# fanzhongyi/diffusion

Measured on AMD Instinct MI355X. Metric: U-Net training images/sec @256 (SD-2-base U-Net, precomputed latents 4x32x32), higher is better.
Workload: dtype bf16; 1 GPU; SD-2-base U-Net train step, latents 4x32x32, text 77x1024, batch 256/GPU (global 256), microbatch 256, AdamW, dp1; global_batch=256, microbatch=256, parallelism=dp1, params=865910724

## Files before the change

diffusion_amd/_lib.py:

```python
from __future__ import annotations

import ctypes as C
import os

_HERE = os.path.dirname(os.path.abspath(__file__))
LIB_PATH = os.path.join(_HERE, os.environ.get('DA_LIB_ALT') or 'libdiffusion_amd.so')

_vp, _l, _i, _f, _fp, _ll = C.c_void_p, C.c_long, C.c_int, C.c_float, C.c_void_p, C.c_void_p



class DaWgradItem(C.Structure):
    _fields_ = [('dY', C.c_void_p), ('lddy', C.c_long), ('X', C.c_void_p), ('ldx', C.c_long), ('dW', C.c_void_p),
                ('dbias', C.c_void_p), ('N', C.c_int), ('Cin', C.c_int)]


SIGNATURES = {
    'da_gemm_nt': [_vp, _l, _vp, _vp, _l, _fp, _vp, _l, _vp, _l, _i, _i, _i, _i, _i, _i, _i, _i, _i, _i, _i, _f, _fp, _l,
                   _vp],
    'da_set_option': [C.c_char_p, _i],
    'da_gemm_nt_variant_for': [_i, _i, _i, _i, _l],
    'da_gemm_nt_geglu': [_vp, _l, _vp, _vp, _l, _vp, _l, _fp, _i, _i, _i, _vp],
    'da_gemm_nt_geglu_bwd': [_vp, _l, _vp, _vp, _l, _vp, _l, _i, _i, _i, _vp],
    'da_gemm_tn_wgrad': [_vp, _l, _vp, _l, _fp, _fp, _fp, _i, _i, _i, _i, _i, _i, _i, _i, _i, _fp, _l, _vp],
    'da_gemm_tn_variant_for': [_i, _i, _i, _i, _i, _i, _i, _i, _i],
    'da_gemm_tn_wgrad_group': [C.POINTER(DaWgradItem), _i, _i, _fp, _l, _vp],
    'da_gemm_tn_group_plan': [C.POINTER(DaWgradItem), _i, _i, _l, C.POINTER(_i), _i, C.POINTER(_i)],
    'da_attn_fwd': [_vp, _l, _vp, _l, _vp, _l, _vp, _l, _fp, _i, _i, _i, _i, _f, _vp],
    'da_attn_fwd_causal': [_vp, _l, _vp, _l, _vp, _l, _vp, _l, _fp, _i, _i, _i, _f, _vp],
    'da_attn_fwd_wide': [_vp, _l, _vp, _l, _vp, _l, _vp, _l, _fp, _i, _i, _i, _i, _i, _f, _vp],
    'da_attn_bwd': [_vp, _l, _vp, _l, _vp, _l, _vp, _l, _vp, _l, _fp, _fp, _vp, _l, _vp, _l, _vp, _l, _i, _i, _i, _i,
                    _f, _vp],
    'da_norm_scratch_floats': [_i, _i, _i],
    'da_groupnorm_fwd': [_vp, _l, _vp, _l, _fp, _fp, _fp, _fp, _fp, _i, _i, _i, _i, _f, _i, _vp],
    'da_groupnorm_bwd': [_vp, _l, _vp, _l, _vp, _l, _vp, _l, _fp, _fp, _fp, _fp, _fp, _fp, _fp, _i, _i, _i, _i, _i,
                         _vp],
    'da_groupnorm_plan_for': [_i, _i, _i, _i, _l, _l, _i, C.POINTER(_i)],
    'da_layernorm_fwd': [_vp, _l, _vp, _l, _fp, _fp, _fp, _i, _i, _f, _vp],
    'da_layernorm_bwd': [_vp, _l, _vp, _l, _vp, _l, _vp, _l, _fp, _fp, _fp, _fp, _fp, _i, _i, _vp],
    'da_colsum_accum': [_vp, _l, _fp, _fp, _i, _i, _vp],
    'da_image_colsum': [_vp, _l, _vp, _l, _fp, _fp, _i, _i, _i, _vp],
    'da_geglu_fwd': [_vp, _l, _vp, _l, _i, _i, _vp],
    'da_geglu_bwd': [_vp, _l, _vp, _l, _vp, _l, _i, _i, _vp],
    'da_silu_fwd': [_vp, _l, _vp, _l, _i, _i, _vp],
    'da_gelu_fwd': [_vp, _l, _vp, _l, _i, _i, _vp],
    'da_silu_bwd': [_vp, _l, _vp, _l, _vp, _l, _i, _i, _vp],
    'da_quick_gelu_fwd': [_vp, _l, _vp, _l, _i, _i, _vp],
    'da_add': [_vp, _l, _vp, _l, _vp, _l, _i, _i, _vp],
    'da_copy2d': [_vp, _l, _vp, _l, _i, _i, _vp],
    'da_upsample2x_fwd': [_vp, _vp, _i, _i, _i, _i, _vp],
    'da_upsample2x_bwd': [_vp, _vp, _i, _i, _i, _i, _vp],
    'da_timestep_embed': [_ll, _vp, _i, _i, _vp],
    'da_timestep_embed_f32': [_fp, _vp, _i, _i, _vp],
    'da_add_noise': [_fp, _fp, _ll, _fp, _fp, _vp, _fp, _i, _i, _i, _vp],
    'da_add_noise_ex': [_fp, _fp, _vp, _i, _fp, _fp, _vp, _fp, _i, _i, _i, _i, _vp],
    'da_image_ingest': [_vp, _vp, _vp, _i, _i, _vp, _i, _vp],
    'da_image_ingest_rect': [_vp, _vp, _vp, _i, _i, _i, _vp, _i, _vp],
    'da_image_resize': [_vp, _vp, _vp, _i, _i, _i, _vp, _i, _i, _i, _i, _vp],
    'da_clip_preprocess': [_vp, _i, _i, _i, _i, _i, _vp, _i, _vp, _i, _fp, _fp, _vp, _i, _vp],
    'da_clip_score': [_fp, _l, _fp, _l, _i, _i, _fp, _fp, _vp],
    'da_sampler_step': [_fp, _fp, _fp, _fp, _fp, _vp, _l, _i, _i, _i, _i, _vp],
    'da_sampler_step_ms': [_fp, _fp, _fp, _fp, _fp, _vp, _l, _i, _i, _i, _i, _vp],
    'da_sampler_step_blend': [_fp, _fp, _fp, _fp, _fp, _fp, _fp, _fp, _vp, _l, _i, _i, _i, _i, _vp],
    'da_sampler_step_ms_blend': [_fp, _fp, _fp, _fp, _fp, _fp, _fp, _fp, _vp, _l, _i, _i, _i, _i, _vp],
    'da_sampler_init': [_fp, _fp, _fp, _fp, _fp, _fp, _fp, _fp, _vp, _i, _i, _i, _i, _i, _i, _vp],
    'da_guidance_rescale': [_fp, _fp, _i, _f, _fp, _l, _i, _i, _vp],
    'da_sampler_step_rs': [_fp, _fp, _fp, _fp, _fp, _fp, _vp, _l, _i, _i, _i, _i, _vp],
    'da_sampler_step_ms_rs': [_fp, _fp, _fp, _fp, _fp, _fp, _vp, _l, _i, _i, _i, _i, _vp],
    'da_sampler_step_blend_rs': [_fp, _fp, _fp, _fp, _fp, _fp, _fp, _fp, _fp, _vp, _l, _i, _i, _i, _i, _vp],
    'da_sampler_step_ms_blend_rs': [_fp, _fp, _fp, _fp, _fp, _fp, _fp, _fp, _fp, _vp, _l, _i, _i, _i, _i, _vp],
    'da_mse_loss_w': [_fp, _fp, _vp, _fp, _fp, _l, _i, _i, _ll, _fp, _i, _f, _f, _i, _vp],
    'da_mse_loss': [_fp, _fp, _vp, _fp, _fp, _l, _f, _f, _i, _vp],
    'da_mse_loss_c': [_fp, _fp, _vp, _fp, _fp, _l, _i, _f, _f, _i, _vp],
    'da_adamw': [_fp, _fp, _fp, _fp, _vp, _fp, _f, _l, _f, _f, _f, _f, _f, _i, _f, _vp],
    'da_segment_sumsq': [_fp, _vp, _i, _vp, _i, _fp, _fp, _fp, _f, _f, _vp],
    'da_segment_sumsq_scratch_floats': [_i],
    'da_adamw_dev': [_fp, _fp, _fp, _fp, _vp, _fp, _f, _l, _f, _f, _f, _f, _f, _i, _fp, _vp],
    'da_cast_f32_bf16': [_fp, _vp, _l, _vp],
    'da_transpose_weight': [_vp, _vp, _i, _i, _i, _vp],
    'da_transpose_weights_batched': [_vp, _vp, _vp, _i, _i, _vp],
}
_RESTYPES = {'da_norm_scratch_floats': C.c_long, 'da_segment_sumsq_scratch_floats': C.c_long}

_lib = None


class NativeLibraryMissing(RuntimeError):
    pass


def load():
    global _lib
    if _lib is not None:
        return _lib
    import torch
    if not os.path.exists(LIB_PATH):
        raise NativeLibraryMissing(
            f'{LIB_PATH} not found: build it with `make -C diffusion_amd/csrc` (or __graft_entry__.build()). '
            'diffusion_amd has no CPU / PyTorch fallback for its kernels.')
    lib = C.CDLL(LIB_PATH)
    for name, argtypes in SIGNATURES.items():
        fn = getattr(lib, name)
        fn.argtypes = argtypes
        fn.restype = _RESTYPES.get(name, C.c_int)
    _lib = lib
    for kv in filter(None, os.environ.get('DA_SET_OPTIONS', '').split(',')):
        k, _, v = kv.partition('=')
        if lib.da_set_option(k.strip().encode(), int(v)) != 0:
            raise ValueError(f'DA_SET_OPTIONS: da_set_option({k.strip()!r}, {v}) was rejected')
    return lib


_ERR = {1: 'DA_ERR_SHAPE (arguments rejected, nothing launched)', 2: 'DA_ERR_LAUNCH (HIP error)'}


def call(name: str, *args):
    fn = getattr(load(), name)
    rc = fn(*args)
    if rc != 0:
        raise RuntimeError(f'{name} failed: {_ERR.get(rc, rc)}')
```

diffusion_amd/csrc/gemm_nt.hip:

```cpp
#include <string.h>

#include "common.hpp"
#include "diffusion_amd.h"

namespace {

struct GemmNTParams {
  const bf16* A;
  const bf16* W;
  void* C;
  const float* bias;
  const bf16* rowbias;
  const bf16* R;
  long lda, ldc, ldrb, ldr;
  int M, N, K, Cin;
  int Hin, Win, Hout, Wout;
  int ksize, mode;
  int out_fp32;
  float alpha;
  int tiles_m, tiles_n;
};

constexpr int BM = 128, BN = 128, BK = 64;
constexpr int STAGE_BYTES = (BM + BN) * BK * 2;
constexpr int EPI_LD = 68;
constexpr int EPI_BYTES = 4 * 64 * EPI_LD * 4;
constexpr int SMEM_BYTES = (2 * STAGE_BYTES > EPI_BYTES) ? 2 * STAGE_BYTES : EPI_BYTES;

DEVINL int swz(int row, int chunk) { return row * 128 + ((chunk ^ ((row >> 1) & 7)) << 4); }

__global__ __launch_bounds__(256, 2) void gemm_nt_kernel(GemmNTParams p) {
  extern __shared__ __attribute__((aligned(16))) char smem[];
  const int tid = threadIdx.x;
  const int lane = tid & 63;
  const int wave = tid >> 6;
  const int wm = wave >> 1, wn = wave & 1;

  const int nblk = p.tiles_m * p.tiles_n;
  int bid = blockIdx.x;
  {
    const int q = nblk >> 3, r = nblk & 7;
    const int xcd = bid & 7, idx = bid >> 3;
    bid = (xcd < r ? xcd * (q + 1) : r * (q + 1) + (xcd - r) * q) + idx;
  }
  const int tm = bid / p.tiles_n, tn = bid - tm * p.tiles_n;
  const int m0 = tm * BM, n0 = tn * BN;

  const int scol = tid & 7;
  const int srow = tid >> 3;
  const int HWo = p.Hout * p.Wout;
  const int pad = (p.ksize == 3) ? 1 : 0;

  int pixbase[4], oh[4], ow[4];
  bool mval[4];
  const bf16* wptr[4];
  bool nval[4];
#pragma unroll
  for (int i = 0; i < 4; ++i) {
    int m = m0 + srow + 32 * i;
    mval[i] = m < p.M;
    int mm = mval[i] ? m : 0;
    int b = mm / HWo;
    int rem = mm - b * HWo;
    oh[i] = rem / p.Wout;
    ow[i] = rem - oh[i] * p.Wout;
    pixbase[i] = b * p.Hin * p.Win;
    int n = n0 + srow + 32 * i;
    nval[i] = n < p.N;
    wptr[i] = p.W + (long)(nval[i] ? n : 0) * p.K;
  }

  int kk = scol * 8;
  int tap = kk / p.Cin;
  int cc = kk - tap * p.Cin;

  bf16x8 ra[4], rb[4];
  auto load_tile = [&]() {
    const bool kval = kk < p.K;
    int r = 0, s = 0;
    if (p.ksize == 3) {
      r = tap / 3;
      s = tap - 3 * r;
    }
#pragma unroll
    for (int i = 0; i < 4; ++i) {
      int ih, iw;
      bool ok = kval && mval[i];
      if (p.mode == 0) {
        ih = oh[i] + r - pad;
        iw = ow[i] + s - pad;
      } else if (p.mode == 1) {
        ih = 2 * oh[i] + r - pad;
        iw = 2 * ow[i] + s - pad;
      } else if (p.mode == 4) {
        ih = 2 * oh[i] + r;
        iw = 2 * ow[i] + s;
      } else if (p.mode == 2) {
        int th = oh[i] + r - 1, tw = ow[i] + s - 1;
        ok = ok && !((th | tw) & 1);
        ih = th >> 1;
        iw = tw >> 1;
      } else {
        int th = oh[i] + r - 1, tw = ow[i] + s - 1;
        ok = ok && th >= 0 && tw >= 0 && th < p.Hout && tw < p.Wout;
        ih = th >> 1;
        iw = tw >> 1;
      }
      ok = ok && ih >= 0 && iw >= 0 && ih < p.Hin && iw < p.Win;
      ra[i] = ok ? ld8(p.A + (long)(pixbase[i] + ih * p.Win + iw) * p.lda + cc) : zero8();
      rb[i] = (kval && nval[i]) ? ld8(wptr[i] + kk) : zero8();
    }
    kk += BK;
    cc += BK;
    while (cc >= p.Cin) {
      cc -= p.Cin;
      ++tap;
    }
  };
  auto store_tile = [&](int buf) {
    char* Ab = smem + buf * STAGE_BYTES;
    char* Bb = Ab + BM * BK * 2;
#pragma unroll
    for (int i = 0; i < 4; ++i) {
      int row = srow + 32 * i;
      int off = swz(row, scol);
      *reinterpret_cast<bf16x8*>(Ab + off) = ra[i];
      *reinterpret_cast<bf16x8*>(Bb + off) = rb[i];
    }
  };

  f32x4 acc[4][4];
#pragma unroll
  for (int i = 0; i < 4; ++i)
#pragma unroll
    for (int j = 0; j < 4; ++j) acc[i][j] = f32x4{0.f, 0.f, 0.f, 0.f};

  auto compute = [&](int buf) {
    const char* Ab = smem + buf * STAGE_BYTES;
    const char* Bb = Ab + BM * BK * 2;
#pragma unroll
    for (int s = 0; s < 2; ++s) {
      bf16x8 a[4], b[4];
      const int chunk = s * 4 + (lane >> 4);
#pragma unroll
      for (int i = 0; i < 4; ++i) {
        int row = wm * 64 + i * 16 + (lane & 15);
        a[i] = *reinterpret_cast<const bf16x8*>(Ab + swz(row, chunk));
        int rowb = wn * 64 + i * 16 + (lane & 15);
        b[i] = *reinterpret_cast<const bf16x8*>(Bb + swz(rowb, chunk));
      }
#pragma unroll
      for (int i = 0; i < 4; ++i)
#pragma unroll
        for (int j = 0; j < 4; ++j)
          acc[i][j] = __builtin_amdgcn_mfma_f32_16x16x32_bf16(a[i], b[j], acc[i][j], 0, 0, 0);
    }
  };

  const int nk = (p.K + BK - 1) / BK;
  load_tile();
  store_tile(0);
  __syncthreads();
  for (int t = 0; t < nk; ++t) {
    if (t + 1 < nk) load_tile();
    compute(t & 1);
    if (t + 1 < nk) store_tile((t + 1) & 1);
    __syncthreads();
  }

  float* ew = reinterpret_cast<float*>(smem) + wave * (64 * EPI_LD);
#pragma unroll
  for (int i = 0; i < 4; ++i)
#pragma unroll
    for (int j = 0; j < 4; ++j)
#pragma unroll
      for (int e = 0; e < 4; ++e) {
        int row = i * 16 + (lane >> 4) * 4 + e;
        int col = j * 16 + (lane & 15);
        ew[row * EPI_LD + col] = acc[i][j][e];
      }
  __syncthreads();
  const int col8 = (lane & 7) * 8;
  const int n = n0 + wn * 64 + col8;
  if (n < p.N) {
    float bv[8];
#pragma unroll
    for (int e = 0; e < 8; ++e) bv[e] = p.bias ? p.bias[n + e] : 0.f;
#pragma unroll
    for (int pass = 0; pass < 8; ++pass) {
      int row = pass * 8 + (lane >> 3);
      int m = m0 + wm * 64 + row;
      if (m >= p.M) continue;
      const f32x4 v0 = *reinterpret_cast<const f32x4*>(&ew[row * EPI_LD + col8]);
      const f32x4 v1 = *reinterpret_cast<const f32x4*>(&ew[row * EPI_LD + col8 + 4]);
      float v[8] = {v0[0], v0[1], v0[2], v0[3], v1[0], v1[1], v1[2], v1[3]};
#pragma unroll
      for (int e = 0; e < 8; ++e) v[e] = v[e] * p.alpha + bv[e];
      if (p.rowbias) {
        int b = m / HWo;
        bf16x8 rbv = ld8(p.rowbias + (long)b * p.ldrb + n);
#pragma unroll
        for (int e = 0; e < 8; ++e) v[e] += bf2f(rbv[e]);
      }
      if (p.R) {
        bf16x8 rv = ld8(p.R + (long)m * p.ldr + n);
#pragma unroll
        for (int e = 0; e < 8; ++e) v[e] += bf2f(rv[e]);
      }
      if (p.out_fp32) {
        float* cp = reinterpret_cast<float*>(p.C) + (long)m * p.ldc + n;
        *reinterpret_cast<f32x4*>(cp) = f32x4{v[0], v[1], v[2], v[3]};
        *reinterpret_cast<f32x4*>(cp + 4) = f32x4{v[4], v[5], v[6], v[7]};
      } else {
        bf16x8 o;
#pragma unroll
        for (int e = 0; e < 8; ++e) o[e] = f2bf(v[e]);
        st8(reinterpret_cast<bf16*>(p.C) + (long)m * p.ldc + n, o);
      }
    }
  }
}

}

int da_gemm_nt_v2_dispatch(int variant, int splits, float* ws, const void* A, long lda, const void* W, void* C, long ldc, const float* bias,
                           const void* rowbias, long ldrb, const void* R, long ldr, int M, int N, int K, int Cin,
                           int Hin, int Win, int Hout, int Wout, int ksize, int mode, int out_fp32, float alpha,
                           hipStream_t stream);

int da_gemm_nt_v3_try(const void* A, long lda, const void* W, void* C, long ldc, const float* bias, const void* R, long ldr,
                      int M, int N, int K, hipStream_t stream);
extern int g_nt_stream, g_nt_stream_lw;
int da_gemm_nt_ws_try(const void* A, long lda, const void* W, const float* bias, const void* R, long ldr, void* C, long ldc,
                      int M, int N, int K, hipStream_t stream);
extern int g_nt_ws;

extern int g_tn_variant;
extern int g_nt_korder;
extern int g_nt_persist;
extern int g_reserve_cus;
extern int g_nt_persist_conv;
extern int g_nt_de;
extern int g_grad_overwrite;
extern int g_attn_fused_bwd;
extern int g_tn_ring, g_tn_ungroup;
extern int g_gn_resident, g_gn_resident_form, g_gn_resident_min_slab;
int da_usable_cus(int cus);
static int g_nt_variant = 0;
static int g_nt_mfma32 = 0;
static int g_nt_splitk = 1;

static int g_nt_dispatch = 1;

static int pick_nt_variant_legacy(int M, int N, int K, int Cin, long ws_floats, int* splits) {
  *splits = 1;
  const long tm = (M + 255) / 256;
  if (N % 320 == 0 && tm * (N / 320) >= 160) return 12;
  if (N % 160 == 0 && tm * (N / 160) >= 200) return 5;
  if (N % 256 == 0 && tm * (N / 256) >= 160) return 14;
  if (N % 160 != 0 && tm * ((N + 127) / 128) >= 200) return 4;
  if (N % 320 == 0 && g_nt_splitk) {
    const long tiles = tm * (N / 320);
    const int nk = K / 64;
    int s = (int)((256 + tiles - 1) / tiles);
    if (s > 8) s = 8;
    while (s > 1 && (nk / s < 8 || (long)s * M * N > ws_floats)) --s;
    if (s > 1 && tiles * s >= 96) {
      *splits = s;
      return 12;
    }
  }
  return 1;
}

static int pick_nt_variant(int M, int N, int K, int Cin, long ws_floats, int* splits) {
  *splits = 1;
  if (Cin % 64 != 0) return 1;
  if (g_nt_variant == 4 || g_nt_variant == 5 || g_nt_variant == 10 || g_nt_variant == 11 || g_nt_variant == 12 || g_nt_variant == 14 ||
      g_nt_variant == 15 || g_nt_variant == 16 || g_nt_variant == 18)
    return g_nt_variant;
  if (g_nt_variant != 0) return 1;
  if (!g_nt_dispatch) return pick_nt_variant_legacy(M, N, K, Cin, ws_floats, splits);
  struct Form { int variant, bm, bn; double step_us, fixed_us; };
  static const Form forms[] = {{12, 256, 320, 1.5, 8.0}, {14, 256, 256, 1.3, 8.0}, {5, 256, 160, 1.16, 6.0}, {18, 384, 128, 1.37, 8.0},
                               {4, 256, 128, 1.07, 5.0}};
  const int nk = K / 64;
  const int ncu = da_usable_cus(256);
  double best = 1e30;
  int best_v = 4, best_s = 1;
  for (const Form& f : forms) {
    const long tiles = ((M + f.bm - 1) / f.bm) * ((N + f.bn - 1) / f.bn);
    for (int s = 1; s <= (g_nt_splitk ? 8 : 1); ++s) {
      if (s > 1 && (nk / s < 4 || (long)s * M * N > ws_floats)) break;
      const long rounds = (tiles * s + ncu - 1) / ncu;
      const int steps = (nk + s - 1) / s;
      double t = (double)rounds * (steps * f.step_us + f.fixed_us);
      if (s > 1) t += 20.0 + ((double)s * M * N * 4.0 + (double)M * N * 2.0) / 5.0e6;
      if (t < best * 0.97) {
        best = t;
        best_v = f.variant;
        best_s = s;
      }
    }
  }
  *splits = best_s;
  if (best_v == 12 && (g_nt_mfma32 == 1 || (g_nt_mfma32 < 0 && K <= 320))) return 15;
  return best_v;
}

extern "C" int da_gemm_nt_variant_for(int M, int N, int K, int Cin, long ws_floats) {
  int s;
  return pick_nt_variant(M, N, K, Cin, ws_floats, &s);
}

extern "C" int da_set_option(const char* key, int value) {
  if (key && !strcmp(key, "gemm_nt_variant")) {
    g_nt_variant = value;
    return DA_OK;
  }
  if (key && !strcmp(key, "gemm_nt_splitk")) {
    g_nt_splitk = value;
    return DA_OK;
  }
  if (key && !strcmp(key, "gemm_nt_dispatch")) {
    g_nt_dispatch = value;
    return DA_OK;
  }
  if (key && !strcmp(key, "gemm_nt_persist")) {
    g_nt_persist = value;
    return DA_OK;
  }
  if (key && !strcmp(key, "gemm_nt_korder")) {
    g_nt_korder = value;
    return DA_OK;
  }
  if (key && !strcmp(key, "gemm_nt_mfma32")) {
    g_nt_mfma32 = value;
    return DA_OK;
  }
  if (key && !strcmp(key, "gemm_tn_variant")) {
    g_tn_variant = value;
    return DA_OK;
  }
  if (key && !strcmp(key, "attn_fused_bwd")) {
    g_attn_fused_bwd = value;
    return DA_OK;
  }
  if (key && !strcmp(key, "gemm_nt_ws")) {
    g_nt_ws = value;
    return DA_OK;
  }
  if (key && !strcmp(key, "gemm_tn_ring")) {
    if (value != 0 && value != 4 && value != 5) return DA_ERR_SHAPE;
    g_tn_ring = value;
    return DA_OK;
  }
  if (key && !strcmp(key, "gemm_tn_ungroup")) {
    if (value != 0 && value != 1) return DA_ERR_SHAPE;
    g_tn_ungroup = value;
    return DA_OK;
  }
  if (key && !strcmp(key, "gemm_nt_stream_lw")) {
    if (value != 4 && value != 16) return DA_ERR_SHAPE;
    g_nt_stream_lw = value;
    return DA_OK;
  }
  if (key && !strcmp(key, "gemm_nt_stream")) {
    g_nt_stream = value;
    return DA_OK;
  }
  if (key && !strcmp(key, "gemm_nt_de")) {
    g_nt_de = value;
    return DA_OK;
  }
  if (key && !strcmp(key, "gemm_nt_persist_conv")) {
    g_nt_persist_conv = value;
    return DA_OK;
  }
  if (key && !strcmp(key, "gn_resident")) {
    if (value < 0) return DA_ERR_SHAPE;
    g_gn_resident = value;
    return DA_OK;
  }
  if (key && !strcmp(key, "gn_resident_min_slab")) {
    if (value < 0) return DA_ERR_SHAPE;
    g_gn_resident_min_slab = value;
    return DA_OK;
  }
  if (key && !strcmp(key, "gn_resident_form")) {
    if (value < 0 || value > 2) return DA_ERR_SHAPE;
    g_gn_resident_form = value;
    return DA_OK;
  }
  if (key && !strcmp(key, "grad_overwrite")) {
    g_grad_overwrite = value ? 1 : 0;
    return DA_OK;
  }
  if (key && !strcmp(key, "reserve_cus")) {
    if (value < 0 || value > 128) return DA_ERR_SHAPE;
    g_reserve_cus = value;
    return DA_OK;
  }
  return DA_ERR_SHAPE;
}

extern "C" int da_gemm_nt(const void* A, long lda, const void* W, void* C, long ldc, const float* bias,
                          const void* rowbias, long ldrb, const void* R, long ldr, int M, int N, int K, int Cin,
                          int Hin, int Win, int Hout, int Wout, int ksize, int mode, int out_fp32, float alpha,
                          float* splitk_ws, long splitk_ws_floats, hipStream_t stream) {
  DA_CLEAR_ERR();
  if (M <= 0 || N <= 0 || K <= 0) return DA_ERR_SHAPE;
  if ((N & 7) || (Cin & 7) || (K % Cin) || (lda & 7) || (ldc & 7)) return DA_ERR_SHAPE;
  if (ksize != 1 && ksize != 3) return DA_ERR_SHAPE;
  if (K != ksize * ksize * Cin) return DA_ERR_SHAPE;
  if (mode < 0 || mode > 4) return DA_ERR_SHAPE;
  if (mode == 4 && ksize != 3) return DA_ERR_SHAPE;
  if (Hout <= 0 || Wout <= 0 || (M % (Hout * Wout))) return DA_ERR_SHAPE;
  if (R && (ldr & 7)) return DA_ERR_SHAPE;
  if (rowbias && (ldrb & 7)) return DA_ERR_SHAPE;
  if (g_nt_ws && g_nt_variant == 0 && ksize == 1 && mode == 0 && !out_fp32 && alpha == 1.0f && !rowbias) {
    const int rc = da_gemm_nt_ws_try(A, lda, W, bias, R, ldr, C, ldc, M, N, K, stream);
    if (rc >= 0) return rc;
  }
  if (g_nt_stream && g_nt_variant == 0 && ksize == 1 && mode == 0 && !out_fp32 && alpha == 1.0f && !rowbias &&
      (g_nt_stream == 2 || (K <= 640 && (long)((M + 127) / 128) * ((N + 319) / 320) >= 512))) {
    const int rc = da_gemm_nt_v3_try(A, lda, W, C, ldc, bias, R, ldr, M, N, K, stream);
    if (rc >= 0) return rc;
  }
  {
    int splits = 1;
    const int variant = pick_nt_variant(M, N, K, Cin, splitk_ws ? splitk_ws_floats : 0, &splits);
    if (variant != 1)
      return da_gemm_nt_v2_dispatch(variant, splits, splitk_ws, A, lda, W, C, ldc, bias, rowbias, ldrb, R, ldr, M, N, K, Cin, Hin, Win,
                                    Hout, Wout, ksize, mode, out_fp32, alpha, stream);
  }
  GemmNTParams p;
  p.A = (const bf16*)A; p.W = (const bf16*)W; p.C = C; p.bias = bias;
  p.rowbias = (const bf16*)rowbias; p.R = (const bf16*)R;
  p.lda = lda; p.ldc = ldc; p.ldrb = ldrb; p.ldr = ldr;
  p.M = M; p.N = N; p.K = K; p.Cin = Cin;
  p.Hin = Hin; p.Win = Win; p.Hout = Hout; p.Wout = Wout;
  p.ksize = ksize; p.mode = mode; p.out_fp32 = out_fp32; p.alpha = alpha;
  p.tiles_m = (M + BM - 1) / BM;
  p.tiles_n = (N + BN - 1) / BN;
  static unsigned long long attr_done = 0;
  if (da_ensure_dyn_smem((const void*)gemm_nt_kernel, SMEM_BYTES, &attr_done) != DA_OK) return DA_ERR_LAUNCH;
  hipLaunchKernelGGL(gemm_nt_kernel, dim3(p.tiles_m * p.tiles_n), dim3(256), SMEM_BYTES, stream, p);
  DA_CHECK_LAUNCH();
  return DA_OK;
}
```

diffusion_amd/csrc/norms.hip:

```cpp
#include "common.hpp"
#include "diffusion_amd.h"

extern int g_grad_overwrite;
int g_gn_resident = 192;
int g_gn_resident_form = 0;
int g_gn_resident_min_slab = 64 * 1024;

namespace {

struct ChanReduceParams {
  const bf16* X;
  const bf16* DY;
  const float* mean_rstd;
  const float* gamma;
  const float* beta;
  float* partial;
  long ldx, lddy;
  int HW, C, G, cpg, nchunks, ppc, pxt, silu;
};

template <int MODE>
__global__ void chan_reduce_kernel(ChanReduceParams p) {
  extern __shared__ __attribute__((aligned(16))) float red[];
  const int tid = threadIdx.x;
  const int vec0 = blockIdx.z * 512;
  const int nvec = min(512, (p.C >> 3) - vec0);
  const int Cb = nvec * 8;
  const int lvec = tid % nvec, pl = tid / nvec;
  const int vec = vec0 + lvec;
  const int b = blockIdx.y, chunk = blockIdx.x;
  const int p0 = chunk * p.ppc;
  const int p1 = min(p.HW, p0 + p.ppc);
  const bool active = pl < p.pxt;
  float s1[8], s2[8];
#pragma unroll
  for (int e = 0; e < 8; ++e) { s1[e] = 0.f; s2[e] = 0.f; }
  float rs[8], nm[8], za[8], zb[8];
  if (MODE == 1) {
#pragma unroll
    for (int e = 0; e < 8; ++e) {
      int c = 8 * vec + e;
      int g = c / p.cpg;
      const float mu = p.mean_rstd[((long)b * p.G + g) * 2];
      rs[e] = p.mean_rstd[((long)b * p.G + g) * 2 + 1];
      nm[e] = -mu * rs[e];
      za[e] = rs[e] * p.gamma[c];
      zb[e] = fmaf(nm[e], p.gamma[c], p.beta[c]);
    }
  }
  if (active) {
    for (int pix = p0 + pl; pix < p1; pix += p.pxt) {
      const long row = (long)b * p.HW + pix;
      bf16x8 x = ld8(p.X + row * p.ldx + 8 * vec);
      if (MODE == 0) {
#pragma unroll
        for (int e = 0; e < 8; ++e) {
          float v = bf2f(x[e]);
          s1[e] += v;
          s2[e] += v * v;
        }
      } else if (MODE == 1) {
        bf16x8 dy = ld8(p.DY + row * p.lddy + 8 * vec);
#pragma unroll
        for (int e = 0; e < 8; ++e) {
          const float xf = bf2f(x[e]);
          const float xh = fmaf(xf, rs[e], nm[e]);
          float dz = bf2f(dy[e]);
          if (p.silu) dz *= dsilu_f(fmaf(xf, za[e], zb[e]));
          s1[e] += dz;
          s2[e] += dz * xh;
        }
      } else {
#pragma unroll
        for (int e = 0; e < 8; ++e) s1[e] += bf2f(x[e]);
      }
    }
#pragma unroll
    for (int e = 0; e < 8; ++e) {
      red[((long)pl * Cb + 8 * lvec + e) * 2] = s1[e];
      red[((long)pl * Cb + 8 * lvec + e) * 2 + 1] = s2[e];
    }
  }
  __syncthreads();
  float* out = p.partial + (((long)b * p.nchunks + chunk) * p.C + 8 * vec0) * 2;
  for (int c = tid; c < Cb; c += blockDim.x) {
    float a = 0.f, q = 0.f;
    for (int k = 0; k < p.pxt; ++k) {
      a += red[((long)k * Cb + c) * 2];
      q += red[((long)k * Cb + c) * 2 + 1];
    }
    out[c * 2] = a;
    out[c * 2 + 1] = q;
  }
}

int launch_chan_reduce(int mode, ChanReduceParams& p, int B, hipStream_t stream) {
  const int nvec_total = p.C >> 3;
  if (nvec_total < 1) return DA_ERR_SHAPE;
  const int zsplit = (nvec_total + 511) / 512;
  const int nvec = nvec_total < 512 ? nvec_total : 512;
  int pxt = 512 / nvec;
  if (pxt > p.HW) pxt = p.HW;
  if (pxt < 1) pxt = 1;
  p.pxt = pxt;
  p.ppc = (p.HW + p.nchunks - 1) / p.nchunks;
  const size_t smem = (size_t)pxt * nvec * 8 * 2 * sizeof(float);
  dim3 grid(p.nchunks, B, zsplit), block(nvec * pxt);
  if (mode == 0) hipLaunchKernelGGL(chan_reduce_kernel<0>, grid, block, smem, stream, p);
  else if (mode == 1) hipLaunchKernelGGL(chan_reduce_kernel<1>, grid, block, smem, stream, p);
  else hipLaunchKernelGGL(chan_reduce_kernel<2>, grid, block, smem, stream, p);
  DA_CHECK_LAUNCH();
  return DA_OK;
}

int pick_chunks(int B, int HW) {
  int n = 2048 / (B > 0 ? B : 1);
  if (n > 64) n = 64;
  int maxc = HW / 16;
  if (n > maxc) n = maxc;
  if (n < 1) n = 1;
  return n;
}

constexpr int GN_GPB = 8;

DEVINL void chunk_sum2(const float* pp, long stride, int nchunks, float& a, float& q) {
  float a0 = 0.f, a1 = 0.f, q0 = 0.f, q1 = 0.f;
  int k = 0;
  for (; k + 1 < nchunks; k += 2) {
    const float2 v0 = *reinterpret_cast<const float2*>(pp + (long)k * stride);
    const float2 v1 = *reinterpret_cast<const float2*>(pp + (long)(k + 1) * stride);
    a0 += v0.x; q0 += v0.y;
    a1 += v1.x; q1 += v1.y;
  }
  if (k < nchunks) {
    const float2 v0 = *reinterpret_cast<const float2*>(pp + (long)k * stride);
    a0 += v0.x; q0 += v0.y;
  }
  a = a0 + a1;
  q = q0 + q1;
}

__global__ void gn_fwd_finalize_kernel(const float* partial, const float* gamma, const float* beta, float* mean_rstd,
                                       float* scale_shift, int C, int G, int cpg, int nchunks, int HW, float eps) {
  extern __shared__ __attribute__((aligned(16))) float sh[];
  const int b = blockIdx.x;
  const int g0 = blockIdx.y * GN_GPB, ng = min(GN_GPB, G - g0);
  const int c0 = g0 * cpg, nc = ng * cpg;
  float* gs = sh + 2 * GN_GPB * cpg;
  for (int cl = threadIdx.x; cl < nc; cl += blockDim.x) {
    float a, q;
    chunk_sum2(partial + ((long)b * nchunks * C + c0 + cl) * 2, (long)C * 2, nchunks, a, q);
    sh[2 * cl] = a;
    sh[2 * cl + 1] = q;
  }
  __syncthreads();
  for (int gl = threadIdx.x; gl < ng; gl += blockDim.x) {
    float a = 0.f, q = 0.f;
    for (int k = 0; k < cpg; ++k) {
      a += sh[2 * (gl * cpg + k)];
      q += sh[2 * (gl * cpg + k) + 1];
    }
    const float n = (float)cpg * (float)HW;
    float mean = a / n;
    float var = fmaxf(q / n - mean * mean, 0.f);
    float rstd = rsqrtf(var + eps);
    gs[2 * gl] = mean;
    gs[2 * gl + 1] = rstd;
    mean_rstd[((long)b * G + g0 + gl) * 2] = mean;
    mean_rstd[((long)b * G + g0 + gl) * 2 + 1] = rstd;
  }
  __syncthreads();
  for (int cl = threadIdx.x; cl < nc; cl += blockDim.x) {
    const int gl = cl / cpg, c = c0 + cl;
    float sc = gs[2 * gl + 1] * gamma[c];
    scale_shift[((long)b * C + c) * 2] = sc;
    scale_shift[((long)b * C + c) * 2 + 1] = beta[c] - gs[2 * gl] * sc;
  }
}

__global__ void gn_apply_kernel(const bf16* X, long ldx, bf16* Y, long ldy, const float* scale_shift, int HW, int C,
                                long total_vec, int silu) {
  const int nvec = C >> 3;
  for (long i = (long)blockIdx.x * blockDim.x + threadIdx.x; i < total_vec; i += (long)gridDim.x * blockDim.x) {
    long row = i / nvec;
    int vec = (int)(i - row * nvec);
    int b = (int)(row / HW);
    bf16x8 x = ld8(X + row * ldx + 8 * vec);
    const float* ss = scale_shift + ((long)b * C + 8 * vec) * 2;
    bf16x8 y;
#pragma unroll
    for (int e = 0; e < 8; ++e) {
      float z = bf2f(x[e]) * ss[2 * e] + ss[2 * e + 1];
      y[e] = f2bf(silu ? silu_f(z) : z);
    }
    st8(Y + row * ldy + 8 * vec, y);
  }
}

__global__ void gn_bwd_finalize_kernel(const float* partial, const float* gamma, float* coef, int C, int G, int cpg,
                                       int nchunks, int HW) {
  extern __shared__ __attribute__((aligned(16))) float sh[];
  const int b = blockIdx.x;
  const int g0 = blockIdx.y * GN_GPB, ng = min(GN_GPB, G - g0);
  const int c0 = g0 * cpg, nc = ng * cpg;
  for (int cl = threadIdx.x; cl < nc; cl += blockDim.x) {
    float a, q;
    chunk_sum2(partial + ((long)b * nchunks * C + c0 + cl) * 2, (long)C * 2, nchunks, a, q);
    sh[2 * cl] = a * gamma[c0 + cl];
    sh[2 * cl + 1] = q * gamma[c0 + cl];
  }
  __syncthreads();
  for (int gl = threadIdx.x; gl < ng; gl += blockDim.x) {
    float a = 0.f, q = 0.f;
    for (int k = 0; k < cpg; ++k) {
      a += sh[2 * (gl * cpg + k)];
      q += sh[2 * (gl * cpg + k) + 1];
    }
    const float n = (float)cpg * (float)HW;
    coef[((long)b * G + g0 + gl) * 2] = a / n;
    coef[((long)b * G + g0 + gl) * 2 + 1] = q / n;
  }
}

struct GnApplyParams {
  const bf16* X; const bf16* DY; const bf16* Radd; bf16* OUT;
  const float* mean_rstd; const float* coef; const float* gamma; const float* beta;
  long ldx, lddy, ldr, ldo;
  int HW, C, G, cpg, nchunks, ppc, pxt, silu;
};

template <bool BWD>
__global__ void gn_apply2_kernel(GnApplyParams p) {
  const int tid = threadIdx.x;
  const int vec0 = blockIdx.z * 512;
  const int nvec = min(512, (p.C >> 3) - vec0);
  const int lvec = tid % nvec, pl = tid / nvec;
  if (pl >= p.pxt) return;
  const int vec = vec0 + lvec;
  const int b = blockIdx.y, chunk = blockIdx.x;
  const int p0 = chunk * p.ppc;
  const int p1 = min(p.HW, p0 + p.ppc);
  float sc[8], sh[8], Q[8], R[8];
#pragma unroll
  for (int e = 0; e < 8; ++e) {
    const int c = 8 * vec + e;
    const int g = c / p.cpg;
    const float mu = p.mean_rstd[((long)b * p.G + g) * 2], rs = p.mean_rstd[((long)b * p.G + g) * 2 + 1];
    sc[e] = rs * p.gamma[c];
    sh[e] = p.beta[c] - mu * sc[e];
    if (BWD) {
      const float c1 = p.coef[((long)b * p.G + g) * 2], c2 = p.coef[((long)b * p.G + g) * 2 + 1];
      Q[e] = -rs * rs * c2;
      R[e] = -rs * c1 + mu * rs * rs * c2;
    }
  }
  for (int pix = p0 + pl; pix < p1; pix += p.pxt) {
    const long row = (long)b * p.HW + pix;
    const bf16x8 x = ld8(p.X + row * p.ldx + 8 * vec);
    bf16x8 o;
    if (!BWD) {
#pragma unroll
      for (int e = 0; e < 8; ++e) {
        const float z = fmaf(bf2f(x[e]), sc[e], sh[e]);
        o[e] = f2bf(p.silu ? silu_f(z) : z);
      }
    } else {
      const bf16x8 dy = ld8(p.DY + row * p.lddy + 8 * vec);
      const bf16x8 ra = p.Radd ? ld8(p.Radd + row * p.ldr + 8 * vec) : zero8();
#pragma unroll
      for (int e = 0; e < 8; ++e) {
        const float xf = bf2f(x[e]);
        float dz = bf2f(dy[e]);
        if (p.silu) dz *= dsilu_f(fmaf(xf, sc[e], sh[e]));
        o[e] = f2bf(fmaf(dz, sc[e], fmaf(xf, Q[e], R[e])) + bf2f(ra[e]));
      }
    }
    st8(p.OUT + row * p.ldo + 8 * vec, o);
  }
}

int launch_gn_apply2(bool bwd, GnApplyParams& p, int B, hipStream_t stream) {
  const int nvec_total = p.C >> 3;
  const int zsplit = (nvec_total + 511) / 512;
  const int nvec = nvec_total < 512 ? nvec_total : 512;
  int pxt = 256 / nvec;
  if (pxt < 1) pxt = 1;
  if (pxt > p.HW) pxt = p.HW;
  p.pxt = pxt;
  int nch = (4096 + B * zsplit - 1) / (B * zsplit);
  int maxc = p.HW / (4 * pxt);
  if (nch > maxc) nch = maxc;
  if (nch < 1) nch = 1;
  p.nchunks = nch;
  p.ppc = (p.HW + nch - 1) / nch;
  dim3 grid(nch, B, zsplit), block(nvec * pxt);
  if (bwd) hipLaunchKernelGGL(gn_apply2_kernel<true>, grid, block, 0, stream, p);
  else hipLaunchKernelGGL(gn_apply2_kernel<false>, grid, block, 0, stream, p);
  DA_CHECK_LAUNCH();
  return DA_OK;
}

__global__ void gn_bwd_apply_kernel(const bf16* X, long ldx, const bf16* DY, long lddy, const bf16* Radd, long ldr,
                                    bf16* DX, long lddx, const float* mean_rstd, const float* coef,
                                    const float* gamma, const float* beta, int HW, int C, int G, int cpg,
                                    long total_vec, int silu) {
  const int nvec = C >> 3;
  for (long i = (long)blockIdx.x * blockDim.x + threadIdx.x; i < total_vec; i += (long)gridDim.x * blockDim.x) {
    long row = i / nvec;
    int vec = (int)(i - row * nvec);
    int b = (int)(row / HW);
    bf16x8 x = ld8(X + row * ldx + 8 * vec);
    bf16x8 dy = ld8(DY + row * lddy + 8 * vec);
    bf16x8 ra = Radd ? ld8(Radd + row * ldr + 8 * vec) : zero8();
    bf16x8 o;
#pragma unroll
    for (int e = 0; e < 8; ++e) {
      int c = 8 * vec + e;
      int g = c / cpg;
      const float mu = mean_rstd[((long)b * G + g) * 2], rs = mean_rstd[((long)b * G + g) * 2 + 1];
      const float c1 = coef[((long)b * G + g) * 2], c2 = coef[((long)b * G + g) * 2 + 1];
      float xh = (bf2f(x[e]) - mu) * rs;
      float dz = bf2f(dy[e]);
      if (silu) dz *= dsilu_f(xh * gamma[c] + beta[c]);
      float dx = rs * (dz * gamma[c] - c1 - xh * c2);
      o[e] = f2bf(dx + bf2f(ra[e]));
    }
    st8(DX + row * lddx + 8 * vec, o);
  }
}

constexpr int CSF_CH = 16, CSF_RL = 64;
__global__ __launch_bounds__(CSF_CH * CSF_RL) void chan_sum_finalize_kernel(const float* partial, int nrows, int C,
                                                                            float* out1, float* out2, int overwrite) {
  __shared__ float sh[CSF_RL][CSF_CH][2];
  const int cx = threadIdx.x % CSF_CH, ry = threadIdx.x / CSF_CH;
  const int c = blockIdx.x * CSF_CH + cx;
  float a = 0.f, q = 0.f;
  if (c < C) {
    const float2* pp = reinterpret_cast<const float2*>(partial) + c;
    float a0 = 0.f, a1 = 0.f, a2 = 0.f, a3 = 0.f, q0 = 0.f, q1 = 0.f, q2 = 0.f, q3 = 0.f;
    int k = ry;
    for (; k + 3 * CSF_RL < nrows; k += 4 * CSF_RL) {
      const float2 v0 = pp[(long)k * C], v1 = pp[(long)(k + CSF_RL) * C], v2 = pp[(long)(k + 2 * CSF_RL) * C],
                   v3 = pp[(long)(k + 3 * CSF_RL) * C];
      a0 += v0.x; q0 += v0.y;
      a1 += v1.x; q1 += v1.y;
      a2 += v2.x; q2 += v2.y;
      a3 += v3.x; q3 += v3.y;
    }
    for (; k < nrows; k += CSF_RL) {
      const float2 v = pp[(long)k * C];
      a0 += v.x;
      q0 += v.y;
    }
    a = (a0 + a1) + (a2 + a3);
    q = (q0 + q1) + (q2 + q3);
  }
  sh[ry][cx][0] = a;
  sh[ry][cx][1] = q;
  __syncthreads();
  float la = 0.f, lq = 0.f;
  if (ry < 8) {
#pragma unroll
    for (int j = 0; j < 8; ++j) {
      la += sh[ry * 8 + j][cx][0];
      lq += sh[ry * 8 + j][cx][1];
    }
  }
  __syncthreads();
  if (ry < 8) {
    sh[ry][cx][0] = la;
    sh[ry][cx][1] = lq;
  }
  __syncthreads();
  if (ry == 0 && c < C) {
    float ta = 0.f, tq = 0.f;
#pragma unroll
    for (int j = 0; j < 8; ++j) {
      ta += sh[j][cx][0];
      tq += sh[j][cx][1];
    }
    if (out1) out1[c] = overwrite ? ta : out1[c] + ta;
    if (out2) out2[c] = overwrite ? tq : out2[c] + tq;
  }
}

static inline dim3 chan_sum_grid(int nrows, int C) {
  (void)nrows;
  return dim3((C + CSF_CH - 1) / CSF_CH);
}

__global__ __launch_bounds__(CSF_CH * CSF_RL) void image_colsum_finalize_kernel(const float* partial, bf16* out, long ldo,
                                                                                float* db, int B, int nchunks, int C,
                                                                                int overwrite) {
  __shared__ float sh[CSF_RL][CSF_CH];
  const int cx = threadIdx.x % CSF_CH, ry = threadIdx.x / CSF_CH;
  const int c = blockIdx.x * CSF_CH + cx;
  float tot = 0.f;
  if (c < C) {
    for (int b = ry; b < B; b += CSF_RL) {
      const float* pp = partial + ((long)b * nchunks * C + c) * 2;
      float a0 = 0.f, a1 = 0.f;
      int k = 0;
      for (; k + 1 < nchunks; k += 2) {
        a0 += pp[(long)k * C * 2];
        a1 += pp[(long)(k + 1) * C * 2];
      }
      if (k < nchunks) a0 += pp[(long)k * C * 2];
      const float a = a0 + a1;
      out[(long)b * ldo + c] = f2bf(a);
      tot += a;
    }
  }
  sh[ry][cx] = tot;
  __syncthreads();
  float lt = 0.f;
  if (ry < 8) {
#pragma unroll
    for (int j = 0; j < 8; ++j) lt += sh[ry * 8 + j][cx];
  }
  __syncthreads();
  if (ry < 8) sh[ry][cx] = lt;
  __syncthreads();
  if (ry == 0 && c < C && db) {
    float t = 0.f;
#pragma unroll
    for (int j = 0; j < 8; ++j) t += sh[j][cx];
    db[c] = overwrite ? t : db[c] + t;
  }
}

constexpr int LN_MAXV = 3;

__global__ __launch_bounds__(256) void ln_fwd_kernel(const bf16* X, long ldx, bf16* Y, long ldy, const float* gamma,
                                                     const float* beta, float* mean_rstd, int M, int C, float eps) {
  const int lane = threadIdx.x & 63;
  const int nvec = C >> 3;
  const int wpb = blockDim.x >> 6;
  for (int row = blockIdx.x * wpb + (threadIdx.x >> 6); row < M; row += gridDim.x * wpb) {
    float v[LN_MAXV][8];
    float s = 0.f;
#pragma unroll
    for (int k = 0; k < LN_MAXV; ++k) {
      int vec = lane + 64 * k;
      bf16x8 x = vec < nvec ? ld8(X + (long)row * ldx + 8 * vec) : zero8();
#pragma unroll
      for (int e = 0; e < 8; ++e) {
        v[k][e] = bf2f(x[e]);
        s += v[k][e];
      }
    }
    const float mean = wave_sum(s) / (float)C;
    float q = 0.f;
#pragma unroll
    for (int k = 0; k < LN_MAXV; ++k) {
      int vec = lane + 64 * k;
      if (vec < nvec) {
#pragma unroll
        for (int e = 0; e < 8; ++e) {
          float d = v[k][e] - mean;
          q += d * d;
        }
      }
    }
    const float rstd = rsqrtf(wave_sum(q) / (float)C + eps);
    if (lane == 0) {
      mean_rstd[2 * (long)row] = mean;
      mean_rstd[2 * (long)row + 1] = rstd;
    }
#pragma unroll
    for (int k = 0; k < LN_MAXV; ++k) {
      int vec = lane + 64 * k;
      if (vec < nvec) {
        bf16x8 y;
#pragma unroll
        for (int e = 0; e < 8; ++e) y[e] = f2bf((v[k][e] - mean) * rstd * gamma[8 * vec + e] + beta[8 * vec + e]);
        st8(Y + (long)row * ldy + 8 * vec, y);
      }
    }
  }
}

__global__ __launch_bounds__(256) void ln_bwd_kernel(const bf16* X, long ldx, const bf16* DY, long lddy,
                                                     const bf16* Radd, long ldr, bf16* DX, long lddx,
                                                     const float* gamma, const float* mean_rstd, float* partial,
                                                     int M, int C) {
  extern __shared__ __attribute__((aligned(16))) float red[];
  const int lane = threadIdx.x & 63, wave = threadIdx.x >> 6;
  const int nvec = C >> 3;
  const int wpb = blockDim.x >> 6;
  float dg[LN_MAXV][8], db[LN_MAXV][8], ga[LN_MAXV][8];
#pragma unroll
  for (int k = 0; k < LN_MAXV; ++k) {
    int vec = lane + 64 * k;
#pragma unroll
    for (int e = 0; e < 8; ++e) {
      dg[k][e] = 0.f;
      db[k][e] = 0.f;
      ga[k][e] = vec < nvec ? gamma[8 * vec + e] : 0.f;
    }
  }
  for (int row = blockIdx.x * wpb + wave; row < M; row += gridDim.x * wpb) {
    const float mean = mean_rstd[2 * (long)row], rstd = mean_rstd[2 * (long)row + 1];
    float xh[LN_MAXV][8], dyv[LN_MAXV][8];
    float a = 0.f, q = 0.f;
#pragma unroll
    for (int k = 0; k < LN_MAXV; ++k) {
      int vec = lane + 64 * k;
      bool ok = vec < nvec;
      bf16x8 x = ok ? ld8(X + (long)row * ldx + 8 * vec) : zero8();
      bf16x8 dy = ok ? ld8(DY + (long)row * lddy + 8 * vec) : zero8();
#pragma unroll
      for (int e = 0; e < 8; ++e) {
        xh[k][e] = ok ? (bf2f(x[e]) - mean) * rstd : 0.f;
        dyv[k][e] = bf2f(dy[e]);
        float dxh = dyv[k][e] * ga[k][e];
        a += dxh;
        q += dxh * xh[k][e];
        dg[k][e] += dyv[k][e] * xh[k][e];
        db[k][e] += dyv[k][e];
      }
    }
    a = wave_sum(a) / (float)C;
    q = wave_sum(q) / (float)C;
#pragma unroll
    for (int k = 0; k < LN_MAXV; ++k) {
      int vec = lane + 64 * k;
      if (vec < nvec) {
        bf16x8 ra = Radd ? ld8(Radd + (long)row * ldr + 8 * vec) : zero8();
        bf16x8 o;
#pragma unroll
        for (int e = 0; e < 8; ++e)
          o[e] = f2bf(rstd * (dyv[k][e] * ga[k][e] - a - xh[k][e] * q) + bf2f(ra[e]));
        st8(DX + (long)row * lddx + 8 * vec, o);
      }
    }
  }
#pragma unroll
  for (int k = 0; k < LN_MAXV; ++k) {
    int vec = lane + 64 * k;
    if (vec < nvec) {
#pragma unroll
      for (int e = 0; e < 8; ++e) {
        red[((long)wave * C + 8 * vec + e) * 2] = dg[k][e];
        red[((long)wave * C + 8 * vec + e) * 2 + 1] = db[k][e];
      }
    }
  }
  __syncthreads();
  float* out = partial + (long)blockIdx.x * C * 2;
  for (int c = threadIdx.x; c < C; c += blockDim.x) {
    float a = 0.f, q = 0.f;
    for (int w = 0; w < wpb; ++w) {
      a += red[((long)w * C + c) * 2];
      q += red[((long)w * C + c) * 2 + 1];
    }
    out[c * 2] = a;
    out[c * 2 + 1] = q;
  }
}

template <int CTRL>
DEVINL float dpp_f(float v) {
  return __builtin_bit_cast(float, __builtin_amdgcn_update_dpp(0, __builtin_bit_cast(int, v), CTRL, 0xf, 0xf, false));
}
template <int LPR>
DEVINL float group_sum(float v) {
  v += dpp_f<0xB1>(v);
  v += dpp_f<0x4E>(v);
  if (LPR >= 8) v += dpp_f<0x141>(v);
  if (LPR >= 16) v += dpp_f<0x140>(v);
  if (LPR >= 32) v += lane_xor<16>(v);
  return v;
}

template <int LPR>
__global__ __launch_bounds__(256) void ln_fwd5_kernel(const bf16* X, long ldx, bf16* Y, long ldy, const float* gamma,
                                                      const float* beta, float* mean_rstd, int M, float eps) {
  constexpr int C = 40 * LPR, RPW = 64 / LPR;
  __shared__ __attribute__((aligned(16))) float gb[2 * C];
  for (int c = threadIdx.x; c < C; c += 256) {
    gb[c] = gamma[c];
    gb[C + c] = beta[c];
  }
  __syncthreads();
  const int lane = threadIdx.x & 63, wave = threadIdx.x >> 6;
  const int sub = lane / LPR, j = lane % LPR;
  const long ngroups = ((long)M + RPW - 1) / RPW;
  for (long rg = (long)blockIdx.x * 4 + wave; rg < ngroups; rg += (long)gridDim.x * 4) {
    const long row = rg * RPW + sub;
    const bool ok = row < M;
    const long rowc = ok ? row : M - 1;
    bf16x8 xv[5];
#pragma unroll
    for (int k = 0; k < 5; ++k) xv[k] = ld8(X + rowc * ldx + 8 * (j + LPR * k));
    float s = 0.f;
#pragma unroll
    for (int k = 0; k < 5; ++k)
#pragma unroll
      for (int e = 0; e < 8; ++e) s += bf2f(xv[k][e]);
    const float mean = group_sum<LPR>(s) * (1.f / C);
    float q = 0.f;
#pragma unroll
    for (int k = 0; k < 5; ++k)
#pragma unroll
      for (int e = 0; e < 8; ++e) {
        const float d = bf2f(xv[k][e]) - mean;
        q += d * d;
      }
    const float rstd = rsqrtf(group_sum<LPR>(q) * (1.f / C) + eps);
    if (ok) {
      if (j == 0) *reinterpret_cast<float2*>(mean_rstd + 2 * row) = make_float2(mean, rstd);
#pragma unroll
      for (int k = 0; k < 5; ++k) {
        const int c0 = 8 * (j + LPR * k);
        const f32x4 g0 = *reinterpret_cast<const f32x4*>(gb + c0), g1 = *reinterpret_cast<const f32x4*>(gb + c0 + 4);
        const f32x4 b0 = *reinterpret_cast<const f32x4*>(gb + C + c0), b1 = *reinterpret_cast<const f32x4*>(gb + C + c0 + 4);
        bf16x8 y;
#pragma unroll
        for (int e = 0; e < 4; ++e) {
          y[e] = f2bf((bf2f(xv[k][e]) - mean) * rstd * g0[e] + b0[e]);
          y[e + 4] = f2bf((bf2f(xv[k][e + 4]) - mean) * rstd * g1[e] + b1[e]);
        }
        st8(Y + row * ldy + c0, y);
      }
    }
  }
}

template <int LPR, bool HAS_R>
__global__ __launch_bounds__(256) void ln_bwd5_kernel(const bf16* X, long ldx, const bf16* DY, long lddy,
                                                      const bf16* Radd, long ldr, bf16* DX, long lddx,
                                                      const float* gamma, const float* mean_rstd, float* partial,
                                                      int M) {
  constexpr int C = 40 * LPR, RPW = 64 / LPR;
  __shared__ __attribute__((aligned(16))) float gsm[C];
  __shared__ __attribute__((aligned(16))) float red[4 * C * 2];
  for (int c = threadIdx.x; c < C; c += 256) gsm[c] = gamma[c];
  __syncthreads();
  const int lane = threadIdx.x & 63, wave = threadIdx.x >> 6;
  const int sub = lane / LPR, j = lane % LPR;
  float dg[5][8], db[5][8];
#pragma unroll
  for (int k = 0; k < 5; ++k)
#pragma unroll
    for (int e = 0; e < 8; ++e) {
      dg[k][e] = 0.f;
      db[k][e] = 0.f;
    }
  const long ngroups = ((long)M + RPW - 1) / RPW;
  for (long rg = (long)blockIdx.x * 4 + wave; rg < ngroups; rg += (long)gridDim.x * 4) {
    const long row = rg * RPW + sub;
    const bool ok = row < M;
    const long rowc = ok ? row : M - 1;
    const float okf = ok ? 1.f : 0.f;
    bf16x8 xv[5], dyv[5], rv[5];
#pragma unroll
    for (int k = 0; k < 5; ++k) {
      const int c0 = 8 * (j + LPR * k);
      xv[k] = ld8(X + rowc * ldx + c0);
      dyv[k] = ld8(DY + rowc * lddy + c0);
      if (HAS_R) rv[k] = ld8(Radd + rowc * ldr + c0);
    }
    const float2 ms = *reinterpret_cast<const float2*>(mean_rstd + 2 * rowc);
    const float mean = ms.x, rstd = ms.y;
    float a = 0.f, q = 0.f;
#pragma unroll
    for (int k = 0; k < 5; ++k) {
      const int c0 = 8 * (j + LPR * k);
      const f32x4 g0 = *reinterpret_cast<const f32x4*>(gsm + c0), g1 = *reinterpret_cast<const f32x4*>(gsm + c0 + 4);
#pragma unroll
      for (int e = 0; e < 8; ++e) {
        const float xh = (bf2f(xv[k][e]) - mean) * rstd;
        const float d = bf2f(dyv[k][e]) * okf;
        const float dxh = d * (e < 4 ? g0[e & 3] : g1[e & 3]);
        a += dxh;
        q += dxh * xh;
        dg[k][e] += d * xh;
        db[k][e] += d;
      }
    }
    a = group_sum<LPR>(a) * (1.f / C);
    q = group_sum<LPR>(q) * (1.f / C);
    if (ok) {
#pragma unroll
      for (int k = 0; k < 5; ++k) {
        const int c0 = 8 * (j + LPR * k);
        const f32x4 g0 = *reinterpret_cast<const f32x4*>(gsm + c0), g1 = *reinterpret_cast<const f32x4*>(gsm + c0 + 4);
        bf16x8 o;
#pragma unroll
        for (int e = 0; e < 8; ++e) {
          const float xh = (bf2f(xv[k][e]) - mean) * rstd;
          float v = rstd * (bf2f(dyv[k][e]) * (e < 4 ? g0[e & 3] : g1[e & 3]) - a - xh * q);
          if (HAS_R) v += bf2f(rv[k][e]);
          o[e] = f2bf(v);
        }
        st8(DX + row * lddx + c0, o);
      }
    }
  }
#pragma unroll
  for (int k = 0; k < 5; ++k)
#pragma unroll
    for (int e = 0; e < 8; ++e) {
      if constexpr (LPR <= 8) {
        dg[k][e] += lane_xor<8>(dg[k][e]);
        db[k][e] += lane_xor<8>(db[k][e]);
      }
      if constexpr (LPR <= 16) {
        dg[k][e] += lane_xor<16>(dg[k][e]);
        db[k][e] += lane_xor<16>(db[k][e]);
      }
      dg[k][e] += lane_xor<32>(dg[k][e]);
      db[k][e] += lane_xor<32>(db[k][e]);
      if (sub == 0) {
        red[(wave * C + 8 * (j + LPR * k) + e) * 2] = dg[k][e];
        red[(wave * C + 8 * (j + LPR * k) + e) * 2 + 1] = db[k][e];
      }
    }
  __syncthreads();
  float* out = partial + (long)blockIdx.x * C * 2;
  for (int c = threadIdx.x; c < C; c += 256) {
    float a = 0.f, q = 0.f;
#pragma unroll
    for (int w = 0; w < 4; ++w) {
      a += red[(w * C + c) * 2];
      q += red[(w * C + c) * 2 + 1];
    }
    out[c * 2] = a;
    out[c * 2 + 1] = q;
  }
}


struct GnResParams {
  const bf16* X; const bf16* DY; const bf16* Radd; bf16* OUT;
  const float* gamma; const float* beta;
  float* mean_rstd;
  float* partial;
  long ldx, lddy, ldr, ldo;
  int HW, C, G, cpg, CW, chunks, P, parts, peers8, silu, nseg;
  float eps, inv_n;
};

DEVINL u32x4 ldnt8w(const bf16* p) { return __builtin_nontemporal_load(reinterpret_cast<const u32x4*>(p)); }
DEVINL void st8w(bf16* p, u32x4 v) { *reinterpret_cast<u32x4*>(p) = v; }
DEVINL u32x4 ldnt8o(const bf16* base, unsigned byte_off) {
  return __builtin_nontemporal_load(reinterpret_cast<const u32x4*>(reinterpret_cast<const char*>(base) + byte_off));
}
DEVINL void st8o(bf16* base, unsigned byte_off, u32x4 v) {
  *reinterpret_cast<u32x4*>(reinterpret_cast<char*>(base) + byte_off) = v;
}
DEVINL u32x4 sel8(bool ok, u32x4 v) {
  u32x4 r;
  r[0] = ok ? v[0] : 0u; r[1] = ok ? v[1] : 0u; r[2] = ok ? v[2] : 0u; r[3] = ok ? v[3] : 0u;
  return r;
}
DEVINL float bflo(unsigned w) { return __uint_as_float(w << 16); }
DEVINL float bfhi(unsigned w) { return __uint_as_float(w & 0xffff0000u); }
DEVINL unsigned bfpack(float lo, float hi) {
  bf16x2 v;
  v[0] = f2bf(lo);
  v[1] = f2bf(hi);
  return __builtin_bit_cast(unsigned, v);
}

DEVINL void gn_res_block(const GnResParams& p, int& img, int& part) {
  const int id = blockIdx.x;
  if (p.peers8) {
    const int span = 8 * p.parts;
    const int g = id / span, r = id - g * span;
    part = r >> 3;
    img = g * 8 + (r & 7);
  } else {
    img = id / p.parts;
    part = id - img * p.parts;
  }
}

DEVINL void gn_res_reduce(const GnResParams& p, const float2* red, float2* red2, float2* chs) {
  const int t = threadIdx.x, T = blockDim.x;
  __syncthreads();
  const int rows = p.P < p.HW ? p.P : p.HW;
  for (int idx = t; idx < p.nseg * p.CW; idx += T) {
    const int seg = idx / p.CW, c = idx - seg * p.CW;
    float a0 = 0.f, q0 = 0.f, a1 = 0.f, q1 = 0.f;
    int k = seg;
    for (; k + p.nseg < rows; k += 2 * p.nseg) {
      const float2 v0 = red[(long)k * p.CW + c], v1 = red[(long)(k + p.nseg) * p.CW + c];
      a0 += v0.x; q0 += v0.y;
      a1 += v1.x; q1 += v1.y;
    }
    if (k < rows) {
      const float2 v0 = red[(long)k * p.CW + c];
      a0 += v0.x; q0 += v0.y;
    }
    red2[idx] = make_float2(a0 + a1, q0 + q1);
  }
  __syncthreads();
  for (int c = t; c < p.CW; c += T) {
    float a = 0.f, q = 0.f;
    for (int sgi = 0; sgi < p.nseg; ++sgi) {
      const float2 v = red2[sgi * p.CW + c];
      a += v.x; q += v.y;
    }
    chs[c] = make_float2(a, q);
  }
  __syncthreads();
}

static inline size_t gn_res_lds_floats(int P, int CW, int nseg, int cpg) {
  return (size_t)2 * (P + 1) * CW + (size_t)2 * nseg * CW + 2 * CW + 4 * CW + 4 * (CW / cpg);
}

template <int NL, bool SILU>
__global__ __launch_bounds__(1024) void gn_res_fwd_kernel(GnResParams p) {
  extern __shared__ __attribute__((aligned(16))) float smem[];
  float2* red = reinterpret_cast<float2*>(smem);
  float2* red2 = red + (long)(p.P + 1) * p.CW;
  float2* chs = red2 + (long)p.nseg * p.CW;
  float2* cf = chs + p.CW;
  float2* gs = cf + 2 * p.CW;
  int img, part;
  gn_res_block(p, img, part);
  const int t = threadIdx.x, j = t % p.chunks, p0 = t / p.chunks;
  const bool live = p0 < p.P;
  const int c0 = part * p.CW;
  const bf16* xb = p.X + (long)img * p.HW * p.ldx + c0;
  const int pl = live ? p0 : p.P - 1;
  const int pl0 = live ? p0 : p.P;
  u32x4 a[NL];
#pragma unroll
  for (int k = 0; k < NL; ++k) {
    const int pix = pl + k * p.P;
    const int pc = pix < p.HW ? pix : p.HW - 1;
    a[k] = ldnt8o(xb, (unsigned)(pc * (int)p.ldx + 8 * j) * 2u);
  }
#pragma unroll
  for (int k = 0; k < NL; ++k) a[k] = sel8(live && pl + k * p.P < p.HW, a[k]);
#pragma unroll
  for (int w = 0; w < 4; ++w) {
    float s1 = 0.f, s2 = 0.f, u1 = 0.f, u2 = 0.f;
#pragma unroll
    for (int k = 0; k < NL; ++k) {
      const float v0 = bflo(a[k][w]), v1 = bfhi(a[k][w]);
      s1 += v0;
      s2 = fmaf(v0, v0, s2);
      u1 += v1;
      u2 = fmaf(v1, v1, u2);
    }
    red[pl0 * p.CW + 8 * j + 2 * w] = make_float2(s1, s2);
    red[pl0 * p.CW + 8 * j + 2 * w + 1] = make_float2(u1, u2);
  }
  gn_res_reduce(p, red, red2, chs);
#pragma unroll
  for (int k = 0; k < NL; ++k) reg_tie(a[k]);
  const int ng = p.CW / p.cpg, g0 = c0 / p.cpg;
  for (int gl = t; gl < ng; gl += blockDim.x) {
    float s = 0.f, q = 0.f;
    for (int i = 0; i < p.cpg; ++i) {
      const float2 v = chs[gl * p.cpg + i];
      s += v.x; q += v.y;
    }
    const float mean = s * p.inv_n;
    const float var = fmaxf(q * p.inv_n - mean * mean, 0.f);
    const float rstd = rsqrtf(var + p.eps);
    gs[gl] = make_float2(mean, rstd);
    p.mean_rstd[((long)img * p.G + g0 + gl) * 2] = mean;
    p.mean_rstd[((long)img * p.G + g0 + gl) * 2 + 1] = rstd;
  }
  __syncthreads();
  for (int c = t; c < p.CW; c += blockDim.x) {
    const float2 g = gs[c / p.cpg];
    const float sc = g.y * p.gamma[c0 + c];
    cf[c] = make_float2(sc, p.beta[c0 + c] - g.x * sc);
  }
  __syncthreads();
  if (!live) return;
#pragma unroll
  for (int w = 0; w < 4; ++w) {
    const float2 f0 = cf[8 * j + 2 * w], f1 = cf[8 * j + 2 * w + 1];
#pragma unroll
    for (int k = 0; k < NL; ++k) {
      float z0 = fmaf(bflo(a[k][w]), f0.x, f0.y), z1 = fmaf(bfhi(a[k][w]), f1.x, f1.y);
      if (SILU) {
        z0 = silu_f(z0);
        z1 = silu_f(z1);
      }
      a[k][w] = bfpack(z0, z1);
    }
    __builtin_amdgcn_sched_barrier(0);
  }
  bf16* yb = p.OUT + (long)img * p.HW * p.ldo + c0;
#pragma unroll
  for (int k = 0; k < NL; ++k) {
    const int pix = p0 + k * p.P;
    if (pix < p.HW) st8o(yb, (unsigned)(pix * (int)p.ldo + 8 * j) * 2u, a[k]);
  }
}

template <int NL, bool SILU, int T>
__global__ __launch_bounds__(T) void gn_res_bwd_kernel(GnResParams p) {
  extern __shared__ __attribute__((aligned(16))) float smem[];
  float2* red = reinterpret_cast<float2*>(smem);
  float2* red2 = red + (long)(p.P + 1) * p.CW;
  float2* chs = red2 + (long)p.nseg * p.CW;
  float4* cf = reinterpret_cast<float4*>(chs + p.CW);
  float4* gs = cf + p.CW;
  int img, part;
  gn_res_block(p, img, part);
  const int t = threadIdx.x, j = t % p.chunks, p0 = t / p.chunks;
  const bool live = p0 < p.P;
  const int c0 = part * p.CW;
  const bf16* xb = p.X + (long)img * p.HW * p.ldx + c0;
  const bf16* dyb = p.DY + (long)img * p.HW * p.lddy + c0;
  const int pl = live ? p0 : p.P - 1;
  const int pl0 = live ? p0 : p.P;
  unsigned a[NL][4], b[NL][4];
  {
    u32x4 va[NL], vb[NL];
#pragma unroll
    for (int k = 0; k < NL; ++k) {
      const int pix = pl + k * p.P;
      const int pc = pix < p.HW ? pix : p.HW - 1;
      va[k] = ldnt8o(xb, (unsigned)(pc * (int)p.ldx + 8 * j) * 2u);
      vb[k] = ldnt8o(dyb, (unsigned)(pc * (int)p.lddy + 8 * j) * 2u);
    }
#pragma unroll
    for (int k = 0; k < NL; ++k) {
      const bool ok = live && pl + k * p.P < p.HW;
#pragma unroll
      for (int w = 0; w < 4; ++w) {
        a[k][w] = ok ? va[k][w] : 0u;
        b[k][w] = ok ? vb[k][w] : 0u;
        reg_tie(b[k][w]);
      }
    }
  }
  for (int c = t; c < p.CW; c += blockDim.x) {
    const int g = (c0 + c) / p.cpg;
    const float mu = p.mean_rstd[((long)img * p.G + g) * 2], rs = p.mean_rstd[((long)img * p.G + g) * 2 + 1];
    const float nm = -mu * rs, ga = p.gamma[c0 + c];
    cf[c] = make_float4(rs, nm, rs * ga, fmaf(nm, ga, p.beta[c0 + c]));
  }
  __syncthreads();
#pragma unroll
  for (int w = 0; w < 4; ++w) {
    const float4 f0 = cf[8 * j + 2 * w], f1 = cf[8 * j + 2 * w + 1];
    float s1 = 0.f, s2 = 0.f, u1 = 0.f, u2 = 0.f;
#pragma unroll
    for (int k = 0; k < NL; ++k) {
      const float x0 = bflo(a[k][w]), x1 = bfhi(a[k][w]);
      float d0 = bflo(b[k][w]), d1 = bfhi(b[k][w]);
      if (SILU) {
        d0 *= dsilu_f(fmaf(x0, f0.z, f0.w));
        d1 *= dsilu_f(fmaf(x1, f1.z, f1.w));
        unsigned pk = bfpack(d0, d1);
        reg_tie(pk);
        b[k][w] = pk;
      }
      s1 += d0;
      s2 = fmaf(d0, fmaf(x0, f0.x, f0.y), s2);
      u1 += d1;
      u2 = fmaf(d1, fmaf(x1, f1.x, f1.y), u2);
      if (SILU) __builtin_amdgcn_sched_barrier(0);
    }
    red[pl0 * p.CW + 8 * j + 2 * w] = make_float2(s1, s2);
    red[pl0 * p.CW + 8 * j + 2 * w + 1] = make_float2(u1, u2);
    __builtin_amdgcn_sched_barrier(0);
  }
  gn_res_reduce(p, red, red2, chs);
#pragma unroll
  for (int k = 0; k < NL; ++k) {
#pragma unroll
    for (int w = 0; w < 4; ++w) {
      reg_tie(a[k][w]);
      reg_tie(b[k][w]);
    }
  }
  int j2 = j, q0 = p0;
  reg_tie(j2);
  reg_tie(q0);
  for (int c = t; c < p.CW; c += blockDim.x) {
    const float2 v = chs[c];
    p.partial[((long)img * p.C + c0 + c) * 2] = v.x;
    p.partial[((long)img * p.C + c0 + c) * 2 + 1] = v.y;
  }
  const int ng = p.CW / p.cpg, g0 = c0 / p.cpg;
  for (int gl = t; gl < ng; gl += blockDim.x) {
    float s = 0.f, q = 0.f;
    for (int i = 0; i < p.cpg; ++i) {
      const float2 v = chs[gl * p.cpg + i];
      const float ga = p.gamma[c0 + gl * p.cpg + i];
      s = fmaf(v.x, ga, s);
      q = fmaf(v.y, ga, q);
    }
    const float c1 = s * p.inv_n, c2 = q * p.inv_n;
    const float mu = p.mean_rstd[((long)img * p.G + g0 + gl) * 2], rs = p.mean_rstd[((long)img * p.G + g0 + gl) * 2 + 1];
    gs[gl] = make_float4(mu, rs, -rs * rs * c2, -rs * c1 + mu * rs * rs * c2);
  }
  __syncthreads();
  if (!live) return;
#pragma unroll
  for (int w = 0; w < 4; ++w) {
    const float4 f0 = cf[8 * j2 + 2 * w], f1 = cf[8 * j2 + 2 * w + 1];
    const float4 g0q = gs[(8 * j2 + 2 * w) / p.cpg], g1q = gs[(8 * j2 + 2 * w + 1) / p.cpg];
#pragma unroll
    for (int k = 0; k < NL; ++k) {
      const float x0 = bflo(a[k][w]), x1 = bfhi(a[k][w]);
      const float d0 = bflo(b[k][w]), d1 = bfhi(b[k][w]);
      a[k][w] = bfpack(fmaf(d0, f0.z, fmaf(x0, g0q.z, g0q.w)), fmaf(d1, f1.z, fmaf(x1, g1q.z, g1q.w)));
      if (SILU) __builtin_amdgcn_sched_barrier(0);
    }
    __builtin_amdgcn_sched_barrier(0);
  }
  bf16* ob = p.OUT + (long)img * p.HW * p.ldo + c0;
  if (p.Radd) {
    const bf16* rb = p.Radd + (long)img * p.HW * p.ldr + c0;
#pragma unroll
    for (int k = 0; k < NL; ++k) {
      const int pix = q0 + k * p.P;
      const int pc = pix < p.HW ? pix : p.HW - 1;
      const u32x4 v = ldnt8o(rb, (unsigned)(pc * (int)p.ldr + 8 * j2) * 2u);
#pragma unroll
      for (int w = 0; w < 4; ++w) b[k][w] = v[w];
    }
#pragma unroll
    for (int k = 0; k < NL; ++k)
#pragma unroll
      for (int w = 0; w < 4; ++w)
        a[k][w] = bfpack(bflo(a[k][w]) + bflo(b[k][w]), bfhi(a[k][w]) + bfhi(b[k][w]));
  }
#pragma unroll
  for (int k = 0; k < NL; ++k) {
    const int pix = q0 + k * p.P;
    if (pix < p.HW) st8o(ob, (unsigned)(pix * (int)p.ldo + 8 * j2) * 2u, u32x4{a[k][0], a[k][1], a[k][2], a[k][3]});
  }
}

bool gn_res_plan(int B, int HW, int C, int G, long ld_min, long ld_max, bool bwd, GnResParams& p, int& nl, int& threads) {
  const int cpg = C / G;
  int unit = cpg;
  while (unit & 7) unit += cpg;
  if (unit > C || (C % unit)) return false;
  if ((long)HW * ld_max * 2 >= (1L << 31)) return false;
  const int nT = (bwd && g_gn_resident_form != 1) ? 2 : 1;
  const int Ts[2] = {1024, 768};
  const int maxnl[2] = {bwd ? (g_gn_resident_form == 2 ? 8 : 11) : 21, 14};
  double best = 1e30;
  int best_cw = 0, best_t = 0;
  for (int ti = 0; ti < nT; ++ti) {
    const int T = Ts[ti];
    for (int cw = unit; cw <= C; cw += unit) {
      if (C % cw) continue;
      const int chunks = cw / 8;
      if (chunks > T) break;
      const int P = T / chunks;
      const int n = (HW + P - 1) / P;
      if (n > maxnl[ti]) continue;
      const long wgs = (long)B * (C / cw);
      if (wgs < g_gn_resident) continue;
      const bool aligned = ((cw * 2) % 128 == 0) && ((ld_min * 2) % 128 == 0);
      double cost = aligned ? 1.0 : (double)(cw * 2 + 128) / (double)(cw * 2);
      if (cost > 1.85) continue;
      if ((long)HW * cw * 2 < g_gn_resident_min_slab) continue;
      if (gn_res_lds_floats(P, cw, T / cw < 1 ? 1 : T / cw, cpg) * sizeof(float) > 160 * 1024) continue;
      cost += 0.8 * (1.0 - (double)HW / ((double)P * n)) + 0.01 * ti - 0.002 * n * T / 1024.0;
      if (wgs < 256) cost += 0.05;
      if (cost < best) { best = cost; best_cw = cw; best_t = T; }
    }
  }
  if (!best_cw) return false;
  threads = best_t;
  p.CW = best_cw;
  p.chunks = best_cw / 8;
  p.P = best_t / p.chunks;
  p.parts = C / best_cw;
  p.peers8 = (B % 8 == 0 && p.parts > 1) ? 1 : 0;
  p.nseg = best_t / best_cw < 1 ? 1 : best_t / best_cw;
  nl = (HW + p.P - 1) / p.P;
  return true;
}

template <int NL, bool SILU>
int launch_gn_res_fwd2(const GnResParams& p, int B, hipStream_t stream) {
  const size_t smem = gn_res_lds_floats(p.P, p.CW, p.nseg, p.cpg) * sizeof(float);
  if (smem > 160 * 1024) return DA_ERR_SHAPE;
  static unsigned long long attr_done = 0;
  if (da_ensure_dyn_smem((const void*)gn_res_fwd_kernel<NL, SILU>, 160 * 1024, &attr_done) != DA_OK) return DA_ERR_LAUNCH;
  hipLaunchKernelGGL((gn_res_fwd_kernel<NL, SILU>), dim3(B * p.parts), dim3(1024), smem, stream, p);
  DA_CHECK_LAUNCH();
  return DA_OK;
}

template <int NL>
int launch_gn_res_fwd(const GnResParams& p, int B, hipStream_t stream) {
  return p.silu ? launch_gn_res_fwd2<NL, true>(p, B, stream) : launch_gn_res_fwd2<NL, false>(p, B, stream);
}

template <int NL, bool SILU, int T>
int launch_gn_res_bwd2(const GnResParams& p, int B, hipStream_t stream) {
  const size_t smem = gn_res_lds_floats(p.P, p.CW, p.nseg, p.cpg) * sizeof(float);
  if (smem > 160 * 1024) return DA_ERR_SHAPE;
  static unsigned long long attr_done = 0;
  if (da_ensure_dyn_smem((const void*)gn_res_bwd_kernel<NL, SILU, T>, 160 * 1024, &attr_done) != DA_OK) return DA_ERR_LAUNCH;
  hipLaunchKernelGGL((gn_res_bwd_kernel<NL, SILU, T>), dim3(B * p.parts), dim3(T), smem, stream, p);
  DA_CHECK_LAUNCH();
  return DA_OK;
}

template <int NL, int T>
int launch_gn_res_bwd(const GnResParams& p, int B, hipStream_t stream) {
  return p.silu ? launch_gn_res_bwd2<NL, true, T>(p, B, stream) : launch_gn_res_bwd2<NL, false, T>(p, B, stream);
}

int gn_res_nl_inst(int nl, bool bwd, int threads) {
  if (bwd && threads == 768) return nl <= 11 ? 11 : 14;
  static const int fwd[] = {1, 2, 3, 4, 6, 8, 11, 16, 21}, bwd1024[] = {1, 2, 3, 4, 6, 8, 11};
  const int* v = bwd ? bwd1024 : fwd;
  const int n = bwd ? 7 : 9;
  for (int i = 0; i < n - 1; ++i)
    if (nl <= v[i]) return v[i];
  return v[n - 1];
}

int dispatch_gn_res_fwd(int nl, const GnResParams& p, int B, hipStream_t s) {
  switch (gn_res_nl_inst(nl, false, 1024)) {
    case 1: return launch_gn_res_fwd<1>(p, B, s);
    case 2: return launch_gn_res_fwd<2>(p, B, s);
    case 3: return launch_gn_res_fwd<3>(p, B, s);
    case 4: return launch_gn_res_fwd<4>(p, B, s);
    case 6: return launch_gn_res_fwd<6>(p, B, s);
    case 8: return launch_gn_res_fwd<8>(p, B, s);
    case 11: return launch_gn_res_fwd<11>(p, B, s);
    case 16: return launch_gn_res_fwd<16>(p, B, s);
    default: return launch_gn_res_fwd<21>(p, B, s);
  }
}

int dispatch_gn_res_bwd(int nl, int threads, const GnResParams& p, int B, hipStream_t s) {
  if (threads == 768) return gn_res_nl_inst(nl, true, 768) == 11 ? launch_gn_res_bwd<11, 768>(p, B, s)
                                                                  : launch_gn_res_bwd<14, 768>(p, B, s);
  switch (gn_res_nl_inst(nl, true, 1024)) {
    case 1: return launch_gn_res_bwd<1, 1024>(p, B, s);
    case 2: return launch_gn_res_bwd<2, 1024>(p, B, s);
    case 3: return launch_gn_res_bwd<3, 1024>(p, B, s);
    case 4: return launch_gn_res_bwd<4, 1024>(p, B, s);
    case 6: return launch_gn_res_bwd<6, 1024>(p, B, s);
    case 8: return launch_gn_res_bwd<8, 1024>(p, B, s);
    default: return launch_gn_res_bwd<11, 1024>(p, B, s);
  }
}

}

extern "C" long da_norm_scratch_floats(int B, int HW, int C) {
  long a = (long)B * pick_chunks(B, HW) * C * 2;
  long b = 1024L * C * 2;
  return a > b ? a : b;
}

extern "C" int da_groupnorm_plan_for(int B, int HW, int C, int G, long ld_min, long ld_max, int bwd, int* out) {
  if (B <= 0 || HW <= 0 || C <= 0 || G <= 0 || (C % G) || (C & 7) || (ld_min & 7) || (ld_max & 7) || !out) return -1;
  GnResParams r = {};
  int nl = 0, threads = 0;
  if (g_gn_resident && gn_res_plan(B, HW, C, G, ld_min, ld_max, bwd != 0, r, nl, threads)) {
    const int o[7] = {threads, gn_res_nl_inst(nl, bwd != 0, threads), r.CW, r.parts, r.peers8, r.P, 0};
    for (int i = 0; i < 7; ++i) out[i] = o[i];
    return 1;
  }
  const int o[7] = {0, 0, C, 1, 0, 0, pick_chunks(B, HW)};
  for (int i = 0; i < 7; ++i) out[i] = o[i];
  return 0;
}

extern "C" int da_groupnorm_fwd(const void* X, long ldx, void* Y, long ldy, const float* gamma, const float* beta,
                                float* mean_rstd, float* scale_shift, float* scratch, int B, int HW, int C, int G,
                                float eps, int silu, hipStream_t stream) {
  DA_CLEAR_ERR();
  if (B <= 0 || HW <= 0 || C <= 0 || G <= 0 || (C % G) || (C & 7) || (ldx & 7) || (ldy & 7)) return DA_ERR_SHAPE;
  if (g_gn_resident) {
    GnResParams r = {};
    int nl = 0, threads = 0;
    if (gn_res_plan(B, HW, C, G, ldx < ldy ? ldx : ldy, ldx > ldy ? ldx : ldy, false, r, nl, threads)) {
      r.X = (const bf16*)X; r.ldx = ldx; r.OUT = (bf16*)Y; r.ldo = ldy; r.gamma = gamma; r.beta = beta;
      r.mean_rstd = mean_rstd; r.HW = HW; r.C = C; r.G = G; r.cpg = C / G; r.silu = silu; r.eps = eps;
      r.inv_n = 1.0f / ((float)(C / G) * (float)HW);
      return dispatch_gn_res_fwd(nl, r, B, stream);
    }
  }
  ChanReduceParams p = {};
  p.X = (const bf16*)X; p.ldx = ldx; p.partial = scratch;
  p.HW = HW; p.C = C; p.G = G; p.cpg = C / G; p.nchunks = pick_chunks(B, HW);
  int rc = launch_chan_reduce(0, p, B, stream);
  if (rc) return rc;
  hipLaunchKernelGGL(gn_fwd_finalize_kernel, dim3(B, (G + GN_GPB - 1) / GN_GPB), dim3(256),
                     (size_t)(2 * GN_GPB * (C / G) + 2 * GN_GPB) * sizeof(float), stream,
                     scratch, gamma, beta, mean_rstd, scale_shift, C, G, C / G, p.nchunks, HW, eps);
  DA_CHECK_LAUNCH();
  GnApplyParams ap = {};
  ap.X = (const bf16*)X; ap.ldx = ldx; ap.OUT = (bf16*)Y; ap.ldo = ldy;
  ap.mean_rstd = mean_rstd; ap.gamma = gamma; ap.beta = beta;
  ap.HW = HW; ap.C = C; ap.G = G; ap.cpg = C / G; ap.silu = silu;
  return launch_gn_apply2(false, ap, B, stream);
}

extern "C" int da_groupnorm_bwd(const void* X, long ldx, const void* dY, long lddy, const void* Radd, long ldr,
                                void* dX, long lddx, const float* gamma, const float* beta, const float* mean_rstd,
                                float* dgamma, float* dbeta, float* coef, float* scratch, int B, int HW, int C, int G,
                                int silu, hipStream_t stream) {
  DA_CLEAR_ERR();
  if (B <= 0 || HW <= 0 || C <= 0 || G <= 0 || (C % G) || (C & 7) || (ldx & 7) || (lddy & 7) || (lddx & 7))
    return DA_ERR_SHAPE;
  if (Radd && (ldr & 7)) return DA_ERR_SHAPE;
  if (g_gn_resident) {
    GnResParams r = {};
    int nl = 0, threads = 0;
    long ldm = ldx < lddy ? ldx : lddy, ldM = ldx > lddy ? ldx : lddy;
    if (lddx < ldm) ldm = lddx;
    if (lddx > ldM) ldM = lddx;
    if (Radd && ldr > ldM) ldM = ldr;
    if (gn_res_plan(B, HW, C, G, ldm, ldM, true, r, nl, threads)) {
      r.X = (const bf16*)X; r.ldx = ldx; r.DY = (const bf16*)dY; r.lddy = lddy; r.Radd = (const bf16*)Radd; r.ldr = ldr;
      r.OUT = (bf16*)dX; r.ldo = lddx; r.gamma = gamma; r.beta = beta; r.mean_rstd = const_cast<float*>(mean_rstd);
      r.partial = scratch; r.HW = HW; r.C = C; r.G = G; r.cpg = C / G; r.silu = silu;
      r.inv_n = 1.0f / ((float)(C / G) * (float)HW);
      int rc = dispatch_gn_res_bwd(nl, threads, r, B, stream);
      if (rc) return rc;
      hipLaunchKernelGGL(chan_sum_finalize_kernel, chan_sum_grid(B, C), dim3(CSF_CH * CSF_RL), 0, stream, scratch, B, C, dbeta,
                         dgamma, g_grad_overwrite);
      DA_CHECK_LAUNCH();
      return DA_OK;
    }
  }
  ChanReduceParams p = {};
  p.X = (const bf16*)X; p.ldx = ldx; p.DY = (const bf16*)dY; p.lddy = lddy;
  p.mean_rstd = mean_rstd; p.gamma = gamma; p.beta = beta; p.partial = scratch;
  p.HW = HW; p.C = C; p.G = G; p.cpg = C / G; p.nchunks = pick_chunks(B, HW); p.silu = silu;
  int rc = launch_chan_reduce(1, p, B, stream);
  if (rc) return rc;
  hipLaunchKernelGGL(gn_bwd_finalize_kernel, dim3(B, (G + GN_GPB - 1) / GN_GPB), dim3(256),
                     (size_t)(2 * GN_GPB * (C / G)) * sizeof(float), stream, scratch,
                     gamma, coef, C, G, C / G, p.nchunks, HW);
  DA_CHECK_LAUNCH();
  hipLaunchKernelGGL(chan_sum_finalize_kernel, chan_sum_grid(B * p.nchunks, C), dim3(CSF_CH * CSF_RL), 0, stream, scratch,
                     B * p.nchunks, C, dbeta, dgamma, g_grad_overwrite);
  DA_CHECK_LAUNCH();
  GnApplyParams ap = {};
  ap.X = (const bf16*)X; ap.ldx = ldx; ap.DY = (const bf16*)dY; ap.lddy = lddy; ap.Radd = (const bf16*)Radd; ap.ldr = ldr;
  ap.OUT = (bf16*)dX; ap.ldo = lddx;
  ap.mean_rstd = mean_rstd; ap.coef = coef; ap.gamma = gamma; ap.beta = beta;
  ap.HW = HW; ap.C = C; ap.G = G; ap.cpg = C / G; ap.silu = silu;
  return launch_gn_apply2(true, ap, B, stream);
}

extern "C" int da_colsum_accum(const void* X, long ldx, float* out, float* scratch, int M, int C,
                               hipStream_t stream) {
  DA_CLEAR_ERR();
  if (M <= 0 || C <= 0 || (C & 7) || (ldx & 7)) return DA_ERR_SHAPE;
  ChanReduceParams p = {};
  p.X = (const bf16*)X; p.ldx = ldx; p.partial = scratch;
  p.HW = M; p.C = C; p.G = 1; p.cpg = C;
  int n = M / 64;
  if (n > 256) n = 256;
  if (n < 1) n = 1;
  p.nchunks = n;
  int rc = launch_chan_reduce(2, p, 1, stream);
  if (rc) return rc;
  hipLaunchKernelGGL(chan_sum_finalize_kernel, chan_sum_grid(n, C), dim3(CSF_CH * CSF_RL), 0, stream, scratch, n, C, out,
                     (float*)nullptr, g_grad_overwrite);
  DA_CHECK_LAUNCH();
  return DA_OK;
}

extern "C" int da_image_colsum(const void* X, long ldx, void* out, long ldo, float* db, float* scratch, int B, int HW,
                               int C, hipStream_t stream) {
  DA_CLEAR_ERR();
  if (B <= 0 || HW <= 0 || C <= 0 || (C & 7) || (ldx & 7)) return DA_ERR_SHAPE;
  ChanReduceParams p = {};
  p.X = (const bf16*)X; p.ldx = ldx; p.partial = scratch;
  p.HW = HW; p.C = C; p.G = 1; p.cpg = C; p.nchunks = pick_chunks(B, HW);
  int rc = launch_chan_reduce(2, p, B, stream);
  if (rc) return rc;
  hipLaunchKernelGGL(image_colsum_finalize_kernel, dim3((C + CSF_CH - 1) / CSF_CH), dim3(CSF_CH * CSF_RL), 0, stream,
                     scratch, (bf16*)out, ldo, db, B, p.nchunks, C, g_grad_overwrite);
  DA_CHECK_LAUNCH();
  return DA_OK;
}

extern "C" int da_layernorm_fwd(const void* X, long ldx, void* Y, long ldy, const float* gamma, const float* beta,
                                float* mean_rstd, int M, int C, float eps, hipStream_t stream) {
  DA_CLEAR_ERR();
  if (M <= 0 || C <= 0 || (C & 7) || C > 8 * 64 * LN_MAXV || (ldx & 7) || (ldy & 7)) return DA_ERR_SHAPE;
  if (C == 320 || C == 640 || C == 1280) {
    const int rpw = 64 / (C / 40);
    long b5 = ((long)M + 4 * rpw - 1) / (4 * rpw);
    if (b5 > 2048) b5 = 2048;
#define LN_FWD5(L) hipLaunchKernelGGL(ln_fwd5_kernel<L>, dim3((int)b5), dim3(256), 0, stream, (const bf16*)X, ldx, \
                                      (bf16*)Y, ldy, gamma, beta, mean_rstd, M, eps)
    if (C == 320) LN_FWD5(8); else if (C == 640) LN_FWD5(16); else LN_FWD5(32);
#undef LN_FWD5
    DA_CHECK_LAUNCH();
    return DA_OK;
  }
  int blocks = (M + 3) / 4;
  if (blocks > 4096) blocks = 4096;
  hipLaunchKernelGGL(ln_fwd_kernel, dim3(blocks), dim3(256), 0, stream, (const bf16*)X, ldx, (bf16*)Y, ldy, gamma,
                     beta, mean_rstd, M, C, eps);
  DA_CHECK_LAUNCH();
  return DA_OK;
}

extern "C" int da_layernorm_bwd(const void* X, long ldx, const void* dY, long lddy, const void* Radd, long ldr,
                                void* dX, long lddx, const float* gamma, const float* mean_rstd, float* dgamma,
                                float* dbeta, float* scratch, int M, int C, hipStream_t stream) {
  DA_CLEAR_ERR();
  if (M <= 0 || C <= 0 || (C & 7) || C > 8 * 64 * LN_MAXV || (ldx & 7) || (lddy & 7) || (lddx & 7))
    return DA_ERR_SHAPE;
  if (Radd && (ldr & 7)) return DA_ERR_SHAPE;
  if (C == 320 || C == 640 || C == 1280) {
    const int rpw = 64 / (C / 40);
    long b5 = ((long)M + 32 * rpw - 1) / (32 * rpw);
    if (b5 < 256) b5 = ((long)M + 4 * rpw - 1) / (4 * rpw) < 256 ? ((long)M + 4 * rpw - 1) / (4 * rpw) : 256;
    if (b5 > 1024) b5 = 1024;
#define LN_BWD5(L)                                                                                                   \
  do {                                                                                                               \
    if (Radd)                                                                                                        \
      hipLaunchKernelGGL((ln_bwd5_kernel<L, true>), dim3((int)b5), dim3(256), 0, stream, (const bf16*)X, ldx,         \
                         (const bf16*)dY, lddy, (const bf16*)Radd, ldr, (bf16*)dX, lddx, gamma, mean_rstd, scratch, M); \
    else                                                                                                             \
      hipLaunchKernelGGL((ln_bwd5_kernel<L, false>), dim3((int)b5), dim3(256), 0, stream, (const bf16*)X, ldx,        \
                         (const bf16*)dY, lddy, (const bf16*)Radd, ldr, (bf16*)dX, lddx, gamma, mean_rstd, scratch, M); \
  } while (0)
    if (C == 320) LN_BWD5(8); else if (C == 640) LN_BWD5(16); else LN_BWD5(32);
#undef LN_BWD5
    DA_CHECK_LAUNCH();
    hipLaunchKernelGGL(chan_sum_finalize_kernel, chan_sum_grid((int)b5, C), dim3(CSF_CH * CSF_RL), 0, stream, scratch, (int)b5, C,
                       dgamma, dbeta, g_grad_overwrite);
    DA_CHECK_LAUNCH();
    return DA_OK;
  }
  int blocks = (M + 3) / 4;
  if (blocks > 1024) blocks = 1024;
  hipLaunchKernelGGL(ln_bwd_kernel, dim3(blocks), dim3(256), (size_t)4 * C * 2 * sizeof(float), stream,
                     (const bf16*)X, ldx, (const bf16*)dY, lddy, (const bf16*)Radd, ldr, (bf16*)dX, lddx, gamma,
                     mean_rstd, scratch, M, C);
  DA_CHECK_LAUNCH();
  hipLaunchKernelGGL(chan_sum_finalize_kernel, chan_sum_grid(blocks, C), dim3(CSF_CH * CSF_RL), 0, stream, scratch, blocks, C,
                     dgamma, dbeta, g_grad_overwrite);
  DA_CHECK_LAUNCH();
  return DA_OK;
}
```

diffusion_amd/models/unet.py:

```python
from __future__ import annotations

import math
import os
from dataclasses import dataclass
from typing import Dict, List, Optional, Tuple

import torch
import torch.nn as nn

from .. import ops
from ..ops import BF16, F32, Geom


@dataclass
class UNetConfig:
    in_channels: int = 4
    out_channels: int = 4
    block_out_channels: Tuple[int, ...] = (320, 640, 1280, 1280)
    attention_head_dim: Tuple[int, ...] = (5, 10, 20, 20)
    cross_attention_dim: int = 1024
    layers_per_block: int = 2
    norm_num_groups: int = 32
    norm_eps: float = 1e-5
    sample_size: int = 64
# ... 245 lines not shown

    @staticmethod
    def append(entry):
        pass


class UNetOutput(dict):

    @property
    def sample(self):
        return self['sample']


def spatial_hw(S) -> Tuple[int, int]:
    if isinstance(S, (tuple, list, torch.Size)):
        if len(S) != 2:
            raise ValueError(f'a spatial size is an int or an (H, W) pair, got {S!r}')
        return int(S[0]), int(S[1])
    return int(S), int(S)


_DGRAD_FIRST = os.environ.get('DA_DGRAD_FIRST', '0') == '1'


class UNetHIP(nn.Module):
    def __init__(self, cfg: Optional[UNetConfig] = None, device='cuda', seed: int = 17, init: bool = True):
        super().__init__()
        self.cfg = cfg or UNetConfig.sd2_base()
        self.cfg.validate()
        self.config = self.cfg
        self.device_ = torch.device(device)
        if self.device_.type != 'cuda':
            raise RuntimeError('UNetHIP runs on an MI355X only (no CPU fallback); device must be cuda')
        from .. import _lib
        _lib.load()
        self.fp, self.resnet_names, self.tproj_offsets, self.tproj_total = build_layout(self.cfg)
        dev = self.device_
        fp = self.fp
        self.master = torch.zeros(fp.total, device=dev, dtype=F32)
        self.grad = torch.zeros(fp.total, device=dev, dtype=F32)
        self.exp_avg = torch.zeros(fp.total, device=dev, dtype=F32)
        self.exp_avg_sq = torch.zeros(fp.total, device=dev, dtype=F32)
        self.shadow = torch.zeros(fp.total, device=dev, dtype=BF16)
        self.shadow_t = torch.zeros(max(fp.total_t, 8), device=dev, dtype=BF16)
        self._bind_views()
        self._scratch = None
        self._scratch_key = None
        self.opt_step = 0
        self._grad_fresh = False
        self._grad_ready_cb = None
        import os
        self.wgrad_stream = torch.cuda.Stream() if os.environ.get('DA_WGRAD_STREAM', '0') == '1' else None
        self._wgrad_defer = None
        self._tape = None
        self._kv, self._record = None, True
        self._ctx = self._tproj = None
        if init:
            self.reset_parameters(seed)

    def _bind_views(self):
        fp = self.fp
        self._mats: Dict[str, Mat] = {}
        self._vecs: Dict[str, Vec] = {}
        for name, st in fp.storages.items():
            sl = slice(st.off, st.off + st.numel)
            if st.ntc is not None:
                N, T, C = st.ntc
                m = Mat()
                m.N, m.T, m.C = N, T, C
                m.w = self.shadow[sl].view(N, T * C)
                m.gw = self.grad[sl].view(N, T * C)
                m.wt = self.shadow_t[st.toff:st.toff + st.numel].view(C, T * N)
                self._mats[name] = m
            else:
                v = Vec()
                v.p = self.master[sl]
                v.g = self.grad[sl]
                self._vecs[name] = v
        self._param_index: Dict[str, nn.Parameter] = {}
        for key, sname, fn in fp.views:
            st = fp.storages[sname]
            sl = slice(st.off, st.off + st.numel)
            p = nn.Parameter(fn(self.master[sl].view(st.shape)), requires_grad=True)
            p.grad = fn(self.grad[sl].view(st.shape))
            node = self
            parts = key.split('.')
            for comp in parts[:-1]:
                if not hasattr(node, comp):
                    node.add_module(comp, _Node())
                node = getattr(node, comp)
            node.register_parameter(parts[-1], p)
            self._param_index[key] = p

    def M(self, name) -> Mat:
        return self._mats[name]

    def V(self, name) -> Vec:
        return self._vecs[name]

    @property
    def num_params(self) -> int:
        return sum(p.numel() for p in self._param_index.values())

    def reset_parameters(self, seed: int = 17):
        g = torch.Generator().manual_seed(seed)
        fan_in: Dict[str, int] = {}
        with torch.no_grad():
            for key, p in self._param_index.items():
                stem, kind = key.rsplit('.', 1)
                if 'norm' in stem.rsplit('.', 1)[-1]:
                    p.fill_(1.0 if kind == 'weight' else 0.0)
                    continue
                if kind == 'weight':
                    fan_in[stem] = math.prod(p.shape[1:])
                bound = 1.0 / math.sqrt(fan_in[stem])
                p.copy_(((torch.rand(p.shape, generator=g, dtype=torch.float64) * 2 - 1) * bound).float())
        self.sync_shadows()

    def load_state_dict(self, state_dict, strict: bool = True, assign: bool = False):
        missing = [k for k in self._param_index if k not in state_dict]
        unexpected = [k for k in state_dict if k not in self._param_index]
        if strict and (missing or unexpected):
            raise RuntimeError(f'load_state_dict: missing {missing[:5]}... unexpected {unexpected[:5]}...')
        with torch.no_grad():
            for k, p in self._param_index.items():
                if k in state_dict:
                    src = state_dict[k]
                    if tuple(src.shape) != tuple(p.shape):
                        raise RuntimeError(f'{k}: shape {tuple(src.shape)} != {tuple(p.shape)}')
                    p.copy_(src.to(device=p.device, dtype=p.dtype))
        self.sync_shadows()
        return torch.nn.modules.module._IncompatibleKeys(missing, unexpected)

    def sync_shadows(self):
        ops.cast_f32_bf16(self.master, self.shadow)
        self.refresh_transposed()

    def refresh_transposed(self):
        if getattr(self, '_tdesc', None) is None:
            import struct
            recs, first = [], 0
            for st in self.fp.storages.values():
                if st.ntc is None:
                    continue
                N, T, C = st.ntc
                recs.append(struct.pack('<qqiiii', st.off, st.toff, N, T, C, first))
                first += T * ((N + 63) // 64) * ((C + 63) // 64)
            self._tdesc = torch.frombuffer(bytearray(b''.join(recs)), dtype=torch.uint8).to(self.device_)
            self._tdesc_n, self._tdesc_blocks = len(recs), first
        ops.transpose_weights_batched(self.shadow, self.shadow_t, self._tdesc, self._tdesc_n, self._tdesc_blocks)

    def grad_segments(self):
        if getattr(self, '_gseg', None) is None:
            names, offs, numels = grad_segment_list(self.fp)
            self._gseg = (names, offs, numels, SumsqTables(list(zip(offs, numels))).to(self.device_))
        return self._gseg

    def zero_grad(self, set_to_none: bool = False):
        self.grad.zero_()
        self._grad_fresh = False

    def begin_gradient_accumulation(self):
        import os
        if os.environ.get('DA_GRAD_OVERWRITE', '1') == '0':
            self.zero_grad()
        else:
            self._grad_fresh = True

    def _apply(self, fn, recurse=True):
        return self

    def check_spatial(self, H: int, W: int):
        f = 2 ** (len(self.cfg.block_out_channels) - 1)
        if H < f or W < f or H % f or W % f:
            raise ValueError(f'U-Net input {H} x {W}: height and width must be positive multiples of {f} '
                             f'(2 ** (len(block_out_channels) - 1)), or the skip connections do not meet')

    def _ensure_scratch(self, B, H, W):
        key = (B, H, W)
        if self._scratch_key == key:
            return
        cfg = self.cfg
        dev = self.device_
        maxc = 2 * max(cfg.block_out_channels)
        need = 0
        for lvl in range(len(cfg.block_out_channels)):
            need = max(need, ops.norm_scratch_floats(B, max(1, H >> lvl) * max(1, W >> lvl), maxc))
        need = max(need, 256 * 8 * max(cfg.block_out_channels) * 2, 256 * self.tproj_total * 2,
                   1024 * max(cfg.block_out_channels) * 2, 4096)
        self._scratch = torch.empty(need, device=dev, dtype=F32)
        self._ss = torch.empty(B * maxc * 2, device=dev, dtype=F32)
        self._coef = torch.empty(B * cfg.norm_num_groups * 2, device=dev, dtype=F32)
        self._delta = torch.empty(B * max(cfg.attention_head_dim) * H * W, device=dev, dtype=F32)
        if ops.SPLITK_WS is None:
            ops.SPLITK_WS = torch.empty(32 * 1024 * 1024, device=dev, dtype=F32)
        if self.wgrad_stream is not None:
            self._wgrad_ws = torch.empty(32 * 1024 * 1024, device=dev, dtype=F32)
            self._wgrad_scratch = torch.empty(need, device=dev, dtype=F32)
        self._scratch_key = key

    def _bf(self, m, c):
        return torch.empty(m, c, device=self.device_, dtype=BF16)

    def _f32(self, n):
        return torch.empty(n, device=self.device_, dtype=F32)

    def _gn_fwd(self, x, key, B, HW, eps, silu, out=None):
        C = x.shape[1]
        G = self.cfg.norm_num_groups
        y = out if out is not None else self._bf(B * HW, C)
        st = self._f32(B * G * 2)
        ops.groupnorm_fwd(x, y, self.V(key + '.weight').p, self.V(key + '.bias').p, st, self._ss, self._scratch, B, HW,
                          C, G, eps, silu)
        return y, st

    def _gn_bwd(self, x, dy, radd, key, st, B, HW, silu, out=None):
        C = x.shape[1]
        G = self.cfg.norm_num_groups
        dx = out if out is not None else self._bf(B * HW, C)
        w, b = self.V(key + '.weight'), self.V(key + '.bias')
        ops.groupnorm_bwd(x, dy, radd, dx, w.p, b.p, st, w.g, b.g, self._coef, self._scratch, B, HW, C, G, silu)
        return dx

    def _wgrad(self, dy, x, gw, g, dbias=None, scratch=None):
        ws = self.wgrad_stream
        if ws is None:
            d = self._wgrad_defer
            if d is not None and g.ksize == 1 and g.mode == 0 and dy.shape[0] == d[0]:
                d[1].append((dy, x, gw, dbias))
                return
            ops.gemm_tn_wgrad(dy, x, gw, g, dbias=dbias, scratch=scratch)
            return
        main = torch.cuda.current_stream()
        ev = torch.cuda.Event()
        ev.record(main)
        ws.wait_event(ev)
        dy.record_stream(ws)
        x.record_stream(ws)
        with torch.cuda.stream(ws):
            old = ops.SPLITK_WS
            ops.SPLITK_WS = self._wgrad_ws
            try:
                ops.gemm_tn_wgrad(dy, x, gw, g, dbias=dbias, scratch=self._wgrad_scratch if scratch is not None else None)
            finally:
                ops.SPLITK_WS = old

    def _lin_fwd(self, x, key, out=None, bias=True, residual=None):
        m = self.M(key + '.weight')
        M = x.shape[0]
        y = out if out is not None else self._bf(M, m.N)
        ops.gemm_nt(x, m.w, y, Geom.linear(M), bias=self.V(key + '.bias').p if bias else None, residual=residual)
        return y

    def _lin_bwd(self, x, dy, key, bias=True, need_dx=True, dx_out=None):
        m = self.M(key + '.weight')
        M = x.shape[0]
        if _DGRAD_FIRST and need_dx:
            dx = dx_out if dx_out is not None else self._bf(M, m.C)
            ops.gemm_nt(dy, m.wt, dx, Geom.linear(M))
            self._wgrad(dy, x, m.gw, Geom.linear(M), dbias=self.V(key + '.bias').g if bias else None, scratch=self._scratch)
            return dx
        self._wgrad(dy, x, m.gw, Geom.linear(M), dbias=self.V(key + '.bias').g if bias else None,
                          scratch=self._scratch)
        if not need_dx:
            return None
        dx = dx_out if dx_out is not None else self._bf(M, m.C)
        ops.gemm_nt(dy, m.wt, dx, Geom.linear(M))
        return dx

    def _resnet_fwd(self, p, x, B, H, W, out=None):
        cfg = self.cfg
        HW = H * W
        M = B * HW
        conv1, conv2 = self.M(p + '.conv1.weight'), self.M(p + '.conv2.weight')
        cout = conv1.N
        g3 = Geom.conv(B, H, W)
        a1, st1 = self._gn_fwd(x, p + '.norm1', B, HW, cfg.norm_eps, 1)
        h1 = self._bf(M, cout)
        to = self.tproj_offsets[p]
        ops.gemm_nt(a1, conv1.w, h1, g3, bias=self.V(p + '.conv1.bias').p, rowbias=self._tproj[:, to:to + cout])
        a2, st2 = self._gn_fwd(h1, p + '.norm2', B, HW, cfg.norm_eps, 1)
        short = (p + '.conv_shortcut.weight') in self._mats
        if short:
            xs = self._bf(M, cout)
            ops.gemm_nt(x, self.M(p + '.conv_shortcut.weight').w, xs, Geom.conv(B, H, W, 1),
                        bias=self.V(p + '.conv_shortcut.bias').p)
            res = xs
        else:
            res = x
        y = out if out is not None else self._bf(M, cout)
        ops.gemm_nt(a2, conv2.w, y, g3, bias=self.V(p + '.conv2.bias').p, residual=res)
        return y, ((p, x, a1, st1, h1, a2, st2, B, H, W) if self._record else None)

    def _resnet_bwd(self, saved, dout):
        p, x, a1, st1, h1, a2, st2, B, H, W = saved
        HW = H * W
        M = B * HW
        conv1, conv2 = self.M(p + '.conv1.weight'), self.M(p + '.conv2.weight')
        cout, cin = conv1.N, conv1.C
        g3 = Geom.conv(B, H, W)
        self._wgrad(dout, a2, conv2.gw, g3, dbias=self.V(p + '.conv2.bias').g, scratch=self._scratch)
        da2 = self._bf(M, cout)
        ops.gemm_nt(dout, conv2.wt, da2, g3)
        dh1 = self._gn_bwd(h1, da2, None, p + '.norm2', st2, B, HW, 1)
        del da2
        to = self.tproj_offsets[p]
        ops.image_colsum(dh1, self._dtproj[:, to:to + cout], self.V(p + '.conv1.bias').g, self._scratch, B, HW)
        self._wgrad(dh1, a1, conv1.gw, g3)
        da1 = self._bf(M, cin)
        ops.gemm_nt(dh1, conv1.wt, da1, g3)
        del dh1
        if (p + '.conv_shortcut.weight') in self._mats:
            sm = self.M(p + '.conv_shortcut.weight')
            g1 = Geom.conv(B, H, W, 1)
            self._wgrad(dout, x, sm.gw, g1, dbias=self.V(p + '.conv_shortcut.bias').g, scratch=self._scratch)
            dxs = self._bf(M, cin)
            ops.gemm_nt(dout, sm.wt, dxs, g1)
        else:
            dxs = dout
        return self._gn_bwd(x, da1, dxs, p + '.norm1', st1, B, HW, 1)

    def _ln_fwd(self, x, key):
        y = self._bf(*x.shape)
        st = self._f32(2 * x.shape[0])
        ops.layernorm_fwd(x, y, self.V(key + '.weight').p, self.V(key + '.bias').p, st)
        return y, st

    def _ln_bwd(self, x, dy, radd, key, st):
        dx = self._bf(*x.shape)
        w, b = self.V(key + '.weight'), self.V(key + '.bias')
        ops.layernorm_bwd(x, dy, radd, dx, w.p, st, w.g, b.g, self._scratch)
        return dx

    def _transformer_fwd(self, p, x, B, H, W, heads, out=None):
        HW = H * W
        M = B * HW
        C = x.shape[1]
        tb = p + '.transformer_blocks.0'
        g, gst = self._gn_fwd(x, p + '.norm', B, HW, 1e-6, 0)
        h0 = self._lin_fwd(g, p + '.proj_in')
        n1, ln1 = self._ln_fwd(h0, tb + '.norm1')
        qkv = self._bf(M, 3 * C)
        ops.gemm_nt(n1, self.M(tb + '.attn1.qkv.weight').w, qkv, Geom.linear(M))
        o1 = self._bf(M, C)
        l1 = self._f32(B * heads * HW)
        ops.attn_fwd(qkv[:, :C], qkv[:, C:2 * C], qkv[:, 2 * C:], o1, l1, B, heads, HW, HW, 0.125)
        h1 = self._lin_fwd(o1, tb + '.attn1.to_out.0', residual=h0)
        n2, ln2 = self._ln_fwd(h1, tb + '.norm2')
        q2 = self._lin_fwd(n2, tb + '.attn2.to_q', bias=False)
        nk = self._ctx.shape[0] // B
        if self._kv is not None:
            kv2 = self._kv[p]
        else:
            kv2 = self._bf(B * nk, 2 * C)
            ops.gemm_nt(self._ctx, self.M(tb + '.attn2.kv.weight').w, kv2, Geom.linear(B * nk))
        o2 = self._bf(M, C)
        l2 = self._f32(B * heads * HW)
        ops.attn_fwd(q2, kv2[:, :C], kv2[:, C:], o2, l2, B, heads, HW, nk, 0.125)
        h2 = self._lin_fwd(o2, tb + '.attn2.to_out.0', residual=h1)
        n3, ln3 = self._ln_fwd(h2, tb + '.norm3')
        gg = self._bf(M, 4 * C)
        if ops.geglu_fusable(4 * C, C):
            f = self._bf(M, 8 * C)
            ops.gemm_nt_geglu(n3, self.M(tb + '.ff.net.0.proj.weight').w, f, gg, self.V(tb + '.ff.net.0.proj.bias').p)
        else:
            f = self._lin_fwd(n3, tb + '.ff.net.0.proj')
            ops.geglu_fwd(f, gg)
        h3 = self._lin_fwd(gg, tb + '.ff.net.2', residual=h2)
        y = self._lin_fwd(h3, p + '.proj_out', out=out, residual=x)
        if not self._record:
            return y, None
        saved = (p, x, gst, g, h0, ln1, n1, qkv, o1, l1, h1, ln2, n2, q2, kv2, o2, l2, h2, ln3, n3, f, gg, h3, B, H, W,
                 heads)
        return y, saved

    def _transformer_bwd(self, saved, dout):
        if self.wgrad_stream is None:
            self._wgrad_defer = (dout.shape[0], [])
        try:
            return self._transformer_bwd_chain(saved, dout)
        finally:
            self._wgrad_defer = None

    def _transformer_bwd_chain(self, saved, dout):
        (p, x, gst, g, h0, ln1, n1, qkv, o1, l1, h1, ln2, n2, q2, kv2, o2, l2, h2, ln3, n3, f, gg, h3, B, H, W,
         heads) = saved
        HW = H * W
        M = B * HW
        C = x.shape[1]
        tb = p + '.transformer_blocks.0'
        nk = self._ctx.shape[0] // B
        dh3 = self._lin_bwd(h3, dout, p + '.proj_out')
        df = self._bf(M, 8 * C)
        if ops.geglu_bwd_fusable(4 * C, C):
            self._lin_bwd(gg, dh3, tb + '.ff.net.2', need_dx=False)
            ops.gemm_nt_geglu_bwd(dh3, self.M(tb + '.ff.net.2.weight').wt, f, df)
        else:
            dgg = self._lin_bwd(gg, dh3, tb + '.ff.net.2')
            ops.geglu_bwd(f, dgg, df)
            del dgg
        dn3 = self._lin_bwd(n3, df, tb + '.ff.net.0.proj')
        del df
        dh2 = self._ln_bwd(h2, dn3, dh3, tb + '.norm3', ln3)
        do2 = self._lin_bwd(o2, dh2, tb + '.attn2.to_out.0')
        dq2 = self._bf(M, C)
        dkv2 = self._bf(B * nk, 2 * C)
        ops.attn_bwd(q2, kv2[:, :C], kv2[:, C:], o2, do2, l2, self._delta, dq2, dkv2[:, :C], dkv2[:, C:], B, heads, HW,
                     nk, 0.125)
        self._wgrad(dkv2, self._ctx, self.M(tb + '.attn2.kv.weight').gw, Geom.linear(B * nk))
        dn2 = self._lin_bwd(n2, dq2, tb + '.attn2.to_q', bias=False)
        dh1 = self._ln_bwd(h1, dn2, dh2, tb + '.norm2', ln2)
        do1 = self._lin_bwd(o1, dh1, tb + '.attn1.to_out.0')
        dqkv = self._bf(M, 3 * C)
        ops.attn_bwd(qkv[:, :C], qkv[:, C:2 * C], qkv[:, 2 * C:], o1, do1, l1, self._delta, dqkv[:, :C],
                     dqkv[:, C:2 * C], dqkv[:, 2 * C:], B, heads, HW, HW, 0.125)
        mq = self.M(tb + '.attn1.qkv.weight')
        self._wgrad(dqkv, n1, mq.gw, Geom.linear(M))
        dn1 = self._bf(M, C)
        ops.gemm_nt(dqkv, mq.wt, dn1, Geom.linear(M))
        dh0 = self._ln_bwd(h0, dn1, dh1, tb + '.norm1', ln1)
        dg = self._lin_bwd(g, dh0, p + '.proj_in')
        if self._wgrad_defer is not None:
            items, self._wgrad_defer = self._wgrad_defer[1], None
            ops.gemm_tn_wgrad_group(items, M)
            del items
        return self._gn_bwd(x, dg, dout, p + '.norm', gst, B, HW, 0)

    def forward_features(self, xt8: torch.Tensor, t: torch.Tensor, ctx: torch.Tensor, B: int, S, kv=None,
                         record: bool = True):
        if kv is None and record:
            return self._walk(xt8, t, ctx, B, S)
        if kv is not None and record:
            raise ValueError('forward_features: kv is for the forward-only walk (backward needs the projections it made)')
        keep = (self._ctx, self._tproj)
        self._kv, self._record = kv, False
        try:
            return self._walk(xt8, t, ctx, B, S)
        finally:
            self._kv, self._record = None, True
            self._ctx, self._tproj = keep

    def project_context(self, ctx: torch.Tensor):
        kv = {}
        for key in self._mats:
            if key.endswith('.attn2.kv.weight'):
                m = self.M(key)
                out = self._bf(ctx.shape[0], m.N)
                ops.gemm_nt(ctx, m.w, out, Geom.linear(ctx.shape[0]))
                kv[key[:-len('.transformer_blocks.0.attn2.kv.weight')]] = out
        return kv

    def _walk(self, xt8, t, ctx, B, S):
        cfg = self.cfg
        boc = cfg.block_out_channels
        n = len(boc)
        record = self._record
        H, W = spatial_hw(S)
        self.check_spatial(H, W)
        if xt8.shape[0] != B * H * W:
            raise ValueError(f'forward_features: {xt8.shape[0]} input rows for B * H * W = {B} * {H} * {W}')
        self._ensure_scratch(B, H, W)
        self._ctx = ctx
        tape = [] if record else _NoTape()
        te0 = self._bf(B, boc[0])
        if t.dtype == F32:
            ops.timestep_embed_f32(t, te0)
        else:
            ops.timestep_embed(t, te0)
        te1 = self._lin_fwd(te0, 'time_embedding.linear_1')
        te1s = self._bf(B, cfg.time_embed_dim)
        ops.silu_fwd(te1, te1s)
        temb = self._lin_fwd(te1s, 'time_embedding.linear_2')
        tembs = self._bf(B, cfg.time_embed_dim)
        ops.silu_fwd(temb, tembs)
        self._tproj = self._bf(B, self.tproj_total)
        ops.gemm_nt(tembs, self.M('time_emb_proj_all.weight').w, self._tproj, Geom.linear(B),
                    bias=self.V('time_emb_proj_all.bias').p)
        if record:
            self._temb_saved = (te0, te1, te1s, temb, tembs)
        del te0, te1, te1s, temb, tembs

        res = [(H >> i, W >> i) for i in range(n)]
        cats: List[torch.Tensor] = []
        cat_cb: List[int] = []

        def skip_slot(M, C):
            s = len(cats)
            i, j = divmod(3 * n - 1 - s, cfg.layers_per_block + 1)
            cb, cs, _ = up_block_resnet_channels(cfg, i, j)
            assert cs == C, (s, cs, C)
            buf = self._bf(M, cb + cs)
            cats.append(buf)
            cat_cb.append(cb)
            return buf[:, cb:]

        h = skip_slot(B * H * W, boc[0])
        ci = self.M('conv_in.weight')
        ops.gemm_nt(xt8, ci.w, h, Geom.conv(B, H, W), bias=self.V('conv_in.bias').p)
        tape.append(('conv_in', (xt8, B, H, W)))
        for i in range(n):
            rh, rw = res[i]
            for j in range(cfg.layers_per_block):
                p = f'down_blocks.{i}.resnets.{j}'
                if i < n - 1:
                    h, sv = self._resnet_fwd(p, h, B, rh, rw)
                    tape.append(('resnet', sv))
                    h, sv = self._transformer_fwd(f'down_blocks.{i}.attentions.{j}', h, B, rh, rw,
                                                  cfg.attention_head_dim[i], out=skip_slot(B * rh * rw, boc[i]))
                    tape.append(('transformer', sv))
                else:
                    h, sv = self._resnet_fwd(p, h, B, rh, rw, out=skip_slot(B * rh * rw, boc[i]))
                    tape.append(('resnet', sv))
                tape.append(('skip', (len(cats) - 1,)))
            if i < n - 1:
                m = self.M(f'down_blocks.{i}.downsamplers.0.conv.weight')
                y = skip_slot(B * (rh // 2) * (rw // 2), boc[i])
                ops.gemm_nt(h, m.w, y, Geom.down(B, rh, rw), bias=self.V(f'down_blocks.{i}.downsamplers.0.conv.bias').p)
                tape.append(('down', (f'down_blocks.{i}.downsamplers.0.conv', h, B, rh, rw)))
                tape.append(('skip', (len(cats) - 1,)))
                h = y
        rh, rw = res[-1]
        h, sv = self._resnet_fwd('mid_block.resnets.0', h, B, rh, rw)
        tape.append(('resnet', sv))
        h, sv = self._transformer_fwd('mid_block.attentions.0', h, B, rh, rw, cfg.attention_head_dim[-1])
        tape.append(('transformer', sv))
        s = len(cats) - 1
        h, sv = self._resnet_fwd('mid_block.resnets.1', h, B, rh, rw, out=cats[s][:, :cat_cb[s]])
        tape.append(('resnet', sv))
        rev_heads = tuple(reversed(cfg.attention_head_dim))
        rev = tuple(reversed(boc))
        for i in range(n):
            rh, rw = res[n - 1 - i]
            for j in range(cfg.layers_per_block + 1):
                last = (i == n - 1 and j == cfg.layers_per_block)
                cat = cats[s]
                tape.append(('cat', (s, cat_cb[s])))
                nxt = None
                if not last and j < cfg.layers_per_block:
                    nxt = cats[s - 1][:, :cat_cb[s - 1]]
                p = f'up_blocks.{i}.resnets.{j}'
                if i > 0:
                    h, sv = self._resnet_fwd(p, cat, B, rh, rw)
                    tape.append(('resnet', sv))
                    h, sv = self._transformer_fwd(f'up_blocks.{i}.attentions.{j}', h, B, rh, rw, rev_heads[i], out=nxt)
                    tape.append(('transformer', sv))
                else:
                    h, sv = self._resnet_fwd(p, cat, B, rh, rw, out=nxt)
                    tape.append(('resnet', sv))
                if not record:
                    cats[s] = cat = None
                s -= 1
            if i < n - 1:
                key = f'up_blocks.{i}.upsamplers.0.conv'
                y = cats[s][:, :cat_cb[s]]
                ops.gemm_nt(h, self.M(key + '.weight').w, y, Geom.up(B, rh, rw), bias=self.V(key + '.bias').p)
                tape.append(('up', (key, h, B, rh, rw)))
                h = y
        a, st = self._gn_fwd(h, 'conv_norm_out', B, H * W, cfg.norm_eps, 1)
        pred = torch.empty(B * H * W, 8, device=self.device_, dtype=F32)
        ops.gemm_nt(a, self.M('conv_out.weight').w, pred, Geom.conv(B, H, W), bias=self.V('conv_out.bias').p)
        if not record:
            return pred
        tape.append(('out', (h, a, st, B, H, W)))
        self._tape = tape
        self._cats = cats
        return pred

    def backward_features(self, dpred: torch.Tensor):
        tape, self._tape = self._tape, None
        if tape is None:
            raise RuntimeError('backward_features called without a recorded forward')
        fresh, self._grad_fresh = getattr(self, '_grad_fresh', False), False
        if fresh:
            ops.set_option('grad_overwrite', 1)
        try:
            self._backward_walk(tape, dpred)
        finally:
            if fresh:
                ops.set_option('grad_overwrite', 0)

    def _backward_walk(self, tape, dpred: torch.Tensor):
        B = dpred.shape[0]
        self._dtproj = self._bf(self._tproj.shape[0], self.tproj_total)
        dskip: Dict[int, torch.Tensor] = {}
        dh = None
        off = lambda name: self.fp.storages[name].off
        for kind, sv in reversed(tape):
            lo = None
            if kind == 'out':
                lo = off('conv_norm_out.weight')
                h, a, st, B, H, W = sv
                m = self.M('conv_out.weight')
                g3 = Geom.conv(B, H, W)
                self._wgrad(dpred, a, m.gw, g3, dbias=self.V('conv_out.bias').g, scratch=self._scratch)
                da = self._bf(B * H * W, m.C)
                ops.gemm_nt(dpred, m.wt, da, g3)
                dh = self._gn_bwd(h, da, None, 'conv_norm_out', st, B, H * W, 1)
            elif kind == 'resnet':
                dh = self._resnet_bwd(sv, dh)
                lo = off(sv[0] + '.norm1.weight')
            elif kind == 'transformer':
                dh = self._transformer_bwd(sv, dh)
                lo = off(sv[0] + '.norm.weight')
            elif kind == 'up':
                key, x, B, rh, rw = sv
                lo = off(key + '.weight')
                m = self.M(key + '.weight')
                self._wgrad(dh, x, m.gw, Geom.up(B, rh, rw), dbias=self.V(key + '.bias').g, scratch=self._scratch)
                dup = self._bf(B * 4 * rh * rw, m.C)
                ops.gemm_nt(dh, m.wt, dup, Geom.conv(B, 2 * rh, 2 * rw))
# ... 80 lines not shown
```

diffusion_amd/ops.py:

```python
from __future__ import annotations

import ctypes
import os
from typing import Optional, Tuple

import torch

from . import _lib

BF16 = torch.bfloat16
F32 = torch.float32


def _stream() -> int:
    return torch.cuda.current_stream().cuda_stream


SPLITK_WS = None


PROFILE = None


class _Timed:
# ... 13 lines not shown
            end.record()
            PROFILE.setdefault(self.name, []).append((self.start, end, self.flops))
            if self.tag is not None:
                PROFILE.setdefault('_shapes', []).append((self.start, end, self.flops, (self.name,) + self.tag))


def _mat(x: torch.Tensor, dtype=BF16, name='arg') -> Tuple[int, int]:
    if x.dim() != 2 or x.stride(1) != 1 or x.dtype != dtype or not x.is_cuda:
        raise ValueError(f'{name}: need a 2-D {dtype} device matrix with unit column stride, got '
                         f'{tuple(x.shape)} strides {x.stride()} {x.dtype} {x.device}')
    ld = x.stride(0) if x.shape[0] > 1 else max(x.stride(0), x.shape[1])
    if ld % 8 or x.shape[1] % 8 or (x.data_ptr() % 16):
        raise ValueError(f'{name}: columns, row stride and base must be multiples of 8 elements / 16 bytes')
    return x.data_ptr(), ld


def _vec(x: Optional[torch.Tensor], n: int, name='vec') -> int:
    if x is None:
        return 0
    if x.dtype != F32 or not x.is_contiguous() or x.numel() != n or not x.is_cuda:
        raise ValueError(f'{name}: need contiguous fp32[{n}] on device, got {tuple(x.shape)} {x.dtype}')
    return x.data_ptr()


def _f32buf(x: torch.Tensor, min_numel: int, name='buf') -> int:
    if x.dtype != F32 or not x.is_contiguous() or x.numel() < min_numel or not x.is_cuda:
        raise ValueError(f'{name}: need contiguous fp32 buffer of >= {min_numel} elements')
    return x.data_ptr()


_OPTS = {}


def set_option(key: str, value: int):
    _lib.call('da_set_option', key.encode(), int(value))
    _OPTS[key] = int(value)


def _opt(key: str, default: int) -> int:
    if key in _OPTS:
        return _OPTS[key]
    for kv in filter(None, os.environ.get('DA_SET_OPTIONS', '').split(',')):
        k, _, v = kv.partition('=')
        if k.strip() == key:
            return int(v)
    return default


class Geom:
    __slots__ = ('B', 'Hin', 'Win', 'Hout', 'Wout', 'ksize', 'mode')

    def __init__(self, B, Hin, Win, Hout, Wout, ksize, mode):
        self.B, self.Hin, self.Win, self.Hout, self.Wout, self.ksize, self.mode = B, Hin, Win, Hout, Wout, ksize, mode

    @staticmethod
    def linear(M):
        return Geom(M, 1, 1, 1, 1, 1, 0)

    @staticmethod
    def conv(B, H, W, ksize=3):
        return Geom(B, H, W, H, W, ksize, 0)

    @staticmethod
    def down(B, H, W):
        return Geom(B, H, W, H // 2, W // 2, 3, 1)

    @staticmethod
    def down_vae(B, H, W):
        return Geom(B, H, W, H // 2, W // 2, 3, 4)

    @staticmethod
    def down_dgrad(B, H, W):
        return Geom(B, H // 2, W // 2, H, W, 3, 2)

    @staticmethod
    def up(B, H, W):
        return Geom(B, H, W, 2 * H, 2 * W, 3, 3)


def gemm_nt(A, W, out, g: Geom, *, bias=None, rowbias=None, residual=None, alpha=1.0):
    a_ptr, lda = _mat(A, BF16, 'A')
    w_ptr, ldw = _mat(W, BF16, 'W')
    N, K = W.shape
    Cin = A.shape[1]
    if ldw != K or K != g.ksize * g.ksize * Cin:
        raise ValueError(f'W must be contiguous [N, {g.ksize * g.ksize * Cin}], got {tuple(W.shape)} ld {ldw}')
    M = g.B * g.Hout * g.Wout
    if A.shape[0] != g.B * g.Hin * g.Win:
        raise ValueError(f'A rows {A.shape[0]} != B*Hin*Win {g.B * g.Hin * g.Win}')
    out_fp32 = out.dtype == F32
    c_ptr, ldc = _mat(out, F32 if out_fp32 else BF16, 'out')
    if tuple(out.shape) != (M, N):
        raise ValueError(f'out shape {tuple(out.shape)} != {(M, N)}')
    rb_ptr, ldrb = (0, 0)
    if rowbias is not None:
        rb_ptr, ldrb = _mat(rowbias, BF16, 'rowbias')
        if tuple(rowbias.shape) != (g.B, N):
            raise ValueError('rowbias must be [B, N]')
    r_ptr, ldr = (0, 0)
    if residual is not None:
        r_ptr, ldr = _mat(residual, BF16, 'residual')
        if tuple(residual.shape) != (M, N):
            raise ValueError('residual must be [M, N]')
    flops = 2.0 * M * N * K * (0.25 if g.mode == 2 else 1.0)
    name = 'gemm_nt'
    if PROFILE is not None:
        v = _lib.load().da_gemm_nt_variant_for(M, N, K, Cin, SPLITK_WS.numel() if SPLITK_WS is not None else 0)
        name = {1: 'gemm_nt_kernel', 4: 'gemm_nt2_kernel<4,4,4,2>', 5: 'gemm_nt2_kernel<4,5,4,2>',
                10: 'gemm_nt2_kernel<8,5,2,4>', 11: 'gemm_nt2_kernel<4,10,2,2>', 12: 'gemm_nt2_kernel<4,5,4,4>',
                14: 'gemm_nt2_kernel<4,4,4,4>', 15: 'gemm_nt2_kernel<1,5,8,2,mf32>', 16: 'gemm_nt2_kernel<2,5,4,2,mf32>',
                18: 'gemm_nt2_kernel<3,4,8,2>'}[v]
        ws = _opt('gemm_nt_ws', 1)
        ws_bn = 320 if (K == 320 and (ws & 1) and N <= 1280) else 128 if (K == 640 and (ws & 2) and N <= 1024) else 0
        if (ws_bn and _opt('gemm_nt_variant', 0) == 0 and N % ws_bn == 0 and M % 32 == 0 and (M // 32) * (N // ws_bn) >= 8 * 256
                and g.ksize == 1 and g.mode == 0 and not out_fp32 and alpha == 1.0 and rowbias is None):
            name = 'gemm_nt_ws_kernel'
    with _Timed(name, flops, (M, N, K, g.ksize, g.mode)):
        _lib.call('da_gemm_nt', a_ptr, lda, w_ptr, c_ptr, ldc, _vec(bias, N, 'bias'), rb_ptr, ldrb, r_ptr, ldr, M, N,
                  K, Cin, g.Hin, g.Win, g.Hout, g.Wout, g.ksize, g.mode, int(out_fp32), float(alpha),
                  SPLITK_WS.data_ptr() if SPLITK_WS is not None else 0,
                  SPLITK_WS.numel() if SPLITK_WS is not None else 0, _stream())
    return out


def geglu_fusable(inner: int, K: int) -> bool:
    return inner % 160 == 0 and K % 64 == 0


def gemm_nt_geglu(A, W, F, G, bias):
    a_ptr, lda = _mat(A, BF16, 'A')
    w_ptr, ldw = _mat(W, BF16, 'W')
    f_ptr, ldf = _mat(F, BF16, 'F')
    g_ptr, ldg = _mat(G, BF16, 'G')
    M, K = A.shape
    inner = G.shape[1]
    if tuple(W.shape) != (2 * inner, K) or ldw != K or tuple(F.shape) != (M, 2 * inner) or G.shape[0] != M:
        raise ValueError('gemm_nt_geglu: shape mismatch')
    if not geglu_fusable(inner, K):
        raise ValueError(f'gemm_nt_geglu needs inner % 160 == 0 and K % 64 == 0, got {inner}, {K}')
    with _Timed('gemm_nt2_kernel<4,5,4,4>', 2.0 * M * 2 * inner * K, (M, 2 * inner, K, 1, 'geglu')):
        _lib.call('da_gemm_nt_geglu', a_ptr, lda, w_ptr, f_ptr, ldf, g_ptr, ldg, _vec(bias, 2 * inner, 'bias'), M, inner,
                  K, _stream())


def geglu_bwd_fusable(inner: int, K: int) -> bool:
    return inner % 320 == 0 and K % 64 == 0


def gemm_nt_geglu_bwd(dY, Wt, F, dF):
    dy_ptr, lddy = _mat(dY, BF16, 'dY')
    w_ptr, ldw = _mat(Wt, BF16, 'Wt')
    f_ptr, ldf = _mat(F, BF16, 'F')
    df_ptr, lddf = _mat(dF, BF16, 'dF')
    M, K = dY.shape
    inner = Wt.shape[0]
    if ldw != K or Wt.shape[1] != K or tuple(F.shape) != (M, 2 * inner) or tuple(dF.shape) != (M, 2 * inner):
        raise ValueError('gemm_nt_geglu_bwd: shape mismatch')
    if not geglu_bwd_fusable(inner, K):
        raise ValueError(f'gemm_nt_geglu_bwd needs inner % 320 == 0 and K % 64 == 0, got {inner}, {K}')
    with _Timed('gemm_nt2_kernel<4,5,4,4>', 2.0 * M * inner * K, (M, inner, K, 1, 'geglu_bwd')):
        _lib.call('da_gemm_nt_geglu_bwd', dy_ptr, lddy, w_ptr, f_ptr, ldf, df_ptr, lddf, M, inner, K, _stream())


def gemm_tn_wgrad(dY, X, dW, g: Geom, dbias=None, scratch=None):
    dy_ptr, lddy = _mat(dY, BF16, 'dY')
    x_ptr, ldx = _mat(X, BF16, 'X')
    M, N = dY.shape
    Cin = X.shape[1]
    if M != g.B * g.Hout * g.Wout or X.shape[0] != g.B * g.Hin * g.Win:
        raise ValueError('wgrad: row counts do not match the geometry')
    if dW.dtype != F32 or not dW.is_contiguous() or dW.numel() != N * g.ksize * g.ksize * Cin:
        raise ValueError(f'dW must be contiguous fp32 with {N * g.ksize * g.ksize * Cin} elements')
    mode = g.mode
    if mode == 2:
        raise ValueError('wgrad has no mode 2')
    with _Timed('gemm_tn', 2.0 * M * N * g.ksize * g.ksize * Cin, (M, N, g.ksize * g.ksize * Cin, g.ksize, g.mode)):
        db = _vec(dbias, N, 'dbias') if dbias is not None else 0
        sc = _f32buf(scratch, 256 * N * 2, 'scratch') if dbias is not None else 0
        _lib.call('da_gemm_tn_wgrad', dy_ptr, lddy, x_ptr, ldx, dW.data_ptr(), db, sc, M, N, Cin, g.Hin, g.Win,
                  g.Hout, g.Wout, g.ksize, mode, SPLITK_WS.data_ptr() if SPLITK_WS is not None else 0,
                  SPLITK_WS.numel() if SPLITK_WS is not None else 0, _stream())


def _wgrad_items(items, M):
    arr = (_lib.DaWgradItem * max(len(items), 1))()
    flops = 0.0
    for i, (dY, X, dW, dbias) in enumerate(items):
        dy_ptr, lddy = _mat(dY, BF16, f'items[{i}].dY')
        x_ptr, ldx = _mat(X, BF16, f'items[{i}].X')
        N, Cin = dY.shape[1], X.shape[1]
        if dY.shape[0] != M or X.shape[0] != M:
            raise ValueError(f'wgrad group: items[{i}] has {dY.shape[0]} / {X.shape[0]} rows, the group has {M}')
        if dW.dtype != F32 or not dW.is_contiguous() or dW.numel() != N * Cin or not dW.is_cuda:
            raise ValueError(f'items[{i}].dW must be contiguous fp32 with {N * Cin} elements on the device')
        db = _vec(dbias, N, f'items[{i}].dbias') if dbias is not None else 0
        arr[i] = _lib.DaWgradItem(dy_ptr, lddy, x_ptr, ldx, dW.data_ptr(), db or None, N, Cin)
        flops += 2.0 * M * N * Cin
    return arr, flops


def gemm_tn_wgrad_group(items, M):
    if not items:
        return
    arr, flops = _wgrad_items(items, M)
    with _Timed('gemm_tn', flops, (M, len(items), 0, 1, 'group')):
        _lib.call('da_gemm_tn_wgrad_group', arr, len(items), M, SPLITK_WS.data_ptr() if SPLITK_WS is not None else 0,
                  SPLITK_WS.numel() if SPLITK_WS is not None else 0, _stream())


def gemm_tn_group_plan(shapes, M, ws_floats):
    n = len(shapes)
    arr = (_lib.DaWgradItem * max(n, 1))()
    for i, (N, Cin, has_db) in enumerate(shapes):
        arr[i] = _lib.DaWgradItem(None, N, None, Cin, None, 1 if has_db else None, N, Cin)
    splits = (ctypes.c_int * max(n, 1))()
    group_of = (ctypes.c_int * max(n, 1))()
    ng = _lib.load().da_gemm_tn_group_plan(arr, n, M, int(ws_floats), splits, n, group_of)
    if ng < 0:
        raise ValueError('da_gemm_tn_group_plan rejected the arguments')
    return {'splits': list(splits[:ng]), 'group_of': list(group_of[:n])}


def attn_fwd(Q, K, V, O, L2, B, H, Nq, Nk, scale):
    q, ldq = _mat(Q, BF16, 'Q')
    k, ldk = _mat(K, BF16, 'K')
    v, ldv = _mat(V, BF16, 'V')
    o, ldo = _mat(O, BF16, 'O')
    for t, n in ((Q, Nq), (O, Nq), (K, Nk), (V, Nk)):
        if tuple(t.shape) != (B * n, H * 64):
            raise ValueError(f'attention operand shape {tuple(t.shape)} != {(B * n, H * 64)}')
    with _Timed('attn_fwd', 4.0 * B * H * Nq * Nk * 64, (B, H, Nq, Nk, 0)):
        _lib.call('da_attn_fwd', q, ldq, k, ldk, v, ldv, o, ldo, _f32buf(L2, B * H * Nq, 'L2'), B, H, Nq, Nk,
                  float(scale), _stream())


def attn_fwd_wide(Q, K, V, O, L2, B, H, D, Nq, Nk, scale):
    q, ldq = _mat(Q, BF16, 'Q')
    k, ldk = _mat(K, BF16, 'K')
    v, ldv = _mat(V, BF16, 'V')
    o, ldo = _mat(O, BF16, 'O')
    for t, n in ((Q, Nq), (O, Nq), (K, Nk), (V, Nk)):
        if tuple(t.shape) != (B * n, H * D):
            raise ValueError(f'attention operand shape {tuple(t.shape)} != {(B * n, H * D)}')
    with _Timed('attn_fwd_wide', 4.0 * B * H * Nq * Nk * D, (B, H, Nq, Nk, D)):
        _lib.call('da_attn_fwd_wide', q, ldq, k, ldk, v, ldv, o, ldo, _f32buf(L2, B * H * Nq, 'L2'), B, H, D, Nq, Nk,
                  float(scale), _stream())


def attn_fwd_causal(Q, K, V, O, L2, B, H, N, scale):
    q, ldq = _mat(Q, BF16, 'Q')
    k, ldk = _mat(K, BF16, 'K')
    v, ldv = _mat(V, BF16, 'V')
    o, ldo = _mat(O, BF16, 'O')
    for t in (Q, K, V, O):
        if tuple(t.shape) != (B * N, H * 64):
            raise ValueError(f'attention operand shape {tuple(t.shape)} != {(B * N, H * 64)}')
    _lib.call('da_attn_fwd_causal', q, ldq, k, ldk, v, ldv, o, ldo, _f32buf(L2, B * H * N, 'L2'), B, H, N, float(scale),
              _stream())


def attn_bwd(Q, K, V, O, dO, L2, Delta, dQ, dK, dV, B, H, Nq, Nk, scale):
    ptrs = []
    for t, n, nm in ((Q, Nq, 'Q'), (K, Nk, 'K'), (V, Nk, 'V'), (O, Nq, 'O'), (dO, Nq, 'dO')):
        if tuple(t.shape) != (B * n, H * 64):
            raise ValueError(f'{nm} shape {tuple(t.shape)} != {(B * n, H * 64)}')
        ptrs += list(_mat(t, BF16, nm))
    outs = []
    for t, n, nm in ((dQ, Nq, 'dQ'), (dK, Nk, 'dK'), (dV, Nk, 'dV')):
        if tuple(t.shape) != (B * n, H * 64):
            raise ValueError(f'{nm} shape {tuple(t.shape)} != {(B * n, H * 64)}')
        outs += list(_mat(t, BF16, nm))
    with _Timed('attn_bwd', 8.0 * B * H * Nq * Nk * 64, (B, H, Nq, Nk, 0)):
        _lib.call('da_attn_bwd', *ptrs, _f32buf(L2, B * H * Nq, 'L2'), _f32buf(Delta, B * H * Nq, 'Delta'), *outs, B,
                  H, Nq, Nk, float(scale), _stream())


def norm_scratch_floats(B, HW, C) -> int:
    return int(_lib.load().da_norm_scratch_floats(B, HW, C))


def groupnorm_fwd(X, Y, gamma, beta, mean_rstd, scale_shift, scratch, B, HW, C, G, eps, silu):
    x, ldx = _mat(X, BF16, 'X')
    y, ldy = _mat(Y, BF16, 'Y')
    if tuple(X.shape) != (B * HW, C) or tuple(Y.shape) != (B * HW, C):
        raise ValueError('groupnorm: bad shapes')
    _lib.call('da_groupnorm_fwd', x, ldx, y, ldy, _vec(gamma, C), _vec(beta, C), _f32buf(mean_rstd, B * G * 2),
              _f32buf(scale_shift, B * C * 2), _f32buf(scratch, norm_scratch_floats(B, HW, C)), B, HW, C, G,
              float(eps), int(silu), _stream())


def groupnorm_bwd(X, dY, Radd, dX, gamma, beta, mean_rstd, dgamma, dbeta, coef, scratch, B, HW, C, G, silu):
    x, ldx = _mat(X, BF16, 'X')
    dy, lddy = _mat(dY, BF16, 'dY')
    dx, lddx = _mat(dX, BF16, 'dX')
    r, ldr = _mat(Radd, BF16, 'Radd') if Radd is not None else (0, 0)
    for t in (X, dY, dX) + ((Radd,) if Radd is not None else ()):
        if tuple(t.shape) != (B * HW, C):
            raise ValueError('groupnorm_bwd: bad shapes')
    _lib.call('da_groupnorm_bwd', x, ldx, dy, lddy, r, ldr, dx, lddx, _vec(gamma, C), _vec(beta, C),
              _f32buf(mean_rstd, B * G * 2), _vec(dgamma, C), _vec(dbeta, C), _f32buf(coef, B * G * 2),
              _f32buf(scratch, norm_scratch_floats(B, HW, C)), B, HW, C, G, int(silu), _stream())


GN_PLAN_FIELDS = ('threads', 'nl', 'cw', 'parts', 'peers8', 'P', 'nchunks')


def groupnorm_plan(B, HW, C, G, ld_min=None, ld_max=None, bwd=False) -> dict:
    out = (ctypes.c_int * 7)()
    ld_min = C if ld_min is None else ld_min
    ld_max = ld_min if ld_max is None else ld_max
    form = _lib.load().da_groupnorm_plan_for(B, HW, C, G, ld_min, ld_max, int(bool(bwd)), out)
    if form < 0:
        raise ValueError(f'groupnorm_plan: arguments rejected ({B}, {HW}, {C}, {G}, {ld_min}, {ld_max})')
    return dict(form='resident' if form == 1 else 'multipass', **dict(zip(GN_PLAN_FIELDS, out)))


def layernorm_fwd(X, Y, gamma, beta, mean_rstd, eps=1e-5):
    x, ldx = _mat(X, BF16, 'X')
    y, ldy = _mat(Y, BF16, 'Y')
    M, C = X.shape
    _lib.call('da_layernorm_fwd', x, ldx, y, ldy, _vec(gamma, C), _vec(beta, C), _f32buf(mean_rstd, 2 * M), M, C,
              float(eps), _stream())


def layernorm_bwd(X, dY, Radd, dX, gamma, mean_rstd, dgamma, dbeta, scratch):
    x, ldx = _mat(X, BF16, 'X')
    dy, lddy = _mat(dY, BF16, 'dY')
    dx, lddx = _mat(dX, BF16, 'dX')
    r, ldr = _mat(Radd, BF16, 'Radd') if Radd is not None else (0, 0)
    M, C = X.shape
    _lib.call('da_layernorm_bwd', x, ldx, dy, lddy, r, ldr, dx, lddx, _vec(gamma, C), _f32buf(mean_rstd, 2 * M),
              _vec(dgamma, C), _vec(dbeta, C), _f32buf(scratch, 1024 * C * 2), M, C, _stream())


def colsum_accum(X, out, scratch):
    x, ldx = _mat(X, BF16, 'X')
    M, C = X.shape
    _lib.call('da_colsum_accum', x, ldx, _vec(out, C), _f32buf(scratch, 256 * C * 2), M, C, _stream())


def image_colsum(X, out, db, scratch, B, HW):
    x, ldx = _mat(X, BF16, 'X')
    o, ldo = _mat(out, BF16, 'out')
    C = X.shape[1]
    if tuple(out.shape) != (B, C) or X.shape[0] != B * HW:
        raise ValueError('image_colsum: bad shapes')
    _lib.call('da_image_colsum', x, ldx, o, ldo, _vec(db, C) if db is not None else 0,
              _f32buf(scratch, norm_scratch_floats(B, HW, C)), B, HW, C, _stream())


def _map2d(entry, *mats, wide=()):
    args = [v for m in mats for v in _mat(m, BF16, entry)]
    M, C = mats[0].shape[0], mats[0].shape[1] // (2 if 0 in wide else 1)
    for k, m in enumerate(mats):
        if tuple(m.shape) != (M, 2 * C if k in wide else C):
            raise ValueError(f'{entry[3:]}: shape mismatch: operand {k} is {tuple(m.shape)}, operand 0 '
                             f'{tuple(mats[0].shape)}' + (f' (operands {wide} have twice the columns)' if wide else ''))
    _lib.call(entry, *args, M, C, _stream())
    return mats[-1]


def geglu_fwd(inp, out):
    _map2d('da_geglu_fwd', inp, out, wide=(0,))


def geglu_bwd(inp, dout, din):
    _map2d('da_geglu_bwd', inp, dout, din, wide=(0, 2))


def silu_fwd(x, y):
    _map2d('da_silu_fwd', x, y)


def gelu_fwd(x, y):
    _map2d('da_gelu_fwd', x, y)


def quick_gelu_fwd(x, y):
    _map2d('da_quick_gelu_fwd', x, y)


def silu_bwd(x, dy, dx):
    _map2d('da_silu_bwd', x, dy, dx)


def add(a, b, out):
    return _map2d('da_add', a, b, out)


def copy2d(a, out):
    return _map2d('da_copy2d', a, out)


def upsample2x_bwd(dy, dx, B, H, W, C):
    if not (dy.is_contiguous() and dx.is_contiguous()) or dy.numel() != 4 * B * H * W * C or dx.numel() != B * H * W * C:
        raise ValueError('upsample2x_bwd: bad shapes')
    _lib.call('da_upsample2x_bwd', dy.data_ptr(), dx.data_ptr(), B, H, W, C, _stream())


def upsample2x_fwd(x, y, B, H, W, C):
    if not (x.is_contiguous() and y.is_contiguous()) or y.numel() != 4 * B * H * W * C or x.numel() != B * H * W * C:
        raise ValueError('upsample2x_fwd: bad shapes')
    _lib.call('da_upsample2x_fwd', x.data_ptr(), y.data_ptr(), B, H, W, C, _stream())


def timestep_embed(t, out):
    if t.dtype != torch.int64 or not t.is_contiguous() or out.dtype != BF16 or not out.is_contiguous():
        raise ValueError('timestep_embed: t int64 contiguous, out bf16 contiguous')
    _lib.call('da_timestep_embed', t.data_ptr(), out.data_ptr(), t.numel(), out.shape[1], _stream())


def timestep_embed_f32(t, out):
    if t.dtype != F32 or not t.is_cuda or not t.is_contiguous() or out.dtype != BF16 or not out.is_cuda \
            or not out.is_contiguous() or out.shape[0] != t.numel():
        raise ValueError('timestep_embed_f32: t fp32 [B] on device, out bf16 [B, dim] on device, both contiguous')
    _lib.call('da_timestep_embed_f32', t.data_ptr(), out.data_ptr(), t.numel(), out.shape[1], _stream())


NOISE_TARGETS = {'epsilon': 0, 'v_prediction': 1, 'sample': 2}


def add_noise_ex(x0, eps, t, xt, target, prediction_type='epsilon', sqrt_ac=None, sqrt_1mac=None):
    if x0.dim() != 4:
        raise ValueError('add_noise_ex: x0/eps must be [B,C,H,W]')
    B, C = x0.shape[0], x0.shape[1]
    HW = x0.shape[2] * x0.shape[3]
    for z in (x0, eps):
        if z.dtype != F32 or not z.is_cuda or not z.is_contiguous() or z.shape != x0.shape:
            raise ValueError('add_noise_ex: x0/eps must be contiguous fp32 [B,C,H,W] device tensors')
    if not 1 <= C <= 8:
        raise ValueError(f'add_noise_ex: {C} channels (1..8 supported)')
    for z, dt in ((xt, BF16), (target, F32)):
        if z.dtype != dt or not z.is_cuda or not z.is_contiguous() or z.numel() != B * HW * 8 or z.data_ptr() % 16:
            raise ValueError('add_noise_ex: xt bf16 [B*HW,8], target fp32 [B*HW,8], contiguous on device')
    if not t.is_cuda or not t.is_contiguous() or t.numel() != B:
        raise ValueError('add_noise_ex: t must be a contiguous [B] device tensor')
    if prediction_type not in NOISE_TARGETS:
        raise ValueError(f'add_noise_ex: unknown prediction_type {prediction_type!r}')
    if t.dtype == F32:
        is_f32, pa, pb = 1, None, None
    elif t.dtype == torch.int64:
        if sqrt_ac is None or sqrt_1mac is None or int(sqrt_ac.numel()) != int(sqrt_1mac.numel()):
            raise ValueError('add_noise_ex: discrete t needs both sqrt(abar) tables')
        is_f32, pa, pb = 0, _vec(sqrt_ac, sqrt_ac.numel(), 'sqrt_ac'), _vec(sqrt_1mac, sqrt_1mac.numel(), 'sqrt_1mac')
    else:
        raise ValueError(f'add_noise_ex: t must be int64 (discrete) or fp32 (continuous), got {t.dtype}')
    _lib.call('da_add_noise_ex', x0.data_ptr(), eps.data_ptr(), t.data_ptr(), is_f32, pa, pb, xt.data_ptr(),
              target.data_ptr(), B, C, HW, NOISE_TARGETS[prediction_type], _stream())


IMAGE_INGEST_MAX_SIDE = 65535


def _image_ingest_args(fn, raw, off, hw, Rh, Rw, out, kind, host):
    for z, dt, nm in ((raw, torch.uint8, 'raw uint8'), (off, torch.int64, 'off int64'), (hw, torch.int32, 'hw int32')):
        if not isinstance(z, torch.Tensor) or not z.is_cuda or z.dtype != dt or not z.is_contiguous():
            raise ValueError(f'{fn}: {nm} must be a contiguous device tensor')
    B = int(off.numel())
    if raw.dim() != 1 or off.dim() != 1 or B < 1 or tuple(hw.shape) != (B, 2):
        raise ValueError(f'{fn}: raw [nbytes], off [B], hw [B, 2] with B >= 1')
    if not (1 <= Rh <= 4096 and 1 <= Rw <= 4096):
        raise ValueError(f'{fn}: target {Rh} x {Rw} outside 1..4096' if Rh != Rw else f'{fn}: R = {Rh} outside 1..4096')
    if kind not in (0, 1):
        raise ValueError(f'{fn}: unknown out kind {kind!r} (0: bf16 NHWC-8, 1: fp32 NCHW)')
    dt, numel, align = ((BF16, B * Rh * Rw * 8, 16), (F32, B * 3 * Rh * Rw, 4))[kind]
    if not isinstance(out, torch.Tensor) or not out.is_cuda or out.dtype != dt or not out.is_contiguous() \
            or out.numel() != numel or out.data_ptr() % align:
        raise ValueError(f'{fn}: out must be a contiguous {dt} device tensor of {numel} elements, '
                         f'{align}-byte aligned (kind {kind})')
    if host is None:
        raise ValueError(f'{fn}: host=(off, hw) copies of the tables are required for the bounds check')
    h_off, h_hw = (torch.as_tensor(z) for z in host)
    if h_off.is_cuda or h_hw.is_cuda or h_off.numel() != B or tuple(h_hw.shape) != (B, 2):
        raise ValueError(f'{fn}: host=(off [B], hw [B, 2]) must be host tensors of the same shapes')
    h_off, h_hw = h_off.to(torch.int64), h_hw.to(torch.int64)
    if int(h_hw.min()) < 1 or int(h_hw.max()) > IMAGE_INGEST_MAX_SIDE:
        raise ValueError(f'{fn}: image sides must be in 1..{IMAGE_INGEST_MAX_SIDE}')
    end = h_off + 3 * h_hw[:, 0] * h_hw[:, 1]
    if int(h_off.min()) < 0 or int(end.max()) > raw.numel():
        raise ValueError(f'{fn}: the offset table runs outside the {raw.numel()}-byte buffer')
    return B


def image_ingest(raw, off, hw, R, out, kind, host=None):
    R = int(R)
    B = _image_ingest_args('image_ingest', raw, off, hw, R, R, out, kind, host)
    _lib.call('da_image_ingest', raw.data_ptr(), off.data_ptr(), hw.data_ptr(), B, R, out.data_ptr(), int(kind), _stream())


def image_ingest_rect(raw, off, hw, Rh, Rw, out, kind, host=None):
    Rh, Rw = int(Rh), int(Rw)
    B = _image_ingest_args('image_ingest_rect', raw, off, hw, Rh, Rw, out, kind, host)
    _lib.call('da_image_ingest_rect', raw.data_ptr(), off.data_ptr(), hw.data_ptr(), B, Rh, Rw, out.data_ptr(), int(kind),
              _stream())


def image_resize(raw, off, hw, Rh, Rw, out, kind, geometry, filter, range, host=None):
    Rh, Rw = int(Rh), int(Rw)
    B = _image_ingest_args('image_resize', raw, off, hw, Rh, Rw, out, kind, host)
    for nm, val in (('geometry', geometry), ('filter', filter), ('range', range)):
        if val not in (0, 1):
            raise ValueError(f'image_resize: {nm} must be 0 or 1, got {val!r}')
    _lib.call('da_image_resize', raw.data_ptr(), off.data_ptr(), hw.data_ptr(), B, Rh, Rw, out.data_ptr(), int(kind),
              int(geometry), int(filter), int(range), _stream())


CLIP_MAX_PATCH, CLIP_MAX_SIZE = 32, 448
_CLIP_TABLES = {}


def clip_patch_cols(P: int) -> int:
    return (3 * P * P + 7) // 8 * 8


def clip_preprocess(images, R, P, out, kind, mean, std):
    from .metrics.clip_preprocess import tables_for
    if not isinstance(images, torch.Tensor) or not images.is_cuda or images.dtype != torch.uint8 or images.dim() != 4 \
            or images.shape[1] != 3 or not images.is_contiguous() or images.shape[0] < 1:
        raise ValueError('clip_preprocess: images must be a contiguous uint8 [B, 3, H, W] device tensor')
    B, _, H, W = images.shape
    R, P = int(R), int(P)
    if not (1 <= P <= CLIP_MAX_PATCH and P <= R <= CLIP_MAX_SIZE and R % P == 0):
        raise ValueError(f'clip_preprocess: R = {R}, P = {P} (P <= {CLIP_MAX_PATCH}, R <= {CLIP_MAX_SIZE}, R % P == 0)')
    if not (1 <= H <= IMAGE_INGEST_MAX_SIDE and 1 <= W <= IMAGE_INGEST_MAX_SIDE):
        raise ValueError(f'clip_preprocess: image sides must be in 1..{IMAGE_INGEST_MAX_SIDE}')
    if kind not in (0, 1):
        raise ValueError(f'clip_preprocess: unknown out kind {kind!r} (0: bf16 patch matrix, 1: fp32 pixel_values)')
    dt, shape, align = ((BF16, (B * ((R // P) ** 2 + 1), clip_patch_cols(P)), 16), (F32, (B, 3, R, R), 4))[kind]
    if not isinstance(out, torch.Tensor) or not out.is_cuda or out.dtype != dt or not out.is_contiguous() \
            or tuple(out.shape) != shape or out.data_ptr() % align:
        raise ValueError(f'clip_preprocess: out must be a contiguous {dt} device tensor {shape}, {align}-byte aligned')
    key = (H, W, R, images.device)
    if key not in _CLIP_TABLES:
        _CLIP_TABLES[key] = tuple(torch.from_numpy(t.copy()).to(images.device) for t in tables_for(H, W, R))
    xtab, ytab = _CLIP_TABLES[key]
    f3 = ctypes.c_float * 3
    _lib.call('da_clip_preprocess', images.data_ptr(), B, H, W, R, P, xtab.data_ptr(), xtab.shape[1], ytab.data_ptr(),
              ytab.shape[1], f3(*map(float, mean)), f3(*map(float, std)), out.data_ptr(), int(kind), _stream())
    return out


def clip_score(img, txt, scores, state):
    for z, nm in ((img, 'img'), (txt, 'txt')):
        if z.dim() != 2 or z.dtype != F32 or not z.is_cuda or z.stride(1) != 1 or z.shape != img.shape:
            raise ValueError(f'clip_score: {nm} must be an fp32 [B, D] device matrix with unit column stride')
    B, D = img.shape
    if B < 1 or D < 1:
        raise ValueError('clip_score: empty batch')
    _lib.call('da_clip_score', img.data_ptr(), max(img.stride(0), D), txt.data_ptr(), max(txt.stride(0), D), B, D,
              _vec(scores, B, 'scores'), _vec(state, 2, 'state'), _stream())


def _rescale_operands(fn, factor, HW, npix):
    if HW is None or int(HW) < 1 or npix % int(HW):
        raise ValueError(f'{fn}: factor needs HW, the pixel count of one sample, dividing npix = {npix}; got {HW}')
    if factor.dtype != F32 or not factor.is_cuda or not factor.is_contiguous() or factor.numel() != npix // int(HW):
        raise ValueError(f'{fn}: factor must be a contiguous fp32 [{npix // int(HW)}] device tensor')
    return int(HW)


def guidance_rescale(pred, coef, factor, *, phi, HW, C, g_index):
    C, HW, g_index, phi = int(C), int(HW), int(g_index), float(phi)
    if not 1 <= C <= 8 or HW < 1 or not 0.0 <= phi <= 1.0:
        raise ValueError(f'guidance_rescale: C = {C} (1..8), HW = {HW} (>= 1), phi = {phi} (in [0, 1])')
    if pred.dim() != 2 or pred.shape[1] != 8 or pred.dtype != F32 or not pred.is_cuda or not pred.is_contiguous() \
            or pred.shape[0] < 2 or pred.shape[0] % (2 * HW) or pred.data_ptr() % 16:
        raise ValueError(f'guidance_rescale: pred must be a contiguous fp32 [2 B * {HW}, 8] device tensor, 16-byte aligned')
    npix = pred.shape[0] // 2
    if coef.dtype != F32 or not coef.is_cuda or not coef.is_contiguous() or coef.numel() not in (4, 8) \
            or coef.data_ptr() % 16 or not 0 <= g_index < coef.numel():
        raise ValueError('guidance_rescale: coef must be 4 or 8 contiguous fp32 on the device, 16-byte aligned, g_index inside')
    _rescale_operands('guidance_rescale', factor, HW, npix)
    _lib.call('da_guidance_rescale', pred.data_ptr(), coef.data_ptr(), g_index, phi, factor.data_ptr(), npix, HW, C,
              _stream())


def _sampler_step(ms, blend, pred, x, coef, x_out, xt_out, C, cfg, copies, factor, HW, *, noise=None, hist=None, known8=None,
                  eps8=None, mask=None):
    fn = 'sampler_step' + ('_ms' if ms else '') + ('_blend' if blend else '')
    C, copies, cfg = int(C), int(copies), bool(cfg)
    if not 1 <= C <= 8 or copies not in (1, 2):
        raise ValueError(f'{fn}: C = {C} (1..8), copies = {copies} (1 or 2)')
    if x.dim() != 2 or x.shape[1] != 8 or x.shape[0] < 1:
        raise ValueError(f'{fn}: x must be [npix, 8]')
    npix = x.shape[0]
    mats = [(pred, (2 if cfg else 1) * npix, 'pred'), (x, npix, 'x')] + ([(hist, npix, 'hist')] if ms else []) \
        + [(x_out, npix, 'x_out')] + ([(known8, npix, 'known8'), (eps8, npix, 'eps8')] if blend else [])
    for z, rows, nm in mats:
        if z.dtype != F32 or not z.is_cuda or not z.is_contiguous() or tuple(z.shape) != (rows, 8) or z.data_ptr() % 16:
            raise ValueError(f'{fn}: {nm} must be a contiguous fp32 [{rows}, 8] device tensor, 16-byte aligned')
    if blend and (mask.dtype != F32 or not mask.is_cuda or not mask.is_contiguous() or tuple(mask.shape) != (npix,)
                  or mask.data_ptr() % 16):
        raise ValueError(f'{fn}: mask must be a contiguous fp32 [{npix}] device tensor, 16-byte aligned')
    if ms and hist.data_ptr() in [z.data_ptr() for z in (x, x_out, pred) + ((known8, eps8) if blend else ())]:
        raise ValueError(f'{fn}: hist must be a buffer of its own')
    ncoef = 8 if ms or blend else 4
    if coef.dtype != F32 or not coef.is_cuda or not coef.is_contiguous() or coef.numel() != ncoef or coef.data_ptr() % 16:
        raise ValueError(f'{fn}: coef must be {ncoef} contiguous fp32 on the device, 16-byte aligned')
    HW_arg, HW = HW, npix
    if noise is not None:
        if noise.dim() != 4 or noise.dtype != F32 or not noise.is_cuda or not noise.is_contiguous() \
                or noise.shape[1] != C or noise.shape[0] * noise.shape[2] * noise.shape[3] != npix or noise.data_ptr() % 16:
            raise ValueError(f'{fn}: noise must be a contiguous fp32 [B, {C}, H, W] device tensor over {npix} pixels')
        HW = noise.shape[2] * noise.shape[3]
    if xt_out is not None and (xt_out.dtype != BF16 or not xt_out.is_cuda or not xt_out.is_contiguous()
                               or tuple(xt_out.shape) != (copies * npix, 8) or xt_out.data_ptr() % 16):
# ... 193 lines not shown
```

include/diffusion_amd.h:

```cpp
#ifndef DIFFUSION_AMD_H
#define DIFFUSION_AMD_H

#ifdef __cplusplus
extern "C" {
#endif

typedef struct ihipStream_t* da_stream_t;

int da_gemm_nt(const void* A, long lda, const void* W, void* C, long ldc, const float* bias, const void* rowbias,
               long ldrb, const void* R, long ldr, int M, int N, int K, int Cin, int Hin, int Win, int Hout, int Wout,
               int ksize, int mode, int out_fp32, float alpha, float* splitk_ws, long splitk_ws_floats,
               da_stream_t stream);

int da_gemm_nt_geglu(const void* A, long lda, const void* W, void* F, long ldf, void* G, long ldg, const float* bias,
                     int M, int inner, int K, da_stream_t stream);

int da_gemm_nt_geglu_bwd(const void* dY, long lddy, const void* Wt, const void* F, long ldf, void* dF, long lddf, int M,
                         int inner, int K, da_stream_t stream);

int da_set_option(const char* key, int value);
int da_gemm_nt_variant_for(int M, int N, int K, int Cin, long splitk_ws_floats);

int da_gemm_tn_wgrad(const void* dY, long lddy, const void* X, long ldx, float* dW, float* dbias, float* scratch, int M,
                     int N, int Cin, int Hin, int Win, int Hout, int Wout, int ksize, int mode, float* split_ws,
                     long split_ws_floats, da_stream_t stream);

int da_gemm_tn_variant_for(int M, int N, int Cin, int Hin, int Win, int Hout, int Wout, int ksize, int mode);

typedef struct DaWgradItem {
  const void* dY;
  long lddy;
  const void* X;
  long ldx;
  float* dW;
  float* dbias;
  int N;
  int Cin;
} DaWgradItem;

int da_gemm_tn_wgrad_group(const DaWgradItem* items, int n_items, int M, float* split_ws, long split_ws_floats,
                           da_stream_t stream);

int da_gemm_tn_group_plan(const DaWgradItem* items, int n_items, int M, long split_ws_floats, int* splits, int cap,
                          int* group_of);

int da_attn_fwd(const void* Q, long ldq, const void* K, long ldk, const void* V, long ldv, void* O, long ldo,
                float* L2, int B, int H, int Nq, int Nk, float scale, da_stream_t stream);
int da_attn_fwd_causal(const void* Q, long ldq, const void* K, long ldk, const void* V, long ldv, void* O, long ldo,
                       float* L2, int B, int H, int N, float scale, da_stream_t stream);
int da_attn_fwd_wide(const void* Q, long ldq, const void* K, long ldk, const void* V, long ldv, void* O, long ldo,
                     float* L2, int B, int H, int D, int Nq, int Nk, float scale, da_stream_t stream);
int da_attn_bwd(const void* Q, long ldq, const void* K, long ldk, const void* V, long ldv, const void* O, long ldo,
                const void* dO, long lddo, const float* L2, float* Delta, void* dQ, long lddq, void* dK, long lddk,
                void* dV, long lddv, int B, int H, int Nq, int Nk, float scale, da_stream_t stream);

long da_norm_scratch_floats(int B, int HW, int C);

int da_groupnorm_fwd(const void* X, long ldx, void* Y, long ldy, const float* gamma, const float* beta,
                     float* mean_rstd, float* scale_shift, float* scratch, int B, int HW, int C, int G, float eps,
                     int silu, da_stream_t stream);
int da_groupnorm_bwd(const void* X, long ldx, const void* dY, long lddy, const void* Radd, long ldr, void* dX,
                     long lddx, const float* gamma, const float* beta, const float* mean_rstd, float* dgamma,
                     float* dbeta, float* coef, float* scratch, int B, int HW, int C, int G, int silu,
                     da_stream_t stream);
int da_groupnorm_plan_for(int B, int HW, int C, int G, long ld_min, long ld_max, int bwd, int* out);

int da_layernorm_fwd(const void* X, long ldx, void* Y, long ldy, const float* gamma, const float* beta,
                     float* mean_rstd, int M, int C, float eps, da_stream_t stream);
int da_layernorm_bwd(const void* X, long ldx, const void* dY, long lddy, const void* Radd, long ldr, void* dX,
                     long lddx, const float* gamma, const float* mean_rstd, float* dgamma, float* dbeta,
                     float* scratch, int M, int C, da_stream_t stream);

int da_colsum_accum(const void* X, long ldx, float* out, float* scratch, int M, int C, da_stream_t stream);

int da_image_colsum(const void* X, long ldx, void* out, long ldo, float* db, float* scratch, int B, int HW, int C,
                    da_stream_t stream);

int da_geglu_fwd(const void* in, long ldi, void* out, long ldo, int M, int Cout, da_stream_t stream);
int da_geglu_bwd(const void* in, long ldi, const void* dout, long lddo, void* din, long lddi, int M, int Cout,
                 da_stream_t stream);

int da_silu_fwd(const void* x, long ldx, void* y, long ldy, int M, int C, da_stream_t stream);
int da_gelu_fwd(const void* x, long ldx, void* y, long ldy, int M, int C, da_stream_t stream);
int da_silu_bwd(const void* x, long ldx, const void* dy, long lddy, void* dx, long lddx, int M, int C,
                da_stream_t stream);
int da_quick_gelu_fwd(const void* x, long ldx, void* y, long ldy, int M, int C, da_stream_t stream);

int da_add(const void* a, long lda, const void* b, long ldb, void* o, long ldo, int M, int C, da_stream_t stream);
int da_copy2d(const void* a, long lda, void* o, long ldo, int M, int C, da_stream_t stream);

int da_upsample2x_fwd(const void* x, void* y, int B, int H, int W, int C, da_stream_t stream);
int da_upsample2x_bwd(const void* dy, void* dx, int B, int H, int W, int C, da_stream_t stream);

int da_timestep_embed(const long long* t, void* out, int B, int dim, da_stream_t stream);
int da_timestep_embed_f32(const float* t, void* out, int B, int dim, da_stream_t stream);

int da_add_noise(const float* x0, const float* eps, const long long* t, const float* sqrt_ac,
                 const float* sqrt_1mac, void* xt, float* target, int B, int HW, int v_pred, da_stream_t stream);

int da_add_noise_ex(const float* x0, const float* eps, const void* t, int t_is_f32, const float* sqrt_ac,
                    const float* sqrt_1mac, void* xt, float* target, int B, int C, int HW, int target_kind,
                    da_stream_t stream);

int da_sampler_step(const float* pred, const float* x, const float* noise, const float* coef, float* x_out, void* xt_out,
                    long npix, int HW, int C, int cfg, int copies, da_stream_t stream);
int da_sampler_step_ms(const float* pred, const float* x, float* hist, const float* coef, float* x_out, void* xt_out,
                       long npix, int HW, int C, int cfg, int copies, da_stream_t stream);
int da_sampler_step_blend(const float* pred, const float* x, const float* noise, const float* coef, const float* known8,
                          const float* eps8, const float* mask, float* x_out, void* xt_out, long npix, int HW, int C,
                          int cfg, int copies, da_stream_t stream);
int da_sampler_step_ms_blend(const float* pred, const float* x, float* hist, const float* coef, const float* known8,
                             const float* eps8, const float* mask, float* x_out, void* xt_out, long npix, int HW, int C,
                             int cfg, int copies, da_stream_t stream);
int da_guidance_rescale(const float* pred, const float* coef, int g_index, float phi, float* factor, long npix, int HW,
                        int C, da_stream_t stream);
int da_sampler_step_rs(const float* pred, const float* x, const float* noise, const float* coef, const float* factor,
                       float* x_out, void* xt_out, long npix, int HW, int C, int cfg, int copies, da_stream_t stream);
int da_sampler_step_ms_rs(const float* pred, const float* x, float* hist, const float* coef, const float* factor,
                          float* x_out, void* xt_out, long npix, int HW, int C, int cfg, int copies, da_stream_t stream);
int da_sampler_step_blend_rs(const float* pred, const float* x, const float* noise, const float* coef, const float* known8,
                             const float* eps8, const float* mask, const float* factor, float* x_out, void* xt_out,
                             long npix, int HW, int C, int cfg, int copies, da_stream_t stream);
int da_sampler_step_ms_blend_rs(const float* pred, const float* x, float* hist, const float* coef, const float* known8,
                                const float* eps8, const float* mask, const float* factor, float* x_out, void* xt_out,
                                long npix, int HW, int C, int cfg, int copies, da_stream_t stream);
int da_sampler_init(const float* known, const float* noise, const float* mask_px, const float* coef, float* known8,
                    float* eps8, float* mask, float* x, void* xt, int B, int H, int W, int C, int f, int copies,
                    da_stream_t stream);

int da_image_ingest(const unsigned char* src, const long long* off, const int* hw, int B, int R, void* out, int out_kind,
                    da_stream_t stream);
int da_image_ingest_rect(const unsigned char* src, const long long* off, const int* hw, int B, int Rh, int Rw, void* out,
                         int out_kind, da_stream_t stream);
int da_image_resize(const unsigned char* src, const long long* off, const int* hw, int B, int Rh, int Rw, void* out,
                    int out_kind, int geometry, int filter, int range, da_stream_t stream);

int da_mse_loss(const float* pred, const float* target, void* dpred, float* loss, float* scratch, long total_pix,
                float grad_coef, float weight, int accumulate, da_stream_t stream);
int da_mse_loss_c(const float* pred, const float* target, void* dpred, float* loss, float* scratch, long total_pix,
                  int C, float grad_coef, float weight, int accumulate, da_stream_t stream);
int da_mse_loss_w(const float* pred, const float* target, void* dpred, float* loss, float* scratch, long total_pix, int C,
                  int HW, const long long* t, const float* wtab, int T, float grad_coef, float weight, int accumulate,
                  da_stream_t stream);

int da_adamw(float* p, const float* g, float* m, float* v, void* shadow, float* ema, float ema_smoothing, long n,
             float lr, float beta1, float beta2, float eps, float wd, int step, float grad_scale, da_stream_t stream);

#define DA_SUMSQ_CHUNK 8192
typedef struct DaGradStats {
  float sumsq, norm, grad_mult, finite;
  int skipped_steps;
  int reserved[3];
} DaGradStats;

int da_segment_sumsq(const float* x, const void* chunk_desc, int n_chunks, const void* seg_desc, int n_segs,
                     float* chunk_partials, float* seg_sumsq, float* stats, float grad_scale, float max_norm,
                     da_stream_t stream);
long da_segment_sumsq_scratch_floats(int n_chunks);

int da_adamw_dev(float* p, const float* g, float* m, float* v, void* shadow, float* ema, float ema_smoothing, long n,
                 float lr, float beta1, float beta2, float eps, float wd, int step, const float* stats, da_stream_t stream);

int da_clip_preprocess(const unsigned char* src, int B, int H, int W, int R, int P, const int* xtab, int xld,
                       const int* ytab, int yld, const float* mean, const float* std, void* out, int out_kind,
                       da_stream_t stream);

int da_clip_score(const float* img, long ldi, const float* txt, long ldt, int B, int D, float* scores, float* state,
                  da_stream_t stream);

int da_cast_f32_bf16(const float* src, void* dst, long n, da_stream_t stream);

int da_transpose_weight(const void* src, void* dst, int N, int T, int C, da_stream_t stream);

int da_transpose_weights_batched(const void* src_base, void* dst_base, const void* desc, int ntensors, int total_blocks,
                                 da_stream_t stream);

#ifdef __cplusplus
}
#endif
#endif
```

Before: 1550 images/sec.

## Add thin-channel 3x3 conv kernels and fuse GroupNorm backward with column sum

Adds a specialised MFMA kernel for 3x3 convolutions with 8 input channels (the conv_in on latents), enabled by default. It also adds an opt-in kernel for 8-output fp32 convolutions that computes per-tap partial products in LDS and reduces them. The resnet backward now computes the time-embedding projection column sum inside the resident GroupNorm backward pass and its finalize kernel, instead of re-reading dh1 in a separate image_colsum pass. The intent is to avoid the generic GEMM's padding waste on thin channel counts and one full activation read per resblock, at the cost of extra scratch space and more code paths.

Result: no change. 1553 images/sec (median of 6 runs) (+0.2%).

```diff
diff --git a/diffusion_amd/_lib.py b/diffusion_amd/_lib.py
--- a/diffusion_amd/_lib.py
+++ b/diffusion_amd/_lib.py
@@ -31,10 +31,13 @@
     'da_attn_fwd_wide': [_vp, _l, _vp, _l, _vp, _l, _vp, _l, _fp, _i, _i, _i, _i, _i, _f, _vp],
     'da_attn_bwd': [_vp, _l, _vp, _l, _vp, _l, _vp, _l, _vp, _l, _fp, _fp, _vp, _l, _vp, _l, _vp, _l, _i, _i, _i, _i,
                     _f, _vp],
+    'da_conv_thin_form_for': [_i, _i, _i, _i, _i, _i, _i],
     'da_norm_scratch_floats': [_i, _i, _i],
     'da_groupnorm_fwd': [_vp, _l, _vp, _l, _fp, _fp, _fp, _fp, _fp, _i, _i, _i, _i, _f, _i, _vp],
     'da_groupnorm_bwd': [_vp, _l, _vp, _l, _vp, _l, _vp, _l, _fp, _fp, _fp, _fp, _fp, _fp, _fp, _i, _i, _i, _i, _i,
                          _vp],
+    'da_groupnorm_bwd_colsum': [_vp, _l, _vp, _l, _vp, _l, _vp, _l, _fp, _fp, _fp, _fp, _fp, _fp, _fp, _vp, _l, _fp, _i, _i,
+                                _i, _i, _i, _vp],
     'da_groupnorm_plan_for': [_i, _i, _i, _i, _l, _l, _i, C.POINTER(_i)],
     'da_layernorm_fwd': [_vp, _l, _vp, _l, _fp, _fp, _fp, _i, _i, _f, _vp],
     'da_layernorm_bwd': [_vp, _l, _vp, _l, _vp, _l, _vp, _l, _fp, _fp, _fp, _fp, _fp, _i, _i, _vp],
diff --git a/diffusion_amd/csrc/conv_thin.hip b/diffusion_amd/csrc/conv_thin.hip
--- /dev/null
+++ b/diffusion_amd/csrc/conv_thin.hip
@@ -0,0 +1,251 @@
+#include "common.hpp"
+#include "diffusion_amd.h"
+
+int da_usable_cus(int cus);
+
+namespace {
+
+struct ThinParams {
+  const bf16* A;
+  const bf16* W;
+  void* C;
+  const float* bias;
+  long lda, ldc;
+  int M, N, Cin, H, Wd;
+  int tiles;
+  int R, bands;
+};
+
+constexpr int CT_WAVES = 8, CT_THREADS = 64 * CT_WAVES;
+constexpr int N8_WAVES = 16, N8_THREADS = 64 * N8_WAVES;
+
+__global__ __launch_bounds__(CT_THREADS) void conv_thin_cin8_kernel(ThinParams p) {
+  extern __shared__ __attribute__((aligned(16))) char smem[];
+  const int tid = threadIdx.x, lane = tid & 63, wave = tid >> 6;
+  const int g = lane >> 4, r15 = lane & 15;
+  const int nblk = p.N >> 4;
+  bf16x8* wl = reinterpret_cast<bf16x8*>(smem);
+  float* bl = reinterpret_cast<float*>(smem + (size_t)nblk * 3 * 64 * 16);
+  const int rowB = p.N * 2 + 16;
+  char* ot = reinterpret_cast<char*>(bl + p.N) + (size_t)wave * 16 * rowB;
+  for (int i = tid; i < nblk * 3 * 64; i += CT_THREADS) {
+    const int l = i & 63, bs = i >> 6;
+    const int blk = bs / 3, s = bs - 3 * blk;
+    const int tap = 4 * s + (l >> 4), n = (blk >> 1) * 32 + 2 * (l & 15) + (blk & 1);
+    wl[i] = tap < 9 ? ld8(p.W + (long)n * 72 + tap * 8) : zero8();
+  }
+  for (int i = tid; i < p.N; i += CT_THREADS) bl[i] = p.bias ? p.bias[i] : 0.f;
+  __syncthreads();
+  const int HW = p.H * p.Wd;
+  int dr[3], dc[3];
+  bool tv[3];
+#pragma unroll
+  for (int s = 0; s < 3; ++s) {
+    const int tap = 4 * s + g;
+    tv[s] = tap < 9;
+    dr[s] = tap / 3 - 1;
+    dc[s] = tap - 3 * (tap / 3) - 1;
+  }
+  auto load_a = [&](int tile, bf16x8* a) {
+    const int m = tile * 16 + r15;
+    const int mm = m < p.M ? m : 0;
+    const int b = mm / HW, rem = mm - b * HW;
+    const int oh = rem / p.Wd, ow = rem - oh * p.Wd;
+#pragma unroll
+    for (int s = 0; s < 3; ++s) {
+      const int ih = oh + dr[s], iw = ow + dc[s];
+      const bool ok = tv[s] && m < p.M && ih >= 0 && iw >= 0 && ih < p.H && iw < p.Wd;
+      a[s] = ok ? ld8(p.A + (long)(b * HW + ih * p.Wd + iw) * p.lda) : zero8();
+    }
+  };
+  const int stride = gridDim.x * CT_WAVES;
+  int tile = blockIdx.x * CT_WAVES + wave;
+  bf16x8 a[3], an[3];
+  if (tile < p.tiles) load_a(tile, a);
+  const int nv = p.N >> 3;
+  for (; tile < p.tiles; tile += stride) {
+    if (tile + stride < p.tiles) load_a(tile + stride, an);
+    for (int c4 = 0; c4 < nblk; c4 += 4) {
+      f32x4 acc[4];
+#pragma unroll
+      for (int j = 0; j < 4; ++j) acc[j] = f32x4{0.f, 0.f, 0.f, 0.f};
+#pragma unroll
+      for (int s = 0; s < 3; ++s)
+#pragma unroll
+        for (int j = 0; j < 4; ++j)
+          acc[j] = __builtin_amdgcn_mfma_f32_16x16x32_bf16(a[s], wl[((c4 + j) * 3 + s) * 64 + lane], acc[j], 0, 0, 0);
+#pragma unroll
+      for (int j = 0; j < 4; j += 2) {
+        const int n = ((c4 + j) >> 1) * 32 + 2 * r15;
+        const float2 bv = *reinterpret_cast<const float2*>(bl + n);
+#pragma unroll
+        for (int e = 0; e < 4; ++e) {
+          bf16x2 o;
+          o[0] = f2bf(acc[j][e] + bv.x);
+          o[1] = f2bf(acc[j + 1][e] + bv.y);
+          *reinterpret_cast<bf16x2*>(ot + (4 * g + e) * rowB + n * 2) = o;
+        }
+      }
+    }
+    __builtin_amdgcn_fence(__ATOMIC_RELEASE, "wavefront");
+    __builtin_amdgcn_wave_barrier();
+    int row = 0, c = lane;
+    for (int v = lane; v < 16 * nv; v += 64) {
+      while (c >= nv) {
+        c -= nv;
+        ++row;
+      }
+      const long m = (long)tile * 16 + row;
+      const bf16x8 o = *reinterpret_cast<const bf16x8*>(ot + row * rowB + c * 16);
+      if (m < p.M) st8(reinterpret_cast<bf16*>(p.C) + m * p.ldc + c * 8, o);
+      c += 64;
+    }
+    __builtin_amdgcn_fence(__ATOMIC_ACQUIRE, "wavefront");
+    __builtin_amdgcn_wave_barrier();
+#pragma unroll
+    for (int s = 0; s < 3; ++s) a[s] = an[s];
+  }
+}
+
+constexpr int N8_PLD = 76;
+
+__global__ __launch_bounds__(N8_THREADS) void conv_thin_n8_kernel(ThinParams p) {
+  extern __shared__ __attribute__((aligned(16))) char smem[];
+  const int tid = threadIdx.x, lane = tid & 63, wave = tid >> 6;
+  const int g = lane >> 4, r15 = lane & 15;
+  const int nsteps = p.Cin >> 5, nch = (nsteps + 3) >> 2;
+  bf16x8* wl = reinterpret_cast<bf16x8*>(smem);
+  float* P = reinterpret_cast<float*>(smem + (size_t)5 * nsteps * 64 * 16);
+  const int K = 9 * p.Cin;
+  for (int i = tid; i < 5 * nsteps * 64; i += N8_THREADS) {
+    const int l = i & 63, bs = i >> 6;
+    const int blk = bs / nsteps, s = bs - blk * nsteps;
+    const int col = blk * 16 + (l & 15);
+    const int ci = 32 * s + 8 * (l >> 4);
+    wl[i] = col < 72 ? ld8(p.W + (long)(col & 7) * K + (col >> 3) * p.Cin + ci) : zero8();
+  }
+  const int HW = p.H * p.Wd;
+  float bn = 0.f;
+  if (p.bias) bn = p.bias[tid & 7];
+  for (int bb = blockIdx.x; bb < p.tiles; bb += gridDim.x) {
+    const int img = bb / p.bands, band = bb - img * p.bands;
+    const int y0 = band * p.R;
+    const int rows_out = min(p.R, p.H - y0);
+    const int q_off = (y0 - 1) * p.Wd;
+    const int npx = (rows_out + 2) * p.Wd;
+    const bf16* Ab = p.A + ((long)img * HW + q_off) * p.lda + 8 * g;
+    auto issue = [&](int t, int ch, bf16x8* dst) {
+      const int q = t * 16 + r15;
+      const bool ok = q < npx && q_off + q >= 0 && q_off + q < HW;
+      const bf16* ap = Ab + (long)(ok ? q : -q_off) * p.lda + 128 * ch;
+#pragma unroll
+      for (int u = 0; u < 4; ++u) dst[u] = (ok && 4 * ch + u < nsteps) ? ld8(ap + 32 * u) : zero8();
+    };
+    __syncthreads();
+    int t = wave;
+    bf16x8 a[4], an[4];
+    if (t * 16 < npx) issue(t, 0, a);
+    for (; t * 16 < npx; t += N8_WAVES) {
+      f32x4 acc[5];
+#pragma unroll
+      for (int j = 0; j < 5; ++j) acc[j] = f32x4{0.f, 0.f, 0.f, 0.f};
+      for (int ch = 0; ch < nch; ++ch) {
+        const bool last = ch + 1 == nch;
+        const int nt = last ? t + N8_WAVES : t, nc = last ? 0 : ch + 1;
+        if (nt * 16 < npx) issue(nt, nc, an);
+#pragma unroll
+        for (int u = 0; u < 4; ++u)
+          if (4 * ch + u < nsteps) {
+#pragma unroll
+            for (int j = 0; j < 5; ++j)
+              acc[j] = __builtin_amdgcn_mfma_f32_16x16x32_bf16(a[u], wl[(j * nsteps + 4 * ch + u) * 64 + lane], acc[j], 0, 0, 0);
+          }
+#pragma unroll
+        for (int u = 0; u < 4; ++u) a[u] = an[u];
+      }
+#pragma unroll
+      for (int j = 0; j < 5; ++j) {
+        const int col = j * 16 + r15;
+        if (col < 72) {
+#pragma unroll
+          for (int e = 0; e < 4; ++e) {
+            const int qq = t * 16 + 4 * g + e;
+            if (qq < npx) P[qq * N8_PLD + col] = acc[j][e];
+          }
+        }
+      }
+    }
+    __syncthreads();
+    float* Cb = reinterpret_cast<float*>(p.C);
+    for (int i = tid; i < rows_out * p.Wd * 8; i += N8_THREADS) {
+      const int n = i & 7, px = i >> 3;
+      const int yl = px / p.Wd, x = px - yl * p.Wd;
+      const int y = y0 + yl;
+      float sum = 0.f;
+#pragma unroll
+      for (int r = 0; r < 3; ++r)
+#pragma unroll
+        for (int s = 0; s < 3; ++s) {
+          const int iy = y + r - 1, ix = x + s - 1;
+          if (iy >= 0 && iy < p.H && ix >= 0 && ix < p.Wd) sum += P[((yl + r) * p.Wd + ix) * N8_PLD + (r * 3 + s) * 8 + n];
+        }
+      sum += bn;
+      Cb[((long)img * HW + (long)y * p.Wd + x) * p.ldc + n] = sum;
+    }
+  }
+}
+
+constexpr int CT_LDS = 160 * 1024;
+
+}
+
+int da_conv_thin_form(int N, int Cin, int Hin, int Win, int out_fp32, int* R8) {
+  if (Cin == 8 && !out_fp32 && N % 64 == 0 && N <= 320) return 1;
+  if (N == 8 && out_fp32 && Cin % 32 == 0) {
+    const long wl = 5L * (Cin / 32) * 64 * 16;
+    if (wl >= CT_LDS) return 0;
+    const long rows = (CT_LDS - wl) / ((long)Win * N8_PLD * 4);
+    if (rows < 3) return 0;
+    if (R8) *R8 = (int)(rows - 2 < Hin ? rows - 2 : Hin);
+    return 2;
+  }
+  return 0;
+}
+
+int da_conv_thin_try(const void* A, long lda, const void* W, void* C, long ldc, const float* bias, const void* rowbias,
+                     const void* R, int M, int N, int K, int Cin, int Hin, int Win, int Hout, int Wout, int ksize,
+                     int mode, int out_fp32, float alpha, hipStream_t stream) {
+  if (ksize != 3 || mode != 0 || alpha != 1.0f || rowbias || R || Hin != Hout || Win != Wout || K != 9 * Cin) return -1;
+  if (M >= (1 << 30)) return -1;
+  int R8 = 0;
+  const int form = da_conv_thin_form(N, Cin, Hin, Win, out_fp32, &R8);
+  if (!form) return -1;
+  ThinParams p = {};
+  p.A = (const bf16*)A; p.W = (const bf16*)W; p.C = C; p.bias = bias; p.lda = lda; p.ldc = ldc;
+  p.M = M; p.N = N; p.Cin = Cin; p.H = Hin; p.Wd = Win;
+  if (form == 1) {
+    p.tiles = (M + 15) / 16;
+    const size_t smem = (size_t)(N / 16) * 3 * 64 * 16 + (size_t)N * 4 + (size_t)CT_WAVES * 16 * (N * 2 + 16);
+    int grid = (p.tiles + CT_WAVES - 1) / CT_WAVES;
+    const int cus = da_usable_cus(256);
+    if (grid > cus) grid = cus;
+    static unsigned long long attr_done = 0;
+    if (da_ensure_dyn_smem((const void*)conv_thin_cin8_kernel, CT_LDS, &attr_done) != DA_OK) return DA_ERR_LAUNCH;
+    hipLaunchKernelGGL(conv_thin_cin8_kernel, dim3(grid), dim3(CT_THREADS), smem, stream, p);
+    DA_CHECK_LAUNCH();
+    return DA_OK;
+  }
+  p.bands = (Hin + R8 - 1) / R8;
+  p.R = (Hin + p.bands - 1) / p.bands;
+  const size_t smem = (size_t)5 * (Cin / 32) * 64 * 16 + (size_t)(p.R + 2) * Win * N8_PLD * 4;
+  const long nbands = (long)(M / (Hin * Win)) * p.bands;
+  if (nbands >= (1L << 31)) return -1;
+  p.tiles = (int)nbands;
+  const int cus8 = da_usable_cus(256);
+  const long grid = nbands < cus8 ? nbands : cus8;
+  static unsigned long long attr_done = 0;
+  if (da_ensure_dyn_smem((const void*)conv_thin_n8_kernel, CT_LDS, &attr_done) != DA_OK) return DA_ERR_LAUNCH;
+  hipLaunchKernelGGL(conv_thin_n8_kernel, dim3((unsigned)grid), dim3(N8_THREADS), smem, stream, p);
+  DA_CHECK_LAUNCH();
+  return DA_OK;
+}
diff --git a/diffusion_amd/csrc/gemm_nt.hip b/diffusion_amd/csrc/gemm_nt.hip
--- a/diffusion_amd/csrc/gemm_nt.hip
+++ b/diffusion_amd/csrc/gemm_nt.hip
@@ -234,6 +234,11 @@
 int da_gemm_nt_ws_try(const void* A, long lda, const void* W, const float* bias, const void* R, long ldr, void* C, long ldc,
                       int M, int N, int K, hipStream_t stream);
 extern int g_nt_ws;
+int da_conv_thin_try(const void* A, long lda, const void* W, void* C, long ldc, const float* bias, const void* rowbias,
+                     const void* R, int M, int N, int K, int Cin, int Hin, int Win, int Hout, int Wout, int ksize,
+                     int mode, int out_fp32, float alpha, hipStream_t stream);
+
+int da_conv_thin_form(int N, int Cin, int Hin, int Win, int out_fp32, int* R8);
 
 extern int g_tn_variant;
 extern int g_nt_korder;
@@ -244,7 +249,9 @@
 extern int g_grad_overwrite;
 extern int g_attn_fused_bwd;
 extern int g_tn_ring, g_tn_ungroup;
-extern int g_gn_resident, g_gn_resident_form, g_gn_resident_min_slab;
+extern int g_gn_resident, g_gn_resident_form, g_gn_resident_min_slab, g_gn_colsum_split;
+static int g_conv_thin_off = 0;
+static int g_conv_thin_n8 = 0;
 int da_usable_cus(int cus);
 static int g_nt_variant = 0;
 static int g_nt_mfma32 = 0;
@@ -313,6 +320,13 @@
   return pick_nt_variant(M, N, K, Cin, ws_floats, &s);
 }
 
+extern "C" int da_conv_thin_form_for(int N, int Cin, int Hin, int Win, int ksize, int mode, int out_fp32) {
+  if (g_nt_variant != 0 || ksize != 3 || mode != 0) return 0;
+  const int form = da_conv_thin_form(N, Cin, Hin, Win, out_fp32, nullptr);
+  if (form == 1) return g_conv_thin_off ? 0 : 1;
+  return (form == 2 && g_conv_thin_n8) ? 2 : 0;
+}
+
 extern "C" int da_set_option(const char* key, int value) {
   if (key && !strcmp(key, "gemm_nt_variant")) {
     g_nt_variant = value;
@@ -380,6 +394,21 @@
   if (key && !strcmp(key, "gn_resident")) {
     if (value < 0) return DA_ERR_SHAPE;
     g_gn_resident = value;
+    return DA_OK;
+  }
+  if (key && !strcmp(key, "gn_colsum_split")) {
+    if (value < 0 || value > 1) return DA_ERR_SHAPE;
+    g_gn_colsum_split = value;
+    return DA_OK;
+  }
+  if (key && !strcmp(key, "conv_thin_off")) {
+    if (value < 0 || value > 1) return DA_ERR_SHAPE;
+    g_conv_thin_off = value;
+    return DA_OK;
+  }
+  if (key && !strcmp(key, "conv_thin_n8")) {
+    if (value < 0 || value > 1) return DA_ERR_SHAPE;
+    g_conv_thin_n8 = value;
     return DA_OK;
   }
   if (key && !strcmp(key, "gn_resident_min_slab")) {
@@ -418,6 +447,11 @@
   if (Hout <= 0 || Wout <= 0 || (M % (Hout * Wout))) return DA_ERR_SHAPE;
   if (R && (ldr & 7)) return DA_ERR_SHAPE;
   if (rowbias && (ldrb & 7)) return DA_ERR_SHAPE;
+  if (ksize == 3 && (Cin == 8 || N == 8) && da_conv_thin_form_for(N, Cin, Hin, Win, ksize, mode, out_fp32)) {
+    const int rc = da_conv_thin_try(A, lda, W, C, ldc, bias, rowbias, R, M, N, K, Cin, Hin, Win, Hout, Wout, ksize, mode,
+                                    out_fp32, alpha, stream);
+    if (rc >= 0) return rc;
+  }
   if (g_nt_ws && g_nt_variant == 0 && ksize == 1 && mode == 0 && !out_fp32 && alpha == 1.0f && !rowbias) {
     const int rc = da_gemm_nt_ws_try(A, lda, W, bias, R, ldr, C, ldc, M, N, K, stream);
     if (rc >= 0) return rc;
diff --git a/diffusion_amd/csrc/norms.hip b/diffusion_amd/csrc/norms.hip
--- a/diffusion_amd/csrc/norms.hip
+++ b/diffusion_amd/csrc/norms.hip
@@ -4,6 +4,7 @@
 extern int g_grad_overwrite;
 int g_gn_resident = 192;
 int g_gn_resident_form = 0;
+int g_gn_colsum_split = 0;
 int g_gn_resident_min_slab = 64 * 1024;
 
 namespace {
@@ -431,6 +432,79 @@
   }
 }
 
+__global__ __launch_bounds__(CSF_CH * CSF_RL) void chan_sum3_finalize_kernel(const float* partial, const float* cs, int B,
+                                                                             int C, float* out1, float* out2, bf16* colsum,
+                                                                             long ldo, float* db, int overwrite) {
+  __shared__ float sh[CSF_RL][CSF_CH][3];
+  const int cx = threadIdx.x % CSF_CH, ry = threadIdx.x / CSF_CH;
+  const int c = blockIdx.x * CSF_CH + cx;
+  float a = 0.f, q = 0.f, s = 0.f;
+  if (c < C) {
+    const float2* pp = reinterpret_cast<const float2*>(partial) + c;
+    const float* cp = cs + c;
+    float a0 = 0.f, a1 = 0.f, a2 = 0.f, a3 = 0.f, q0 = 0.f, q1 = 0.f, q2 = 0.f, q3 = 0.f;
+    float s0 = 0.f, s1 = 0.f, s2 = 0.f, s3 = 0.f;
+    int k = ry;
+    for (; k + 3 * CSF_RL < B; k += 4 * CSF_RL) {
+      const float2 v0 = pp[(long)k * C], v1 = pp[(long)(k + CSF_RL) * C], v2 = pp[(long)(k + 2 * CSF_RL) * C],
+                   v3 = pp[(long)(k + 3 * CSF_RL) * C];
+      const float w0 = cp[(long)k * C], w1 = cp[(long)(k + CSF_RL) * C], w2 = cp[(long)(k + 2 * CSF_RL) * C],
+                  w3 = cp[(long)(k + 3 * CSF_RL) * C];
+      a0 += v0.x; q0 += v0.y; s0 += w0;
+      a1 += v1.x; q1 += v1.y; s1 += w1;
+      a2 += v2.x; q2 += v2.y; s2 += w2;
+      a3 += v3.x; q3 += v3.y; s3 += w3;
+      colsum[(long)k * ldo + c] = f2bf(w0);
+      colsum[(long)(k + CSF_RL) * ldo + c] = f2bf(w1);
+      colsum[(long)(k + 2 * CSF_RL) * ldo + c] = f2bf(w2);
+      colsum[(long)(k + 3 * CSF_RL) * ldo + c] = f2bf(w3);
+    }
+    for (; k < B; k += CSF_RL) {
+      const float2 v = pp[(long)k * C];
+      const float w = cp[(long)k * C];
+      a0 += v.x;
+      q0 += v.y;
+      s0 += w;
+      colsum[(long)k * ldo + c] = f2bf(w);
+    }
+    a = (a0 + a1) + (a2 + a3);
+    q = (q0 + q1) + (q2 + q3);
+    s = (s0 + s1) + (s2 + s3);
+  }
+  sh[ry][cx][0] = a;
+  sh[ry][cx][1] = q;
+  sh[ry][cx][2] = s;
+  __syncthreads();
+  float la = 0.f, lq = 0.f, ls = 0.f;
+  if (ry < 8) {
+#pragma unroll
+    for (int j = 0; j < 8; ++j) {
+      la += sh[ry * 8 + j][cx][0];
+      lq += sh[ry * 8 + j][cx][1];
+      ls += sh[ry * 8 + j][cx][2];
+    }
+  }
+  __syncthreads();
+  if (ry < 8) {
+    sh[ry][cx][0] = la;
+    sh[ry][cx][1] = lq;
+    sh[ry][cx][2] = ls;
+  }
+  __syncthreads();
+  if (ry == 0 && c < C) {
+    float ta = 0.f, tq = 0.f, ts = 0.f;
+#pragma unroll
+    for (int j = 0; j < 8; ++j) {
+      ta += sh[j][cx][0];
+      tq += sh[j][cx][1];
+      ts += sh[j][cx][2];
+    }
+    if (out1) out1[c] = overwrite ? ta : out1[c] + ta;
+    if (out2) out2[c] = overwrite ? tq : out2[c] + tq;
+    if (db) db[c] = overwrite ? ts : db[c] + ts;
+  }
+}
+
 constexpr int LN_MAXV = 3;
 
 __global__ __launch_bounds__(256) void ln_fwd_kernel(const bf16* X, long ldx, bf16* Y, long ldy, const float* gamma,
@@ -742,6 +816,7 @@
   long ldx, lddy, ldr, ldo;
   int HW, C, G, cpg, CW, chunks, P, parts, peers8, silu, nseg;
   float eps, inv_n;
+  float* cs_partial;
 };
 
 DEVINL u32x4 ldnt8w(const bf16* p) { return __builtin_nontemporal_load(reinterpret_cast<const u32x4*>(p)); }
@@ -900,7 +975,7 @@
   }
 }
 
-template <int NL, bool SILU, int T>
+template <int NL, bool SILU, int T, bool CS = false>
 __global__ __launch_bounds__(T) void gn_res_bwd_kernel(GnResParams p) {
   extern __shared__ __attribute__((aligned(16))) float smem[];
   float2* red = reinterpret_cast<float2*>(smem);
@@ -1001,7 +1076,7 @@
     gs[gl] = make_float4(mu, rs, -rs * rs * c2, -rs * c1 + mu * rs * rs * c2);
   }
   __syncthreads();
-  if (!live) return;
+  if (!CS) { if (!live) return; }
 #pragma unroll
   for (int w = 0; w < 4; ++w) {
     const float4 f0 = cf[8 * j2 + 2 * w], f1 = cf[8 * j2 + 2 * w + 1];
@@ -1011,7 +1086,7 @@
       const float x0 = bflo(a[k][w]), x1 = bfhi(a[k][w]);
       const float d0 = bflo(b[k][w]), d1 = bfhi(b[k][w]);
       a[k][w] = bfpack(fmaf(d0, f0.z, fmaf(x0, g0q.z, g0q.w)), fmaf(d1, f1.z, fmaf(x1, g1q.z, g1q.w)));
-      if (SILU) __builtin_amdgcn_sched_barrier(0);
+      if (SILU || CS) __builtin_amdgcn_sched_barrier(0);
     }
     __builtin_amdgcn_sched_barrier(0);
   }
@@ -1032,10 +1107,29 @@
       for (int w = 0; w < 4; ++w)
         a[k][w] = bfpack(bflo(a[k][w]) + bflo(b[k][w]), bfhi(a[k][w]) + bfhi(b[k][w]));
   }
+  const bool act = !CS || q0 < p.P;
 #pragma unroll
   for (int k = 0; k < NL; ++k) {
     const int pix = q0 + k * p.P;
-    if (pix < p.HW) st8o(ob, (unsigned)(pix * (int)p.ldo + 8 * j2) * 2u, u32x4{a[k][0], a[k][1], a[k][2], a[k][3]});
+    if ((!CS || act) && pix < p.HW) st8o(ob, (unsigned)(pix * (int)p.ldo + 8 * j2) * 2u, u32x4{a[k][0], a[k][1], a[k][2], a[k][3]});
+  }
+  if constexpr (CS) {
+    const int row = act ? q0 : p.P;
+#pragma unroll
+    for (int w = 0; w < 4; ++w) {
+      float s = 0.f, u = 0.f;
+#pragma unroll
+      for (int k = 0; k < NL; ++k) {
+        const bool ok = act && q0 + k * p.P < p.HW;
+        s += ok ? bflo(a[k][w]) : 0.f;
+        u += ok ? bfhi(a[k][w]) : 0.f;
+      }
+      red[row * p.CW + 8 * j2 + 2 * w] = make_float2(s, 0.f);
+      red[row * p.CW + 8 * j2 + 2 * w + 1] = make_float2(u, 0.f);
+      __builtin_amdgcn_sched_barrier(0);
+    }
+    gn_res_reduce(p, red, red2, chs);
+    for (int c = t; c < p.CW; c += blockDim.x) p.cs_partial[(long)img * p.C + c0 + c] = chs[c].x;
   }
 }
 
@@ -1099,20 +1193,20 @@
   return p.silu ? launch_gn_res_fwd2<NL, true>(p, B, stream) : launch_gn_res_fwd2<NL, false>(p, B, stream);
 }
 
-template <int NL, bool SILU, int T>
+template <int NL, bool SILU, int T, bool CS>
 int launch_gn_res_bwd2(const GnResParams& p, int B, hipStream_t stream) {
   const size_t smem = gn_res_lds_floats(p.P, p.CW, p.nseg, p.cpg) * sizeof(float);
   if (smem > 160 * 1024) return DA_ERR_SHAPE;
   static unsigned long long attr_done = 0;
-  if (da_ensure_dyn_smem((const void*)gn_res_bwd_kernel<NL, SILU, T>, 160 * 1024, &attr_done) != DA_OK) return DA_ERR_LAUNCH;
-  hipLaunchKernelGGL((gn_res_bwd_kernel<NL, SILU, T>), dim3(B * p.parts), dim3(T), smem, stream, p);
+  if (da_ensure_dyn_smem((const void*)gn_res_bwd_kernel<NL, SILU, T, CS>, 160 * 1024, &attr_done) != DA_OK) return DA_ERR_LAUNCH;
+  hipLaunchKernelGGL((gn_res_bwd_kernel<NL, SILU, T, CS>), dim3(B * p.parts), dim3(T), smem, stream, p);
   DA_CHECK_LAUNCH();
   return DA_OK;
 }
 
-template <int NL, int T>
+template <int NL, int T, bool CS>
 int launch_gn_res_bwd(const GnResParams& p, int B, hipStream_t stream) {
-  return p.silu ? launch_gn_res_bwd2<NL, true, T>(p, B, stream) : launch_gn_res_bwd2<NL, false, T>(p, B, stream);
+  return p.silu ? launch_gn_res_bwd2<NL, true, T, CS>(p, B, stream) : launch_gn_res_bwd2<NL, false, T, CS>(p, B, stream);
 }
 
 int gn_res_nl_inst(int nl, bool bwd, int threads) {
@@ -1139,17 +1233,18 @@
   }
 }
 
+template <bool CS>
 int dispatch_gn_res_bwd(int nl, int threads, const GnResParams& p, int B, hipStream_t s) {
-  if (threads == 768) return gn_res_nl_inst(nl, true, 768) == 11 ? launch_gn_res_bwd<11, 768>(p, B, s)
-                                                                  : launch_gn_res_bwd<14, 768>(p, B, s);
+  if (threads == 768) return gn_res_nl_inst(nl, true, 768) == 11 ? launch_gn_res_bwd<11, 768, CS>(p, B, s)
+                                                                  : launch_gn_res_bwd<14, 768, CS>(p, B, s);
   switch (gn_res_nl_inst(nl, true, 1024)) {
-    case 1: return launch_gn_res_bwd<1, 1024>(p, B, s);
-    case 2: return launch_gn_res_bwd<2, 1024>(p, B, s);
-    case 3: return launch_gn_res_bwd<3, 1024>(p, B, s);
-    case 4: return launch_gn_res_bwd<4, 1024>(p, B, s);
-    case 6: return launch_gn_res_bwd<6, 1024>(p, B, s);
-    case 8: return launch_gn_res_bwd<8, 1024>(p, B, s);
-    default: return launch_gn_res_bwd<11, 1024>(p, B, s);
+    case 1: return launch_gn_res_bwd<1, 1024, CS>(p, B, s);
+    case 2: return launch_gn_res_bwd<2, 1024, CS>(p, B, s);
+    case 3: return launch_gn_res_bwd<3, 1024, CS>(p, B, s);
+    case 4: return launch_gn_res_bwd<4, 1024, CS>(p, B, s);
+    case 6: return launch_gn_res_bwd<6, 1024, CS>(p, B, s);
+    case 8: return launch_gn_res_bwd<8, 1024, CS>(p, B, s);
+    default: return launch_gn_res_bwd<11, 1024, CS>(p, B, s);
   }
 }
 
@@ -1158,6 +1253,8 @@
 extern "C" long da_norm_scratch_floats(int B, int HW, int C) {
   long a = (long)B * pick_chunks(B, HW) * C * 2;
   long b = 1024L * C * 2;
+  long c = (long)B * C * 3;
+  if (c > a) a = c;
   return a > b ? a : b;
 }
 
@@ -1206,11 +1303,10 @@
   return launch_gn_apply2(false, ap, B, stream);
 }
 
-extern "C" int da_groupnorm_bwd(const void* X, long ldx, const void* dY, long lddy, const void* Radd, long ldr,
-                                void* dX, long lddx, const float* gamma, const float* beta, const float* mean_rstd,
-                                float* dgamma, float* dbeta, float* coef, float* scratch, int B, int HW, int C, int G,
-                                int silu, hipStream_t stream) {
-  DA_CLEAR_ERR();
+static int groupnorm_bwd_impl(const void* X, long ldx, const void* dY, long lddy, const void* Radd, long ldr, void* dX,
+                              long lddx, const float* gamma, const float* beta, const float* mean_rstd, float* dgamma,
+                              float* dbeta, float* coef, float* scratch, int B, int HW, int C, int G, int silu,
+                              void* colsum_out, long ldo, float* db, hipStream_t stream) {
   if (B <= 0 || HW <= 0 || C <= 0 || G <= 0 || (C % G) || (C & 7) || (ldx & 7) || (lddy & 7) || (lddx & 7))
     return DA_ERR_SHAPE;
   if (Radd && (ldr & 7)) return DA_ERR_SHAPE;
@@ -1226,11 +1322,21 @@
       r.OUT = (bf16*)dX; r.ldo = lddx; r.gamma = gamma; r.beta = beta; r.mean_rstd = const_cast<float*>(mean_rstd);
       r.partial = scratch; r.HW = HW; r.C = C; r.G = G; r.cpg = C / G; r.silu = silu;
       r.inv_n = 1.0f / ((float)(C / G) * (float)HW);
-      int rc = dispatch_gn_res_bwd(nl, threads, r, B, stream);
+      if (colsum_out && !g_gn_colsum_split) {
+        r.cs_partial = scratch + (long)B * C * 2;
+        int rc = dispatch_gn_res_bwd<true>(nl, threads, r, B, stream);
+        if (rc) return rc;
+        hipLaunchKernelGGL(chan_sum3_finalize_kernel, chan_sum_grid(B, C), dim3(CSF_CH * CSF_RL), 0, stream, scratch,
+                           r.cs_partial, B, C, dbeta, dgamma, (bf16*)colsum_out, ldo, db, g_grad_overwrite);
+        DA_CHECK_LAUNCH();
+        return DA_OK;
+      }
+      int rc = dispatch_gn_res_bwd<false>(nl, threads, r, B, stream);
       if (rc) return rc;
       hipLaunchKernelGGL(chan_sum_finalize_kernel, chan_sum_grid(B, C), dim3(CSF_CH * CSF_RL), 0, stream, scratch, B, C, dbeta,
                          dgamma, g_grad_overwrite);
       DA_CHECK_LAUNCH();
+      if (colsum_out) return da_image_colsum(dX, lddx, colsum_out, ldo, db, scratch, B, HW, C, stream);
       return DA_OK;
     }
   }
@@ -1252,7 +1358,28 @@
   ap.OUT = (bf16*)dX; ap.ldo = lddx;
   ap.mean_rstd = mean_rstd; ap.coef = coef; ap.gamma = gamma; ap.beta = beta;
   ap.HW = HW; ap.C = C; ap.G = G; ap.cpg = C / G; ap.silu = silu;
-  return launch_gn_apply2(true, ap, B, stream);
+  rc = launch_gn_apply2(true, ap, B, stream);
+  if (rc || !colsum_out) return rc;
+  return da_image_colsum(dX, lddx, colsum_out, ldo, db, scratch, B, HW, C, stream);
+}
+
+extern "C" int da_groupnorm_bwd(const void* X, long ldx, const void* dY, long lddy, const void* Radd, long ldr,
+                                void* dX, long lddx, const float* gamma, const float* beta, const float* mean_rstd,
+                                float* dgamma, float* dbeta, float* coef, float* scratch, int B, int HW, int C, int G,
+                                int silu, hipStream_t stream) {
+  DA_CLEAR_ERR();
+  return groupnorm_bwd_impl(X, ldx, dY, lddy, Radd, ldr, dX, lddx, gamma, beta, mean_rstd, dgamma, dbeta, coef, scratch, B,
+                            HW, C, G, silu, nullptr, 0, nullptr, stream);
+}
+
+extern "C" int da_groupnorm_bwd_colsum(const void* X, long ldx, const void* dY, long lddy, const void* Radd, long ldr,
+                                       void* dX, long lddx, const float* gamma, const float* beta, const float* mean_rstd,
+                                       float* dgamma, float* dbeta, float* coef, float* scratch, void* colsum_out, long ldo,
+                                       float* db, int B, int HW, int C, int G, int silu, hipStream_t stream) {
+  DA_CLEAR_ERR();
+  if (!colsum_out || ldo < C) return DA_ERR_SHAPE;
+  return groupnorm_bwd_impl(X, ldx, dY, lddy, Radd, ldr, dX, lddx, gamma, beta, mean_rstd, dgamma, dbeta, coef, scratch, B,
+                            HW, C, G, silu, colsum_out, ldo, db, stream);
 }
 
 extern "C" int da_colsum_accum(const void* X, long ldx, float* out, float* scratch, int M, int C,
diff --git a/diffusion_amd/models/unet.py b/diffusion_amd/models/unet.py
--- a/diffusion_amd/models/unet.py
+++ b/diffusion_amd/models/unet.py
@@ -571,10 +571,13 @@
         self._wgrad(dout, a2, conv2.gw, g3, dbias=self.V(p + '.conv2.bias').g, scratch=self._scratch)
         da2 = self._bf(M, cout)
         ops.gemm_nt(dout, conv2.wt, da2, g3)
-        dh1 = self._gn_bwd(h1, da2, None, p + '.norm2', st2, B, HW, 1)
+        to = self.tproj_offsets[p]
+        dh1 = self._bf(M, cout)
+        w2, b2 = self.V(p + '.norm2.weight'), self.V(p + '.norm2.bias')
+        ops.groupnorm_bwd_colsum(h1, da2, None, dh1, w2.p, b2.p, st2, w2.g, b2.g, self._coef, self._scratch,
+                                 self._dtproj[:, to:to + cout], self.V(p + '.conv1.bias').g, B, HW, cout,
+                                 self.cfg.norm_num_groups, 1)
         del da2
-        to = self.tproj_offsets[p]
-        ops.image_colsum(dh1, self._dtproj[:, to:to + cout], self.V(p + '.conv1.bias').g, self._scratch, B, HW)
         self._wgrad(dh1, a1, conv1.gw, g3)
         da1 = self._bf(M, cin)
         ops.gemm_nt(dh1, conv1.wt, da1, g3)
diff --git a/diffusion_amd/ops.py b/diffusion_amd/ops.py
--- a/diffusion_amd/ops.py
+++ b/diffusion_amd/ops.py
@@ -339,6 +339,24 @@
               _f32buf(scratch, norm_scratch_floats(B, HW, C)), B, HW, C, G, int(silu), _stream())
 
 
+def groupnorm_bwd_colsum(X, dY, Radd, dX, gamma, beta, mean_rstd, dgamma, dbeta, coef, scratch, colsum_out, db, B, HW, C,
+                         G, silu):
+    x, ldx = _mat(X, BF16, 'X')
+    dy, lddy = _mat(dY, BF16, 'dY')
+    dx, lddx = _mat(dX, BF16, 'dX')
+    r, ldr = _mat(Radd, BF16, 'Radd') if Radd is not None else (0, 0)
+    o, ldo = _mat(colsum_out, BF16, 'colsum_out')
+    for t in (X, dY, dX) + ((Radd,) if Radd is not None else ()):
+        if tuple(t.shape) != (B * HW, C):
+            raise ValueError('groupnorm_bwd_colsum: bad shapes')
+    if tuple(colsum_out.shape) != (B, C):
+        raise ValueError('groupnorm_bwd_colsum: bad colsum_out shape')
+    _lib.call('da_groupnorm_bwd_colsum', x, ldx, dy, lddy, r, ldr, dx, lddx, _vec(gamma, C), _vec(beta, C),
+              _f32buf(mean_rstd, B * G * 2), _vec(dgamma, C), _vec(dbeta, C), _f32buf(coef, B * G * 2),
+              _f32buf(scratch, norm_scratch_floats(B, HW, C)), o, ldo, _vec(db, C) if db is not None else 0, B, HW, C, G,
+              int(silu), _stream())
+
+
 GN_PLAN_FIELDS = ('threads', 'nl', 'cw', 'parts', 'peers8', 'P', 'nchunks')
 
 
diff --git a/include/diffusion_amd.h b/include/diffusion_amd.h
--- a/include/diffusion_amd.h
+++ b/include/diffusion_amd.h
@@ -11,6 +11,8 @@
                long ldrb, const void* R, long ldr, int M, int N, int K, int Cin, int Hin, int Win, int Hout, int Wout,
                int ksize, int mode, int out_fp32, float alpha, float* splitk_ws, long splitk_ws_floats,
                da_stream_t stream);
+
+int da_conv_thin_form_for(int N, int Cin, int Hin, int Win, int ksize, int mode, int out_fp32);
 
 int da_gemm_nt_geglu(const void* A, long lda, const void* W, void* F, long ldf, void* G, long ldg, const float* bias,
                      int M, int inner, int K, da_stream_t stream);
@@ -63,6 +65,10 @@
                      long lddx, const float* gamma, const float* beta, const float* mean_rstd, float* dgamma,
                      float* dbeta, float* coef, float* scratch, int B, int HW, int C, int G, int silu,
                      da_stream_t stream);
+int da_groupnorm_bwd_colsum(const void* X, long ldx, const void* dY, long lddy, const void* Radd, long ldr, void* dX,
+                            long lddx, const float* gamma, const float* beta, const float* mean_rstd, float* dgamma,
+                            float* dbeta, float* coef, float* scratch, void* colsum_out, long ldo, float* db, int B,
+                            int HW, int C, int G, int silu, da_stream_t stream);
 int da_groupnorm_plan_for(int B, int HW, int C, int G, long ld_min, long ld_max, int bwd, int* out);
 
 int da_layernorm_fwd(const void* X, long ldx, void* Y, long ldy, const float* gamma, const float* beta,
```
